# cure-lab/MotionCraft

Hardware: AMD Instinct MI355X
Metric: sampled SMPL-X frames/sec (196-frame seq, 1000-step DDPM) (higher is better)
Workload: dtype f32

## Files before the change

### include/motioncraft_amd.h

```cpp
#ifndef MOTIONCRAFT_AMD_H
#define MOTIONCRAFT_AMD_H
#include <stdint.h>

#ifdef __cplusplus
extern "C" {
#endif

#define MC_OK 0
#define MC_ERR_ARG 1
#define MC_ERR_HIP 2
#define MC_ERR_STATE 3
#define MC_ERR_NOCONV 4

typedef struct mc_model mc_model;
typedef struct mc_ctx mc_ctx;

typedef struct mc_model_config {
    int32_t input_feats;
    int32_t max_seq_len;
    int32_t latent_dim;
    int32_t num_parts;
    int32_t num_layers;
    int32_t ffn_dim;
    int32_t time_embed_dim;
    int32_t text_latent_dim;
    int32_t max_text_len;
    int32_t num_experts;
    int32_t topk;
    int32_t dyn_heads;
    float capacity_factor;
    float cfg_scale;
    int32_t num_ctrl_layers;
    int32_t ctrl_cond_feats;
    int32_t ctrl_condition_cfg;
} mc_model_config;

#define MC_SAMPLER_DDPM 0
#define MC_SAMPLER_DDIM 1
#define MC_SAMPLER_MULTISTEP 2
typedef struct mc_step_coefs {
    int32_t mode;
    float text_coef;
    float none_coef;
    float c1, c2;
    float log_var;
    float sqrt_recip, sqrt_recipm1, ab, ab_prev, eta;
    float nonzero;
} mc_step_coefs;

typedef struct mc_inpaint {
    const float* gt_dev;
    const uint8_t* keep_dev;
    const float* gt_noise_dev;
    const float* blend_w_dev;
    int32_t blend_len;
} mc_inpaint;

#define MC_MAX_TRANSL 8
typedef struct mc_seed {
    const float* pre_seq_dev;
    const float* pre_noise_dev;
    int32_t pre_len;
    float sqrt_ab, sqrt_1mab;
    int32_t num_transl;
    int32_t transl_channel[MC_MAX_TRANSL];
    float transl_value[MC_MAX_TRANSL][2];
} mc_seed;

const char* mc_last_error(void);
int mc_device_count(int* n);
int mc_set_device(int dev);

int mc_model_create(const mc_model_config* cfg, mc_model** out);
void mc_model_destroy(mc_model* m);
int mc_model_set_param(mc_model* m, const char* name, const float* host, int64_t numel);
int mc_model_finalize(mc_model* m);

int mc_ctx_create(mc_model* m, int32_t batch, int32_t frames, int32_t max_steps, mc_ctx** out);
void mc_ctx_destroy(mc_ctx* c);
int64_t mc_ctx_workspace_bytes(const mc_ctx* c);
int mc_ctx_check(mc_ctx* c, void* stream);
int mc_ctx_profile(mc_ctx* c, int32_t on);
int mc_ctx_profile_read(mc_ctx* c, int64_t rows_filter, double* avg_us, int32_t* count, double* gflop_per_launch);
int mc_ctx_effective_precision(const mc_ctx* c);
int mc_ctx_uses_coop_routing(const mc_ctx* c);
int mc_ctx_enable_capture(mc_ctx* c);
#define MC_PREC_F32 0
#define MC_PREC_F16 1
#define MC_PREC_F16X3 2
int mc_ctx_set_precision(mc_ctx* c, int32_t precision);
#define MC_TIE_STABLE 0
#define MC_TIE_REVERSE 1
int mc_ctx_set_tie_policy(mc_ctx* c, int32_t policy);
int mc_ctx_set_option(mc_ctx* c, const char* key, int64_t value);
int mc_ctx_set_timesteps(mc_ctx* c, const int32_t* t_orig_host, int32_t num_steps, void* stream);
int mc_ctx_set_condition(mc_ctx* c, const float* xf_out_dev, const float* mask_dev, void* stream);
int mc_ctx_set_control(mc_ctx* c, const float* c_feat_dev, int32_t Tc, void* stream);

int mc_denoise(mc_ctx* c, const float* x_t_dev, int32_t step_index, float* out2_dev,
               int32_t stop_after_layers, void* stream);
int mc_sample_step(mc_ctx* c, const float* x_t_dev, int32_t step_index, const mc_step_coefs* coefs,
                   const float* noise_dev, float* x_prev_dev, float* x0_dev, void* stream);

int mc_sample_loop(mc_ctx* c, float* x_dev, const int32_t* step_indices_host, const mc_step_coefs* coefs_host, int32_t num_steps,
                   const float* noise_dev, uint64_t seed, uint64_t noise_draw0, float* x0_last_dev, void* stream);
int mc_op_philox_normal(float* out_dev, uint32_t* bits_dev, int64_t n, uint64_t seed, uint64_t draw, void* stream);

int mc_ctx_graph_capture(mc_ctx* c, float* x_dev, const float* noise_dev, const mc_step_coefs* coefs_host, int32_t num_steps,
                         void* stream);
int mc_ctx_graph_step(mc_ctx* c, int32_t step_index, void* stream);
int mc_ctx_graph_release(mc_ctx* c);

int mc_sample_step_seeded(mc_ctx* c, float* x_t_dev, int32_t step_index, const mc_step_coefs* coefs,
                          const float* noise_dev, const mc_seed* seed, float* x_prev_dev, float* x0_dev, void* stream);

int mc_sample_step_inpaint(mc_ctx* c, const float* x_t_dev, int32_t step_index, const mc_step_coefs* coefs,
                           const float* noise_dev, const mc_inpaint* inpaint, float* x_prev_dev, float* x0_dev,
                           void* stream);

int mc_ctx_get_buffer(mc_ctx* c, const char* name, int32_t layer, void** dev_ptr, int64_t* numel);

int mc_debug_flop_ledger(int32_t enable);
int64_t mc_debug_flop_ledger_dump(char* buf, int64_t cap);

enum { MC_ACT_NONE = 0, MC_ACT_GELU = 1, MC_ACT_SILU = 2, MC_ACT_LRELU = 3, MC_ACT_QUICKGELU = 4 };
int mc_op_gemm(const float* a_dev, const float* w_dev, const float* bias_dev, const float* res_dev,
               float* c_dev, int32_t M, int32_t N, int32_t K, int32_t ldw, int32_t act, void* stream);
int mc_op_gemm_f16(const float* a_dev, const float* w_dev, const float* bias_dev, const float* res_dev, float* c_dev,
                   int32_t M, int32_t N, int32_t K, int32_t split, void* stream);
int mc_op_gemm_f16_planes(const void* a_hi_dev, const void* a_lo_dev, const float* w_dev, const float* bias_dev, const float* res_dev,
                          float* c_dev, int32_t M, int32_t N, int32_t K, int32_t split, int32_t pre, int32_t frag_major, void* stream);
int mc_op_gemm_tail(const float* h_dev, const float* a_dev, const float* w_dev, const float* bias_dev, float* c_dev, float* c2_dev,
                    int32_t M, int32_t N, int32_t K, float wc, float wu, int32_t variant, void* stream);
int mc_op_ln_rows(const float* x_dev, int64_t ldx, const float* gamma_dev, const float* beta_dev,
                  const float* add_dev, int32_t add_mod, float* y_dev, int64_t rows, int32_t L, void* stream);
enum { MC_TEMPORAL_STEP = 0,
       MC_TEMPORAL_WHOLE = 1,
       MC_TEMPORAL_LSPLIT = 2,
       MC_TEMPORAL_PAIR = 3,
       MC_TEMPORAL_F16X3 = 4,
       MC_TEMPORAL_F16 = 5 };
int mc_op_body_attention(const float* mf_dev, int64_t ldmf, const float* qkv_dev, const float* wsm_dev, float* ys_dev, int64_t frames,
                         int32_t H, int32_t L, int64_t twin_from, const int32_t* split_flag_dev, int64_t frame0, void* stream);
int mc_op_temporal_attention(const float* mf_dev, const float* tf_dev, const float* mask_dev, float* yt_dev, int32_t b0, int32_t nb,
                             int32_t B, int32_t T, int32_t Nt, int32_t H, int32_t L, int32_t form, int32_t skip_text,
                             const int32_t* twin_flag_dev, void* stream);
enum { MC_ENC_ATTN_LAYER = 0,
       MC_ENC_ATTN_SMALL = 1,
       MC_ENC_ATTN_STREAM = 2 };
int mc_op_enc_ln(const float* x_dev, const float* gamma_dev, const float* beta_dev, float* y_dev, int64_t rows, int32_t L, float eps,
                 int32_t relu, void* stream);
int mc_op_enc_embed_tokens(const int32_t* ids_dev, const float* emb_dev, const float* pos_dev, float* x_dev, int64_t rows, int32_t S,
                           int32_t d, int32_t vocab, void* stream);
int mc_op_enc_attention(const float* qkv_dev, const uint8_t* valid_dev, float* out_dev, int32_t B, int32_t S, int32_t d, int32_t heads,
                        int32_t causal, int32_t form, void* stream);
enum { MC_GM_PLAIN = 0, MC_GM_ENC = 4 };
typedef struct mc_gemm_strided {
    const float* a_dev; int64_t lda, a_gstride;
    const float* w_dev; int64_t ldw, w_gstride;
    const float* bias_dev; int64_t b_gstride;
    float* c_dev; int64_t ldc, c_gstride;
    const float* res_dev; int64_t ldr, r_gstride;
    const float* add_dev; int64_t ld_add, dup_rows;
    int32_t add_mod, act, act_after_res, M, N, K;
} mc_gemm_strided;
int mc_op_gemm_strided(int32_t mode, int32_t groups, const mc_gemm_strided* args, void* stream);
int mc_op_bigru_steps(const float* gi_dev, const float* whh_dev, const float* bhh_dev, float* h_dev, const int32_t* lens_dev,
                      int32_t len_div, int32_t B, int32_t S, int32_t H, int32_t s0, int32_t steps, void* stream);
int mc_op_conv1d_k4s2(const float* x_dev, int64_t ldx, const float* w_tapmajor_dev, const float* bias_dev, float* y_padded_dev, int32_t B,
                      int32_t T, int32_t C, int32_t Cp, int32_t O, float slope, void* stream);
int mc_op_sampler_update(const float* x_t_dev, const float* out_text_dev, const float* out_none_dev,
                         const float* noise_dev, float* x_prev_dev, float* x0_dev, int64_t n,
                         const mc_step_coefs* coefs, void* stream);
int mc_op_sampler_multistep(const float* x_t_dev, const float* out_text_dev, const float* out_none_dev, float* x0_hist_dev,
                            float* x_prev_dev, float* x0_dev, int64_t n, const mc_step_coefs* coefs, void* stream);

#define MC_POST_MAXTAP 129
int mc_postprocess_smplx(const float* pred_dev, const int32_t* lengths_dev, const double* mean_dev,
                         const double* std_dev, const double* taps_dev, const int32_t radius[4], int32_t stats_f32,
                         int32_t B, int32_t T, int32_t C, double* poses_dev, double* expr_dev, double* trans_dev,
                         void* stream);
int mc_postprocess_smplx_stitched(const float* pred_dev, const int32_t* rows_dev, int32_t n_frames,
                                  const double* mean_dev, const double* std_dev, const double* taps_dev,
                                  const int32_t radius[4], int32_t stats_f32, int32_t C, double* poses_dev,
                                  double* expr_dev, double* trans_dev, void* stream);

int mc_postprocess_t2m_joints(const float* pred_dev, const int32_t* lengths_dev, const double* mean_dev,
                              const double* std_dev, const double* taps_dev, int32_t radius, int32_t stats_f32,
                              int32_t B, int32_t T, int32_t C, int32_t joints_num, float* joints_out_dev, void* stream);
int mc_postprocess_t2m_joints_stitched(const float* pred_dev, const int32_t* rows_dev, int32_t n_frames,
                                       const double* mean_dev, const double* std_dev, const double* taps_dev,
                                       int32_t radius, int32_t stats_f32, int32_t C, int32_t joints_num,
                                       double* work_dev, float* joints_out_dev, void* stream);

typedef struct mc_textenc mc_textenc;
typedef struct mc_textenc_config {
    int32_t clip_dim;
    int32_t text_latent_dim;
    int32_t num_layers;
    int32_t ff_size;
    int32_t num_heads;
    int32_t max_len;
    int32_t clip_layers;
    int32_t clip_heads;
    int32_t clip_ff;
    int32_t vocab;
} mc_textenc_config;
int mc_textenc_create(const mc_textenc_config* cfg, mc_textenc** out);
void mc_textenc_destroy(mc_textenc* e);
int mc_textenc_set_param(mc_textenc* e, const char* name, const float* host, int64_t numel);
int mc_textenc_finalize(mc_textenc* e);
int mc_textenc_forward_feat(mc_textenc* e, const float* clip_feat_dev, int32_t B, float* xf_out_dev, void* stream);
int mc_textenc_forward_tokens(mc_textenc* e, const int32_t* tokens_dev, int32_t B, float* clip_feat_out_dev,
                              float* xf_out_dev, void* stream);

typedef struct mc_evalenc mc_evalenc;
typedef struct mc_evalenc_config {
    int32_t nfeats;
    int32_t latent_dim;
    int32_t ff_size;
    int32_t num_layers;
    int32_t num_heads;
    int32_t pe_len;
    int32_t bert_dim;
    int32_t bert_layers;
    int32_t bert_heads;
    int32_t bert_ff;
    int32_t bert_vocab;
    int32_t bert_max_pos;
} mc_evalenc_config;
int mc_evalenc_create(const mc_evalenc_config* cfg, mc_evalenc** out);
void mc_evalenc_destroy(mc_evalenc* e);
int mc_evalenc_set_param(mc_evalenc* e, const char* name, const float* host, int64_t numel);
int mc_evalenc_finalize(mc_evalenc* e);
int mc_evalenc_encode_motion(mc_evalenc* e, const float* motion_dev, const int32_t* lengths_dev, int32_t B, int32_t T,
                             float* mu_out_dev, void* stream);
int mc_evalenc_encode_text(mc_evalenc* e, const int32_t* ids_dev, const uint8_t* mask_dev, int32_t B, int32_t S,
                           float* mu_out_dev, void* stream);

typedef struct mc_t2meval mc_t2meval;
typedef struct mc_t2meval_config {
    int32_t input_size;
    int32_t movement_hidden;
    int32_t movement_latent;
    int32_t motion_hidden;
    int32_t motion_latent;
    int32_t word_size;
    int32_t pos_size;
    int32_t text_hidden;
    int32_t text_out;
} mc_t2meval_config;
int mc_t2meval_create(const mc_t2meval_config* cfg, mc_t2meval** out);
void mc_t2meval_destroy(mc_t2meval* e);
int mc_t2meval_set_param(mc_t2meval* e, const char* name, const float* host, int64_t numel);
int mc_t2meval_finalize(mc_t2meval* e);
int mc_t2meval_encode_motion(mc_t2meval* e, const float* motion_dev, const int32_t* lengths_dev, int32_t B, int32_t T,
                             float* out_dev, void* stream);
int mc_t2meval_encode_text(mc_t2meval* e, const float* word_emb_dev, const float* pos_onehot_dev, const int32_t* sent_len_dev,
                           int32_t B, int32_t S, float* out_dev, void* stream);

typedef struct mc_wavenc mc_wavenc;
int mc_wavenc_create(int32_t audio_in, int32_t out_dim, mc_wavenc** out);
void mc_wavenc_destroy(mc_wavenc* e);
int mc_wavenc_set_param(mc_wavenc* e, const char* name, const float* host, int64_t numel);
int mc_wavenc_finalize(mc_wavenc* e);
int mc_wavenc_out_len(const mc_wavenc* e, int32_t samples, int32_t* frames);
int mc_wavenc_forward(mc_wavenc* e, const float* wav_dev, int32_t B, int32_t samples, float* out_dev, void* stream);

typedef struct mc_smplx mc_smplx;
typedef struct mc_smplx_config {
    int32_t num_vertices;
    int32_t num_joints;
    int32_t num_betas;
    int32_t num_expr;
    int32_t num_pose_feats;
} mc_smplx_config;
int mc_smplx_create(const mc_smplx_config* cfg, mc_smplx** out);
void mc_smplx_destroy(mc_smplx* m);
int mc_smplx_set_param(mc_smplx* m, const char* name, const float* host, int64_t numel);
int mc_smplx_finalize(mc_smplx* m);
int mc_smplx_joints(mc_smplx* m, const double* poses_dev, const double* expr_dev, const double* trans_dev,
                    const double* betas_dev, int32_t betas_per_frame, int32_t n, float* joints_out_dev, void* stream);
int64_t mc_smplx_work_bytes(const mc_smplx* m, int32_t n_frames, int32_t betas_per_frame);
int mc_smplx_vertices(mc_smplx* m, const double* poses_dev, const double* expr_dev, const double* trans_dev,
                      const double* betas_dev, int32_t betas_per_frame, int32_t n, void* work_dev, int64_t work_bytes,
                      float* verts_out_dev, float* joints_out_dev, void* stream);
int64_t mc_smplx_vertex_errors_work_bytes(const mc_smplx* m, int32_t chunk_frames, int32_t n_frames, int32_t betas_per_frame);
int mc_smplx_vertex_errors(mc_smplx* m, const double* poses_a_dev, const double* expr_a_dev, const double* trans_a_dev,
                           const double* poses_b_dev, const double* expr_b_dev, const double* trans_b_dev, const double* betas_dev,
                           int32_t betas_per_frame, int32_t n, void* work_dev, int64_t work_bytes, double* sums_out_dev, void* stream);

#define MC_BEAT_MAX_ORDER 64
#define MC_BEAT_MAX_UPPER 64
int mc_beat_mask(const float* joints_dev, int32_t n_frames, int32_t num_joints, const double* mean_vel_dev, int32_t mean_vel_fp32,
                 int32_t t_start, int32_t t_end, double pose_fps, int32_t order, double threshold, uint8_t* mask_out_dev, void* stream);
int64_t mc_beat_align_work_bytes(int32_t n_slice, int32_t n_upper);
int mc_beat_align(const uint8_t* mask_dev, int32_t num_joints, int32_t n_slice, const int32_t* upper_body_host, int32_t n_upper,
                  const double* onsets_dev, int32_t n_onsets, double pose_fps, double sigma, void* work_dev, int64_t work_bytes,
                  double* score_out_dev, void* stream);

#define MC_ONSET_N_FFT 2048
#define MC_ONSET_MAX_HOP 512
#define MC_ONSET_MAX_MELS 128
int64_t mc_onset_work_bytes(int64_t n_samples, int32_t n_fft, int32_t hop, int32_t n_mels);
int mc_onset_strength(const float* wave_dev, int64_t n_samples, const float* dft_dev, const float* mel_dev, int32_t n_fft, int32_t hop,
                      int32_t n_mels, void* work_dev, int64_t work_bytes, float* env_out_dev, void* stream);
int mc_onset_pick(const float* env_dev, int32_t n_frames, int32_t pre_max, int32_t post_max, int32_t pre_avg, int32_t post_avg, double delta,
                  int32_t wait, int32_t normalize, uint8_t* mask_out_dev, int32_t* count_out_dev, void* stream);

#define MC_AUDIO_COND_MAX_WINDOW 1024
#define MC_AUDIO_COND_TILE 4096
int mc_audio_condition(const float* wave_dev, int64_t n_samples, int32_t window, const uint8_t* onset_mask_dev, int32_t n_frames,
                       float* out_dev, void* stream);

#define MC_RESAMPLE_TILE 512
int mc_pcm_decode(const uint8_t* pcm_dev, int64_t n_frames, int32_t channels, int32_t sample_bytes, int32_t mono, float* out_dev, void* stream);
int64_t mc_resample_out_len(int64_t n_in, int32_t up, int32_t down);
int mc_resample_poly(const float* x_dev, int64_t n_in, int32_t up, int32_t down, const double* taps_dev, int32_t n_taps, float* y_dev,
                     int64_t n_out, void* stream);
// ... 76 lines not shown
```

### motioncraft_amd/csrc/mc_ctx.h

```cpp
#pragma once
#include <map>
#include <mutex>
#include <string>
#include <vector>

#include "../../include/motioncraft_amd.h"
#include "mc_common.h"
#include "mc_gemm.h"
#include "mc_kernels.h"
#include "mc_chain.h"
#include "mc_half.h"
#include "mc_options.h"
#include "mc_params.h"

struct mc_model {
    mc_model_config cfg;
    ParamStore params{""};
    std::map<std::string, HalfW> half;
    std::mutex half_mu;
    size_t half_bytes = 0;
    bool finalized = false;
    int Cp = 0;
};

struct MoeW {
    const float *emb, *gate_w, *gate_b, *sim_n, *sim_nT, *scale, *fc1_w, *fc1_b, *fc2_wt, *fc2_b, *proj_w, *proj_b;
    int din, dout;
};

struct LayerW {
    const float *norm_g, *norm_b, *tnorm_g, *tnorm_b, *wsm;
    MoeW mm, tm;
    const float *dyn_g, *dyn_b, *qkv_w, *qkv_b;
    const float *ca_film_w, *ca_film_b, *ca_ln_g, *ca_ln_b, *ca_out_w, *ca_out_b;
    const float *ffn_w1, *ffn_b1, *ffn_w2, *ffn_b2;
    const float *ffn_film_w, *ffn_film_b, *ffn_ln_g, *ffn_ln_b, *ffn_out_w, *ffn_out_b;
    const float *before_w = nullptr, *before_b = nullptr, *after_w = nullptr, *after_b = nullptr;
    HalfW h_ca_out, h_ffn_out, h_fc1, h_fc2, h_w1, h_w2, h_after, h_proj, h_qkv;
};

struct ProfRec { hipEvent_t e0 = nullptr, e1 = nullptr; long rows = 0; };

struct mc_ctx {
    mc_model* m = nullptr;
    McOptions opt{};
    int B = 0, T = 0, S = 0, maxS = 0;
    long N = 0, rows = 0, Ntxt = 0;
    std::vector<LayerW> lw;
    const float *enc_w, *enc_b, *seq_emb, *time_w0, *time_b0, *time_w2, *time_b2, *dec_w, *dec_b;
    const float *dec_wf = nullptr, *dec_bf = nullptr;
    float *dec_cat_w = nullptr, *dec_cat_b = nullptr;
    const float *ctrl_in_w = nullptr, *ctrl_in_b = nullptr;
    int NLA = 0;
    float *hc = nullptr, *cb = nullptr, *cenc = nullptr;
    bool have_ctrl = false;
    std::vector<void*> allocs;
    int64_t bytes = 0;
    float *h, *z, *proj, *hbuf, *y2, *mf, *qkv, *ys, *yt, *a, *z2, *fh, *out2, *xpad;
    float* a_tail = nullptr;
    size_t hbuf_cap = 0;
    size_t hbuf_floats = 0;
    bool cnt_clean = false;
    long led_nsrc = 0, led_gsplit = 0;
    float *xfn, *tf;
    const float* mask = nullptr;
    float* mask_own = nullptr;
    int* t_orig;
    float *te, *e1, *emb, *semb, *ss;
    RouteBufs rb;
    int device = 0;
    int coop_reserved = 0;
    bool prof_on = false;
    std::vector<ProfRec> prof;
    bool have_cond = false;
    hipStream_t side = nullptr;
    bool xpad_ready = false;
    hipEvent_t ev_fork = nullptr, ev_join = nullptr;
    hipEvent_t ev_side = nullptr;
    hipEvent_t ev_stag = nullptr;
    hipEvent_t ev_gate1 = nullptr, ev_sel = nullptr, ev_front = nullptr;
    bool early_clean = false;
    bool no_alias = false;
    bool defer_last_gemm = false;
    static constexpr int SIDE_CAND = 4;
    hipStream_t side_cand[SIDE_CAND] = {nullptr, nullptr, nullptr, nullptr};
    hipStream_t side_for = nullptr;
    bool side_picked = false;
    float side_probe_ms[SIDE_CAND] = {0.f, 0.f, 0.f, 0.f};
    static constexpr int SIDE_MEMO = 4;
    hipStream_t side_memo_for[SIDE_MEMO] = {nullptr, nullptr, nullptr, nullptr};
    int side_memo_pick[SIDE_MEMO] = {-1, -1, -1, -1};
    int side_memo_n = 0;
    int* gstep = nullptr;
    SamplerCoefs* gcoefs = nullptr;
    bool graph_mode = false;
    hipGraph_t graph = nullptr;
    hipGraphExec_t graph_exec = nullptr;
    int graph_steps = 0;
    float* x0_hist = nullptr;
    bool hist_valid = false;
    bool graph_multistep = false;
    std::vector<float> graph_k1;
    int prec = MC_PREC_F32;
    int* cap_idx = nullptr;
    float* cap_w = nullptr;
};

#pragma GCC visibility push(hidden)
inline bool chain_on(const mc_ctx* c, ChainBit which) { return (c->opt.chain >> which) & 1; }
bool use_half(const mc_ctx* c);
int dense(const mc_ctx* c, const float* A, long lda, const float* W, long ldw, const float* bias, const float* R, long ldr,
          float* C, long ldc, long M, int N, int K, int act, hipStream_t s);
int run_moe(mc_ctx* c, const MoeW& w, const float* z, long Ntok, float* out, long ldout, bool gated, bool twin, long gsplit,
            hipStream_t s, const HalfW* hw, const HalfW* hw2);
inline float* deferred_a(const mc_ctx* c) { return c->a_tail ? c->a_tail : c->a; }
bool a_holds_planes(const mc_ctx* c);
int denoise_impl(mc_ctx* c, const float* x_t, int32_t step, float* out2_dev, int32_t stop_after, void* stream, const SeedArgs* seed);
SamplerCoefs to_coefs(const mc_step_coefs* k);

struct X0Parts {
    const float *a = nullptr, *b = nullptr;
    const float* second() const { return b ? b : a; }
    SamplerCoefs coefs(const mc_step_coefs* k) const {
        SamplerCoefs sc = to_coefs(k);
        sc.text_coef = 1.f; sc.none_coef = b ? 1.f : 0.f;
        return sc;
    }
};
int denoise_combined(mc_ctx* c, const float* x_t, int32_t step, const mc_step_coefs* k, void* stream, X0Parts* x0, const SeedArgs* seed = nullptr);
int sampler_update(mc_ctx* c, const float* x_t, const X0Parts& x0p, const mc_step_coefs* k, const float* noise, float* x_prev, float* x0,
                   hipStream_t s, const RngArgs* rng = nullptr, const PadOut* pad = nullptr);
#pragma GCC visibility pop
```

### motioncraft_amd/csrc/mc_gemm.h

```cpp
#pragma once
#include <hip/hip_runtime.h>
#include "mc_options.h"
#include "../../include/motioncraft_amd.h"

enum { GM_PLAIN = MC_GM_PLAIN, GM_EXP1 = 1, GM_EXP2 = 2, GM_COMB = 3, GM_ENC = MC_GM_ENC };

enum : int {
    kTuneStaging = 1 << 0,
    kTuneDma = 1 << 4,
    kTuneWp = 1 << 5,
    kTuneNoXcd = 1 << 6,
    kTuneSmallXcd = 1 << 8,
    kTuneEncWp = 1 << 9,
    kTuneTail2 = 1 << 10,
    kTuneBits = kTuneStaging | kTuneDma | kTuneWp | kTuneNoXcd | kTuneSmallXcd | kTuneEncWp | kTuneTail2,
    kTuneDefault = kTuneBits & ~kTuneNoXcd,
};
static_assert(kTuneDefault == 1841, "the default tune bits are public ABI");

struct GemmArgs {
    const float* A = nullptr;
    long lda = 0;
    int a_col = 0;
    long a_gstride = 0;
    const float* W = nullptr;
    long ldw = 0;
    long w_gstride = 0;
    const float* bias = nullptr;
    long b_gstride = 0;
    float* C = nullptr;
    long ldc = 0;
    int c_col = 0;
    long c_gstride = 0;
    const float* R = nullptr;
    long ldr = 0;
    long r_gstride = -1;
    int act = 0;
    int act_after_res = 0;
    const float* add = nullptr;
    int add_mod = 1;
    long ld_add = 0;
    long dup_rows = 0;
    int M = 0, N = 0, K = 0;
    const int* tile_group = nullptr;
    const int* tile_row0 = nullptr;
    const int* tile_nrows = nullptr;
    const int* num_tiles = nullptr;
    const int* src_row = nullptr;
    const int* dst_row = nullptr;
    const float* comb_w = nullptr;
    int small_tile_n = 0;
    int wp_grid = 0;
    int tune = -1;
};

inline void mc_gemm_opts(const McOptions& o, GemmArgs& g) {
    g.tune = (int)o.gemm_tune;
    g.small_tile_n = o.small_tile_n ? (int)o.small_tile_n : -1;
    g.wp_grid = o.gemm_wp_grid > 0 ? (int)o.gemm_wp_grid : -1;
}

inline double mc_cu_load(long workgroups) {
    const long n = (workgroups + 255) / 256;
    return (1.45 * (double)(n / 2) + (double)(n % 2));
}

int mc_device_cus();
int mc_launch_gemm(int mode, const GemmArgs& g, int groups, int max_tiles, hipStream_t stream);
int mc_launch_gemm_small(const GemmArgs& g, hipStream_t stream, int groups = 1);

struct TailArgs {
    const float* H = nullptr;
    const float* Af = nullptr;
    long half = 0, lda = 0;
    const float* W = nullptr;
    long ldw = 0, w_gstride = 0;
    const float* bias = nullptr;
    long b_gstride = 0;
    float* C = nullptr;
    float* C2 = nullptr;
    long ldc = 0;
    int M = 0, N = 0, K = 0;
    float wc = 1.f, wu = 0.f;
    const float* coef_table = nullptr;
    const int* step_ptr = nullptr;
    long coef_stride = 0;
    int tune = -1;
};
int mc_launch_gemm_tail(const TailArgs& g, hipStream_t stream);
bool mc_gemm_tail_two_outputs(const TailArgs& g);
```

### motioncraft_amd/csrc/mc_gemm.hip

```cpp
#include "mc_common.h"
#include "mc_gemm.h"

namespace {

constexpr int BM = 128, BN = 128, BK = 32, LD = BK + 4;

struct Stage {
    long aoff[4], woff[4];
    bool aok[4], wok[4];
    float cw0[4], cw1[4];
};

template <int MODE, bool GUARD>
__device__ __forceinline__ void load_tile(const GemmArgs& g, const float* __restrict__ Ab, const float* __restrict__ Wb,
                                          const Stage& st, int k, f32x4 (&ra)[4], f32x4 (&rb)[4]) {
    const bool kin = !GUARD || k < g.K;
#pragma unroll
    for (int i = 0; i < 4; ++i) {
        f32x4 v = {0.f, 0.f, 0.f, 0.f};
        if ((!GUARD || st.aok[i]) && kin) {
            if constexpr (MODE == GM_COMB) {
                f32x4 y0 = {0.f, 0.f, 0.f, 0.f}, y1 = {0.f, 0.f, 0.f, 0.f};
                if (st.cw0[i] != 0.f) y0 = *reinterpret_cast<const f32x4*>(Ab + st.aoff[i] + k);
                if (st.cw1[i] != 0.f) y1 = *reinterpret_cast<const f32x4*>(Ab + st.aoff[i] + g.lda + k);
#pragma unroll
                for (int j = 0; j < 4; ++j) v[j] = gelu_exact(st.cw0[i] * y0[j] + st.cw1[i] * y1[j]);
            } else if constexpr (MODE == GM_ENC && GUARD) {
#pragma unroll
                for (int j = 0; j < 4; ++j)
                    if (k + j < g.K) v[j] = Ab[st.aoff[i] + k + j];
            } else {
                v = *reinterpret_cast<const f32x4*>(Ab + st.aoff[i] + k);
            }
        }
        ra[i] = v;
        f32x4 w = {0.f, 0.f, 0.f, 0.f};
        if ((!GUARD || st.wok[i]) && kin) w = *reinterpret_cast<const f32x4*>(Wb + st.woff[i] + k);
        rb[i] = w;
    }
}

template <int MODE, bool GUARD, bool EARLY>
__device__ __forceinline__ void mainloop(const GemmArgs& g, const float* __restrict__ Ab, const float* __restrict__ Wb,
                                         const Stage& st, float* As, float* Bs, int sr, int sk, int wm, int wn, int lane,
                                         f32x16 (&acc)[2][2]) {
    f32x4 ra[4], rb[4];
    auto store_tile = [&](int buf) {
#pragma unroll
        for (int i = 0; i < 4; ++i) {
            *reinterpret_cast<f32x4*>(As + buf * BM * LD + (sr + 32 * i) * LD + sk) = ra[i];
            *reinterpret_cast<f32x4*>(Bs + buf * BN * LD + (sr + 32 * i) * LD + sk) = rb[i];
        }
    };
    const int nk = (g.K + BK - 1) / BK;
    const int frow = lane & 31;
    const int fk = (lane >> 5) * 4;
    struct Frag { f32x4 a0, a1, b0, b1; };
    auto ld_frag = [&](const float* Ap, const float* Bp, int j) {
        Frag f;
        f.a0 = *reinterpret_cast<const f32x4*>(Ap + j * 8);
        f.a1 = *reinterpret_cast<const f32x4*>(Ap + 32 * LD + j * 8);
        f.b0 = *reinterpret_cast<const f32x4*>(Bp + j * 8);
        f.b1 = *reinterpret_cast<const f32x4*>(Bp + 32 * LD + j * 8);
        return f;
    };
    auto mma = [&](const Frag& f) {
#pragma unroll
        for (int i = 0; i < 4; ++i) {
            acc[0][0] = __builtin_amdgcn_mfma_f32_32x32x2f32(f.b0[i], f.a0[i], acc[0][0], 0, 0, 0);
            acc[0][1] = __builtin_amdgcn_mfma_f32_32x32x2f32(f.b1[i], f.a0[i], acc[0][1], 0, 0, 0);
            acc[1][0] = __builtin_amdgcn_mfma_f32_32x32x2f32(f.b0[i], f.a1[i], acc[1][0], 0, 0, 0);
            acc[1][1] = __builtin_amdgcn_mfma_f32_32x32x2f32(f.b1[i], f.a1[i], acc[1][1], 0, 0, 0);
        }
    };
    if constexpr (!EARLY) {
        load_tile<MODE, GUARD>(g, Ab, Wb, st, sk, ra, rb);
        store_tile(0);
        __syncthreads();
        for (int kt = 0; kt < nk; ++kt) {
            const int buf = kt & 1;
            if (kt + 1 < nk) load_tile<MODE, GUARD>(g, Ab, Wb, st, (kt + 1) * BK + sk, ra, rb);
            const float* Ap = As + buf * BM * LD + (wm * 64 + frow) * LD + fk;
            const float* Bp = Bs + buf * BN * LD + (wn * 64 + frow) * LD + fk;
            Frag f0 = ld_frag(Ap, Bp, 0);
            Frag f1 = ld_frag(Ap, Bp, 1);
            mma(f0);
            f0 = ld_frag(Ap, Bp, 2);
            mma(f1);
            f1 = ld_frag(Ap, Bp, 3);
            mma(f0);
            mma(f1);
            if (kt + 1 < nk) store_tile(buf ^ 1);
            __syncthreads();
        }
    } else {
        load_tile<MODE, GUARD>(g, Ab, Wb, st, sk, ra, rb);
        store_tile(0);
        if (nk > 1) load_tile<MODE, GUARD>(g, Ab, Wb, st, BK + sk, ra, rb);
        __syncthreads();
        for (int kt = 0; kt < nk; ++kt) {
            const int buf = kt & 1;
            const float* Ap = As + buf * BM * LD + (wm * 64 + frow) * LD + fk;
            const float* Bp = Bs + buf * BN * LD + (wn * 64 + frow) * LD + fk;
            Frag f0 = ld_frag(Ap, Bp, 0);
            Frag f1 = ld_frag(Ap, Bp, 1);
            mma(f0);
            f0 = ld_frag(Ap, Bp, 2);
            if (kt + 1 < nk) store_tile(buf ^ 1);
            if (kt + 2 < nk) load_tile<MODE, GUARD>(g, Ab, Wb, st, (kt + 2) * BK + sk, ra, rb);
            mma(f1);
            f1 = ld_frag(Ap, Bp, 3);
            mma(f0);
            mma(f1);
            __syncthreads();
        }
    }
}

template <int MODE, bool GUARD, int ACT>
__device__ __forceinline__ void epilogue_vec(const GemmArgs& g, int grp, int row0, int nrows, int tn, int wm, int wn,
                                             int lane, f32x16 (&acc)[2][2]) {
    const float* __restrict__ bias = g.bias ? g.bias + (long)grp * g.b_gstride : nullptr;
    float* __restrict__ Cb = g.C + (long)grp * g.c_gstride + g.c_col;
    const float* __restrict__ Rb = g.R ? g.R + (long)grp * (g.r_gstride >= 0 ? g.r_gstride : g.c_gstride) + g.c_col : nullptr;
#pragma unroll
    for (int mi = 0; mi < 2; ++mi) {
        const int m = wm * 64 + mi * 32 + (lane & 31);
        if (GUARD && m >= nrows) continue;
        long drow = row0 + m;
        if constexpr (MODE == GM_EXP2) drow = g.dst_row[row0 + m];
        float* crow = Cb + drow * g.ldc;
        const float* rrow = Rb ? Rb + drow * g.ldr : nullptr;
        const float* arow = nullptr;
        if constexpr (MODE == GM_ENC) arow = g.add ? g.add + (long)((row0 + m) % g.add_mod) * g.ld_add : nullptr;
#pragma unroll
        for (int ni = 0; ni < 2; ++ni) {
#pragma unroll
            for (int q = 0; q < 4; ++q) {
                const int n = tn * BN + wn * 64 + ni * 32 + 8 * q + 4 * (lane >> 5);
                if (GUARD && n >= g.N) continue;
                f32x4 v = {acc[mi][ni][4 * q], acc[mi][ni][4 * q + 1], acc[mi][ni][4 * q + 2], acc[mi][ni][4 * q + 3]};
                if (bias) v += *reinterpret_cast<const f32x4*>(bias + n);
                if (g.act_after_res && rrow) v += *reinterpret_cast<const f32x4*>(rrow + n);
#pragma unroll
                for (int j = 0; j < 4; ++j) v[j] = apply_act(v[j], ACT);
                if constexpr (MODE == GM_ENC) {
                    if (arow) v += *reinterpret_cast<const f32x4*>(arow + n);
                }
                if (!g.act_after_res && rrow) v += *reinterpret_cast<const f32x4*>(rrow + n);
                *reinterpret_cast<f32x4*>(crow + n) = v;
                if constexpr (MODE == GM_ENC) {
                    if (g.dup_rows) *reinterpret_cast<f32x4*>(crow + g.dup_rows * g.ldc + n) = v;
                }
            }
// ... 52 lines not shown
    }
    const int tm = bid / ntn, tn = bid % ntn;
    int row0, nrows;
    if constexpr (MODE == GM_EXP1 || MODE == GM_EXP2) {
        grp = g.tile_group[tm];
        row0 = g.tile_row0[tm];
        nrows = g.tile_nrows[tm];
    } else {
        row0 = tm * BM;
        nrows = min(BM, g.M - row0);
        if (nrows <= 0) return;
    }
    const float* __restrict__ Ab = g.A + (long)grp * g.a_gstride + g.a_col;
    const float* __restrict__ Wb = g.W + (long)grp * g.w_gstride;

    const int sr = tid >> 3;
    const int sk = (tid & 7) * 4;
    Stage st;
#pragma unroll
    for (int i = 0; i < 4; ++i) {
        const int r = sr + 32 * i;
        st.aok[i] = r < nrows;
        long srow = row0 + r;
        if constexpr (MODE == GM_EXP1) srow = st.aok[i] ? g.src_row[row0 + r] : 0;
        if constexpr (MODE == GM_COMB) {
            st.aoff[i] = 2 * srow * g.lda;
            st.cw0[i] = st.aok[i] ? g.comb_w[2 * srow] : 0.f;
            st.cw1[i] = st.aok[i] ? g.comb_w[2 * srow + 1] : 0.f;
        } else {
            st.aoff[i] = srow * g.lda;
        }
        const int n = tn * BN + r;
        st.wok[i] = n < g.N;
        st.woff[i] = (long)n * g.ldw;
    }

    f32x16 acc[2][2];
#pragma unroll
    for (int mi = 0; mi < 2; ++mi)
#pragma unroll
        for (int ni = 0; ni < 2; ++ni)
#pragma unroll
            for (int r = 0; r < 16; ++r) acc[mi][ni][r] = 0.f;

    const bool full = nrows == BM && (tn + 1) * BN <= g.N && (g.K % BK) == 0 &&
                      (MODE != GM_ENC || (g.lda % 4 == 0 && g.a_gstride % 4 == 0));
    if (full) {
        if (g.tune & kTuneStaging) mainloop<MODE, false, true>(g, Ab, Wb, st, As, Bs, sr, sk, wm, wn, lane, acc);
        else mainloop<MODE, false, false>(g, Ab, Wb, st, As, Bs, sr, sk, wm, wn, lane, acc);
    } else {
        mainloop<MODE, true, false>(g, Ab, Wb, st, As, Bs, sr, sk, wm, wn, lane, acc);
    }

    const bool vec = (g.N % 4 == 0) && (g.ldc % 4 == 0) && (g.c_col % 4 == 0) && (g.c_gstride % 4 == 0) &&
                     (!g.R || (g.ldr % 4 == 0 && (g.r_gstride < 0 || g.r_gstride % 4 == 0)));
    if (!vec) {
        epilogue_scalar<MODE>(g, grp, row0, nrows, tn, wm, wn, lane, acc);
    } else if (full) {
        if (g.act == ACT_GELU) epilogue_vec<MODE, false, ACT_GELU>(g, grp, row0, nrows, tn, wm, wn, lane, acc);
        else if (g.act == ACT_SILU) epilogue_vec<MODE, false, ACT_SILU>(g, grp, row0, nrows, tn, wm, wn, lane, acc);
        else if (g.act == ACT_LRELU) epilogue_vec<MODE, false, ACT_LRELU>(g, grp, row0, nrows, tn, wm, wn, lane, acc);
        else if (g.act == ACT_QUICKGELU) epilogue_vec<MODE, false, ACT_QUICKGELU>(g, grp, row0, nrows, tn, wm, wn, lane, acc);
        else epilogue_vec<MODE, false, ACT_NONE>(g, grp, row0, nrows, tn, wm, wn, lane, acc);
    } else {
        if (g.act == ACT_GELU) epilogue_vec<MODE, true, ACT_GELU>(g, grp, row0, nrows, tn, wm, wn, lane, acc);
        else if (g.act == ACT_SILU) epilogue_vec<MODE, true, ACT_SILU>(g, grp, row0, nrows, tn, wm, wn, lane, acc);
        else if (g.act == ACT_LRELU) epilogue_vec<MODE, true, ACT_LRELU>(g, grp, row0, nrows, tn, wm, wn, lane, acc);
        else if (g.act == ACT_QUICKGELU) epilogue_vec<MODE, true, ACT_QUICKGELU>(g, grp, row0, nrows, tn, wm, wn, lane, acc);
        else epilogue_vec<MODE, true, ACT_NONE>(g, grp, row0, nrows, tn, wm, wn, lane, acc);
    }
}

__global__ __launch_bounds__(256, 2) void gemm_dma_k(GemmArgs g) {
    __shared__ __attribute__((aligned(16))) float smem[2 * (BM + BN) * BK];
    float* As = smem;
    float* Bs = smem + 2 * BM * BK;
    const int tid = threadIdx.x, lane = tid & 63, wave = tid >> 6;
    const int wm = wave >> 1, wn = wave & 1;
    const int ntn = g.N / BN;
    const int bid = (g.tune & kTuneNoXcd) ? (int)blockIdx.x : xcd_remap(blockIdx.x, gridDim.x);
    const int tm = bid / ntn, tn = bid % ntn;
    const int row0 = tm * BM;
    const float* __restrict__ Ab = g.A + g.a_col;
    const float* __restrict__ Wb = g.W;
    const int dr = lane >> 3, dc = ((lane & 7) ^ dr) * 4;
    const float* ga = Ab + (long)(row0 + 32 * wave + dr) * g.lda + dc;
    const float* gw = Wb + (long)(tn * BN + 32 * wave + dr) * g.ldw + dc;
    const int wave_u = __builtin_amdgcn_readfirstlane(wave);
    auto issue = [&](int kt, int buf) {
        float* la = As + buf * BM * BK + 32 * wave_u * BK;
        float* lw = Bs + buf * BN * BK + 32 * wave_u * BK;
#pragma unroll
        for (int q = 0; q < 4; ++q) {
            __builtin_amdgcn_global_load_lds(ga + (long)8 * q * g.lda + kt * BK, la + 8 * q * BK, 16, 0, 0);
            __builtin_amdgcn_global_load_lds(gw + (long)8 * q * g.ldw + kt * BK, lw + 8 * q * BK, 16, 0, 0);
        }
    };
    f32x16 acc[2][2];
#pragma unroll
    for (int mi = 0; mi < 2; ++mi)
#pragma unroll
        for (int ni = 0; ni < 2; ++ni)
#pragma unroll
            for (int r = 0; r < 16; ++r) acc[mi][ni][r] = 0.f;
    const int frow = lane & 31, hf = lane >> 5, sw = frow & 7;
    struct Frag { f32x4 a0, a1, b0, b1; };
    auto ld_frag = [&](const float* At, const float* Bt, int j) {
        const int pos = ((2 * j + hf) ^ sw) * 4;
        Frag f;
        f.a0 = *reinterpret_cast<const f32x4*>(At + pos);
        f.a1 = *reinterpret_cast<const f32x4*>(At + 32 * BK + pos);
        f.b0 = *reinterpret_cast<const f32x4*>(Bt + pos);
        f.b1 = *reinterpret_cast<const f32x4*>(Bt + 32 * BK + pos);
        return f;
    };
    auto mma = [&](const Frag& f) {
#pragma unroll
        for (int i = 0; i < 4; ++i) {
            acc[0][0] = __builtin_amdgcn_mfma_f32_32x32x2f32(f.b0[i], f.a0[i], acc[0][0], 0, 0, 0);
            acc[0][1] = __builtin_amdgcn_mfma_f32_32x32x2f32(f.b1[i], f.a0[i], acc[0][1], 0, 0, 0);
            acc[1][0] = __builtin_amdgcn_mfma_f32_32x32x2f32(f.b0[i], f.a1[i], acc[1][0], 0, 0, 0);
            acc[1][1] = __builtin_amdgcn_mfma_f32_32x32x2f32(f.b1[i], f.a1[i], acc[1][1], 0, 0, 0);
        }
    };
    const int nk = g.K / BK;
    issue(0, 0);
    __syncthreads();
    for (int kt = 0; kt < nk; ++kt) {
        const int buf = kt & 1;
        if (kt + 1 < nk) issue(kt + 1, buf ^ 1);
        const float* At = As + buf * BM * BK + (wm * 64 + frow) * BK;
        const float* Bt = Bs + buf * BN * BK + (wn * 64 + frow) * BK;
        Frag f0 = ld_frag(At, Bt, 0);
        Frag f1 = ld_frag(At, Bt, 1);
        __builtin_amdgcn_sched_barrier(0);
        mma(f0);
        f0 = ld_frag(At, Bt, 2);
        __builtin_amdgcn_sched_barrier(0);
        mma(f1);
        f1 = ld_frag(At, Bt, 3);
        __builtin_amdgcn_sched_barrier(0);
        mma(f0);
        mma(f1);
        __syncthreads();
    }
    if (g.act == ACT_GELU) epilogue_vec<GM_PLAIN, false, ACT_GELU>(g, 0, row0, BM, tn, wm, wn, lane, acc);
    else if (g.act == ACT_SILU) epilogue_vec<GM_PLAIN, false, ACT_SILU>(g, 0, row0, BM, tn, wm, wn, lane, acc);
    else if (g.act == ACT_NONE) epilogue_vec<GM_PLAIN, false, ACT_NONE>(g, 0, row0, BM, tn, wm, wn, lane, acc);
    else epilogue_vec<GM_PLAIN, false, ACT_LRELU>(g, 0, row0, BM, tn, wm, wn, lane, acc);
}

constexpr int WBK = 16, WSTAGE = 128 * WBK;

__global__ __launch_bounds__(256, 2) void gemm_wp_k(GemmArgs g) {
    __shared__ __attribute__((aligned(16))) float smem[4 * 2 * WSTAGE];
    const int tid = threadIdx.x, lane = tid & 63, wave = tid >> 6;
    const int wm = wave >> 1, wn = wave & 1;
    const int ntn = g.N / BN, ntiles = (g.M / BM) * ntn;
    const int wave_u = __builtin_amdgcn_readfirstlane(wave);
    float* wbase = smem + wave_u * 2 * WSTAGE;
    const unsigned lds0 = (unsigned)(size_t)wbase;
    const int dr = lane >> 2, dc = ((lane & 3) ^ ((dr >> 2) & 3)) * 4;
    const int frow = lane & 31, hf = lane >> 5, sw = (frow >> 2) & 3;
    const float* Ab = g.A + g.a_col;
    const float* Wb = g.W;
    const float* __restrict__ Rb = g.R ? g.R + g.c_col : nullptr;
    float* __restrict__ Cb = g.C + g.c_col;
    const int nk = g.K / WBK;
    struct Frag { f32x4 a0, a1, b0, b1; };
    auto ld_frag = [&](int st, int j) {
        const float* S = wbase + st * WSTAGE + frow * WBK + ((2 * j + hf) ^ sw) * 4;
        Frag f;
        f.a0 = *reinterpret_cast<const f32x4*>(S);
        f.a1 = *reinterpret_cast<const f32x4*>(S + 32 * WBK);
        f.b0 = *reinterpret_cast<const f32x4*>(S + 64 * WBK);
        f.b1 = *reinterpret_cast<const f32x4*>(S + 96 * WBK);
        return f;
    };
    for (int t = blockIdx.x; t < ntiles; t += gridDim.x) {
        const int bid = (g.tune & kTuneNoXcd) ? t : xcd_remap(t, ntiles);
        const int tm = bid / ntn, tn = bid % ntn;
        const int row0 = tm * BM;
        unsigned voa[4], vow[4];
#pragma unroll
        for (int q = 0; q < 4; ++q) {
            voa[q] = (unsigned)(((long)(row0 + wm * 64 + 16 * q + dr) * g.lda + dc) * 4);
            vow[q] = (unsigned)(((long)(tn * BN + wn * 64 + 16 * q + dr) * g.ldw + dc) * 4);
        }
        auto issue_q = [&](int kt, int st, int q) {
            const unsigned l = lds0 + st * WSTAGE * 4;
            dma16(voa[q], Ab + kt * WBK, l + q * 1024);
            dma16(vow[q], Wb + kt * WBK, l + 4096 + q * 1024);
        };
        f32x16 acc[2][2];
#pragma unroll
        for (int mi = 0; mi < 2; ++mi)
#pragma unroll
            for (int ni = 0; ni < 2; ++ni)
#pragma unroll
                for (int r = 0; r < 16; ++r) acc[mi][ni][r] = 0.f;
        auto mma2 = [&](const Frag& f, int i0) {
#pragma unroll
            for (int i = i0; i < i0 + 2; ++i) {
                acc[0][0] = __builtin_amdgcn_mfma_f32_32x32x2f32(f.b0[i], f.a0[i], acc[0][0], 0, 0, 0);
                acc[0][1] = __builtin_amdgcn_mfma_f32_32x32x2f32(f.b1[i], f.a0[i], acc[0][1], 0, 0, 0);
                acc[1][0] = __builtin_amdgcn_mfma_f32_32x32x2f32(f.b0[i], f.a1[i], acc[1][0], 0, 0, 0);
                acc[1][1] = __builtin_amdgcn_mfma_f32_32x32x2f32(f.b1[i], f.a1[i], acc[1][1], 0, 0, 0);
            }
        };
#pragma unroll
        for (int q = 0; q < 4; ++q) issue_q(0, 0, q);
        asm volatile("s_waitcnt vmcnt(0)" ::: "memory");
        Frag f0 = ld_frag(0, 0);
        auto ktile = [&](int kt) {
            const int st = kt & 1;
            const bool more = kt + 1 < nk;
            Frag f1 = ld_frag(st, 1);
            __builtin_amdgcn_sched_barrier(0);
            mma2(f0, 0);
            if (more) { issue_q(kt + 1, st ^ 1, 0); issue_q(kt + 1, st ^ 1, 1); }
            __builtin_amdgcn_sched_barrier(0);
            mma2(f0, 2);
            if (more) { issue_q(kt + 1, st ^ 1, 2); issue_q(kt + 1, st ^ 1, 3); }
            __builtin_amdgcn_sched_barrier(0);
            mma2(f1, 0);
            if (more) {
                asm volatile("s_waitcnt vmcnt(0)" ::: "memory");
                f0 = ld_frag(st ^ 1, 0);
            }
            __builtin_amdgcn_sched_barrier(0);
            mma2(f1, 2);
        };
        const int npre = nk > 2 ? nk - 2 : 0;
        for (int kt = 0; kt < npre; ++kt) ktile(kt);
        f32x4 rv[2][2][4], bv[2][4];
#pragma unroll
        for (int ni = 0; ni < 2; ++ni)
#pragma unroll
            for (int q = 0; q < 4; ++q) {
                const int n = tn * BN + wn * 64 + ni * 32 + 8 * q + 4 * hf;
                bv[ni][q] = g.bias ? *reinterpret_cast<const f32x4*>(g.bias + n) : f32x4{0.f, 0.f, 0.f, 0.f};
#pragma unroll
                for (int mi = 0; mi < 2; ++mi) {
                    const long m = row0 + wm * 64 + mi * 32 + frow;
                    rv[mi][ni][q] = Rb ? *reinterpret_cast<const f32x4*>(Rb + m * g.ldr + n) : f32x4{0.f, 0.f, 0.f, 0.f};
                    if (g.add) rv[mi][ni][q] = *reinterpret_cast<const f32x4*>(g.add + (m % g.add_mod) * g.ld_add + n);
                }
            }
        for (int kt = npre; kt < nk; ++kt) ktile(kt);
#pragma unroll
        for (int mi = 0; mi < 2; ++mi) {
            float* crow = Cb + (long)(row0 + wm * 64 + mi * 32 + frow) * g.ldc;
#pragma unroll
            for (int ni = 0; ni < 2; ++ni)
#pragma unroll
                for (int q = 0; q < 4; ++q) {
                    const int n = tn * BN + wn * 64 + ni * 32 + 8 * q + 4 * hf;
                    f32x4 v = {acc[mi][ni][4 * q], acc[mi][ni][4 * q + 1], acc[mi][ni][4 * q + 2], acc[mi][ni][4 * q + 3]};
                    v += bv[ni][q];
                    if (g.act != ACT_NONE) {
#pragma unroll
                        for (int jj = 0; jj < 4; ++jj) v[jj] = apply_act(v[jj], g.act);
                    }
                    v += rv[mi][ni][q];
                    *reinterpret_cast<f32x4*>(crow + n) = v;
                    if (g.dup_rows) *reinterpret_cast<f32x4*>(crow + g.dup_rows * g.ldc + n) = v;
                }
        }
    }
}

constexpr int SM = 64, SN = 64, SRING = 4;
template <bool VEC>
__global__ __launch_bounds__(256) void gemm_small_k(GemmArgs g) {
    __shared__ __attribute__((aligned(16))) float smem[SRING * 2 * SM * BK];
    const int tid = threadIdx.x, lane = tid & 63, wave = tid >> 6;
    const int wm = wave >> 1, wn = wave & 1;
    const int ntn = (g.N + SN - 1) / SN;
    const int bid = (g.tune & kTuneSmallXcd) ? xcd_remap((int)blockIdx.x, (int)gridDim.x) : (int)blockIdx.x;
    const int tm = bid / ntn, tn = bid % ntn, grp = blockIdx.y;
    const int row0 = tm * SM;
    const int wave_u = __builtin_amdgcn_readfirstlane(wave);
    const int dr = lane >> 3, dc = ((lane & 7) ^ dr) * 4;
    const float* Ab = g.A + (long)grp * g.a_gstride + g.a_col;
    const float* Wb = g.W + (long)grp * g.w_gstride;
    unsigned voa[2], vow[2];
#pragma unroll
    for (int q = 0; q < 2; ++q) {
        const int ar = min(row0 + 16 * wave + 8 * q + dr, g.M - 1), wr = min(tn * SN + 16 * wave + 8 * q + dr, g.N - 1);
        voa[q] = (unsigned)(((long)ar * g.lda + dc) * 4);
        vow[q] = (unsigned)(((long)wr * g.ldw + dc) * 4);
    }
    const unsigned lds0 = (unsigned)(size_t)smem + (unsigned)(16 * wave_u) * BK * 4;
    auto issue = [&](int kt) {
        const unsigned l = lds0 + (unsigned)(kt & (SRING - 1)) * (2 * SM * BK * 4);
#pragma unroll
        for (int q = 0; q < 2; ++q) {
            dma16(voa[q], Ab + kt * BK, l + q * 8 * BK * 4);
            dma16(vow[q], Wb + kt * BK, l + SM * BK * 4 + q * 8 * BK * 4);
        }
    };
    f32x16 acc;
#pragma unroll
    for (int r = 0; r < 16; ++r) acc[r] = 0.f;
    const int nk = g.K / BK;
    const int frow = lane & 31, hf = lane >> 5, sw = frow & 7;
    const int me = min(row0 + wm * 32 + frow, g.M - 1);
    const long rgs = g.r_gstride >= 0 ? g.r_gstride : g.c_gstride;
    f32x4 pb[4], pa[4], pr[4];
    if constexpr (VEC) {
#pragma unroll
        for (int q = 0; q < 4; ++q) {
            const int n = tn * SN + wn * 32 + 8 * q + 4 * hf;
            const f32x4 z = {0.f, 0.f, 0.f, 0.f};
            pb[q] = g.bias ? *reinterpret_cast<const f32x4*>(g.bias + (long)grp * g.b_gstride + n) : z;
            pa[q] = g.add ? *reinterpret_cast<const f32x4*>(g.add + (long)(me % g.add_mod) * g.ld_add + n) : z;
            pr[q] = g.R ? *reinterpret_cast<const f32x4*>(g.R + (long)grp * rgs + (long)me * g.ldr + g.c_col + n) : z;
        }
    }
    for (int kt = 0; kt < SRING - 1 && kt < nk; ++kt) issue(kt);
    for (int kt = 0; kt < nk; ++kt) {
        const int ahead = min(nk - 1 - kt, SRING - 2);
        if (ahead == 2) asm volatile("s_waitcnt vmcnt(8)" ::: "memory");
        else if (ahead == 1) asm volatile("s_waitcnt vmcnt(4)" ::: "memory");
        else asm volatile("s_waitcnt vmcnt(0)" ::: "memory");
        __syncthreads();
        if (kt + SRING - 1 < nk) issue(kt + SRING - 1);
        const float* St = smem + (kt & (SRING - 1)) * (2 * SM * BK);
        const float* At = St + (wm * 32 + frow) * BK;
        const float* Bt = St + SM * BK + (wn * 32 + frow) * BK;
        f32x4 fa[4], fb[4];
#pragma unroll
        for (int j = 0; j < 4; ++j) {
            const int pos = ((2 * j + hf) ^ sw) * 4;
            fa[j] = *reinterpret_cast<const f32x4*>(At + pos);
            fb[j] = *reinterpret_cast<const f32x4*>(Bt + pos);
        }
        __builtin_amdgcn_sched_barrier(0);
#pragma unroll
        for (int j = 0; j < 4; ++j)
#pragma unroll
            for (int i = 0; i < 4; ++i) acc = __builtin_amdgcn_mfma_f32_32x32x2f32(fb[j][i], fa[j][i], acc, 0, 0, 0);
    }
    const int m = row0 + wm * 32 + frow;
    if (m >= g.M) return;
    float* crow = g.C + (long)grp * g.c_gstride + (long)m * g.ldc + g.c_col;
    const float* rrow = g.R ? g.R + (long)grp * rgs + (long)m * g.ldr + g.c_col : nullptr;
    const float* arow = g.add ? g.add + (long)(m % g.add_mod) * g.ld_add : nullptr;
    const float* bias = g.bias ? g.bias + (long)grp * g.b_gstride : nullptr;
#pragma unroll
    for (int q = 0; q < 4; ++q) {
        const int n = tn * SN + wn * 32 + 8 * q + 4 * hf;
        f32x4 v = {acc[4 * q], acc[4 * q + 1], acc[4 * q + 2], acc[4 * q + 3]};
        if constexpr (VEC) {
            v += pb[q];
            v += pa[q];
            v += pr[q];
            *reinterpret_cast<f32x4*>(crow + n) = v;
            if (g.dup_rows) *reinterpret_cast<f32x4*>(crow + g.dup_rows * g.ldc + n) = v;
        } else {
#pragma unroll
            for (int i = 0; i < 4; ++i) {
                if (n + i >= g.N) continue;
                float x = v[i];
                if (bias) x += bias[n + i];
                if (arow) x += arow[n + i];
                if (rrow) x += rrow[n + i];
                crow[n + i] = x;
                if (g.dup_rows) crow[g.dup_rows * g.ldc + n + i] = x;
            }
        }
    }
}

template <int NBLK, bool VEC>
__global__ __launch_bounds__(256) void gemm_small16_k(GemmArgs g) {
    constexpr int NB = 16 * NBLK, NWP = NB / 8;
    constexpr int STAGE = (SM + NB) * BK;
    __shared__ __attribute__((aligned(16))) float smem[SRING * STAGE];
    const int tid = threadIdx.x, lane = tid & 63, wave = tid >> 6;
    const int ntn = (g.N + NB - 1) / NB;
    const int bid = (g.tune & kTuneSmallXcd) ? xcd_remap((int)blockIdx.x, (int)gridDim.x) : (int)blockIdx.x;
    const int tm = bid / ntn, tn = bid % ntn, grp = blockIdx.y;
    const int row0 = tm * SM;
    const int wave_u = __builtin_amdgcn_readfirstlane(wave);
    const int dr = lane >> 3, dc = ((lane & 7) ^ dr) * 4;
    const float* Ab = g.A + (long)grp * g.a_gstride + g.a_col;
    const float* Wb = g.W + (long)grp * g.w_gstride;
    constexpr int MAXW = (NWP + 3) / 4;
    unsigned voa[2], vow[MAXW];
#pragma unroll
    for (int q = 0; q < 2; ++q) voa[q] = (unsigned)(((long)min(row0 + 16 * wave + 8 * q + dr, g.M - 1) * g.lda + dc) * 4);
#pragma unroll
    for (int q = 0; q < MAXW; ++q) vow[q] = (unsigned)(((long)min(tn * NB + 8 * (wave + 4 * q) + dr, g.N - 1) * g.ldw + dc) * 4);
    const int nw = (NWP - wave_u + 3) / 4;
    const unsigned lds_base = (unsigned)(size_t)smem;
    auto issue = [&](int kt) {
        const unsigned l = lds_base + (unsigned)(kt & (SRING - 1)) * (STAGE * 4);
#pragma unroll
        for (int q = 0; q < 2; ++q) dma16(voa[q], Ab + kt * BK, l + (unsigned)(16 * wave_u + 8 * q) * BK * 4);
#pragma unroll
        for (int q = 0; q < MAXW; ++q)
            if (q < nw) dma16(vow[q], Wb + kt * BK, l + SM * BK * 4 + (unsigned)(8 * (wave_u + 4 * q)) * BK * 4);
    };
    f32x4 acc[NBLK];
#pragma unroll
    for (int b = 0; b < NBLK; ++b) acc[b] = f32x4{0.f, 0.f, 0.f, 0.f};
    const int nk = g.K / BK;
    const int frow = lane & 15, kg = lane >> 4;
    const int per = 2 + nw;
    const int sw = frow & 7;
    const int me = min(row0 + 16 * wave + frow, g.M - 1);
    const long rgs = g.r_gstride >= 0 ? g.r_gstride : g.c_gstride;
    f32x4 pb[NBLK], pa[NBLK], pr[NBLK];
    if constexpr (VEC) {
#pragma unroll
        for (int b = 0; b < NBLK; ++b) {
            const int n = tn * NB + 16 * b + 4 * kg;
            const f32x4 z = {0.f, 0.f, 0.f, 0.f};
            pb[b] = g.bias ? *reinterpret_cast<const f32x4*>(g.bias + (long)grp * g.b_gstride + n) : z;
            pa[b] = g.add ? *reinterpret_cast<const f32x4*>(g.add + (long)(me % g.add_mod) * g.ld_add + n) : z;
// ... 56 lines not shown
                if (bias) x += bias[n + i];
                if (arow) x += arow[n + i];
                if (rrow) x += rrow[n + i];
                crow[n + i] = x;
                if (g.dup_rows) crow[g.dup_rows * g.ldc + n + i] = x;
            }
        }
    }
}

__device__ __forceinline__ void gload16(f32x4& v, const float* p) {
    asm volatile("global_load_dwordx4 %0, %1, off" : "=v"(v) : "v"(p) : "memory");
}

__device__ __forceinline__ void vm_wait(int n) {
    switch (n) {
        case 0: asm volatile("s_waitcnt vmcnt(0)" ::: "memory"); break;
        case 1: asm volatile("s_waitcnt vmcnt(1)" ::: "memory"); break;
        case 2: asm volatile("s_waitcnt vmcnt(2)" ::: "memory"); break;
        case 3: asm volatile("s_waitcnt vmcnt(3)" ::: "memory"); break;
        case 4: asm volatile("s_waitcnt vmcnt(4)" ::: "memory"); break;
        case 5: asm volatile("s_waitcnt vmcnt(5)" ::: "memory"); break;
        case 6: asm volatile("s_waitcnt vmcnt(6)" ::: "memory"); break;
        case 7: asm volatile("s_waitcnt vmcnt(7)" ::: "memory"); break;
        case 8: asm volatile("s_waitcnt vmcnt(8)" ::: "memory"); break;
        case 9: asm volatile("s_waitcnt vmcnt(9)" ::: "memory"); break;
        case 10: asm volatile("s_waitcnt vmcnt(10)" ::: "memory"); break;
        case 11: asm volatile("s_waitcnt vmcnt(11)" ::: "memory"); break;
        case 12: asm volatile("s_waitcnt vmcnt(12)" ::: "memory"); break;
        case 13: asm volatile("s_waitcnt vmcnt(13)" ::: "memory"); break;
        default: asm volatile("s_waitcnt vmcnt(14)" ::: "memory"); break;
    }
}

template <int NBLK>
__global__ __launch_bounds__(256) void gemm_tail_k(TailArgs g) {
    constexpr int NB = 16 * NBLK, NWP = NB / 8;
    constexpr int STAGE = (SM + NB) * BK;
    __shared__ __attribute__((aligned(16))) float smem[SRING * STAGE];
    const int tid = threadIdx.x, lane = tid & 63, wave = tid >> 6;
    const int ntn = (g.N + NB - 1) / NB;
    const int bid = (g.tune & kTuneSmallXcd) ? xcd_remap((int)blockIdx.x, (int)gridDim.x) : (int)blockIdx.x;
    const int tm = bid / ntn, tn = bid % ntn;
    const int row0 = tm * SM;
    const int wave_u = __builtin_amdgcn_readfirstlane(wave);
    float wc = g.wc, wu = g.wu;
    if (g.coef_table) { wc = g.coef_table[(long)*g.step_ptr * g.coef_stride]; wu = g.coef_table[(long)*g.step_ptr * g.coef_stride + 1]; }
    long aoff[2];
    int alds[2];
#pragma unroll
    for (int j = 0; j < 2; ++j) {
        const int i = tid + 256 * j, row = i >> 3, pos = i & 7;
        aoff[j] = (long)min(row0 + row, g.M - 1) * g.lda + ((pos ^ (row & 7)) << 2);
        alds[j] = row * BK + (pos << 2);
    }
    const int dr = lane >> 3, dc = ((lane & 7) ^ dr) * 4;
    constexpr int MAXW = (NWP + 3) / 4;
    unsigned vow[MAXW];
#pragma unroll
    for (int q = 0; q < MAXW; ++q) vow[q] = (unsigned)(((long)min(tn * NB + 8 * (wave + 4 * q) + dr, g.N - 1) * g.ldw + dc) * 4);
    const int nw = (NWP - wave_u + 3) / 4;
    const unsigned lds_base = (unsigned)(size_t)smem;
    const int nk = g.K / BK, NK = 2 * nk;
    auto a_load = [&](int kt, f32x4 (&c)[2], f32x4 (&u)[2]) {
        const float* A = (kt < nk ? g.H : g.Af) + (long)(kt < nk ? kt : kt - nk) * BK;
#pragma unroll
        for (int j = 0; j < 2; ++j) {
            gload16(c[j], A + aoff[j]);
            gload16(u[j], A + g.half + aoff[j]);
        }
    };
    auto a_store = [&](int kt, const f32x4 (&c)[2], const f32x4 (&u)[2]) {
        float* St = smem + (kt & (SRING - 1)) * STAGE;
#pragma unroll
        for (int j = 0; j < 2; ++j) {
            f32x4 v;
#pragma unroll
            for (int i = 0; i < 4; ++i) v[i] = wc * c[j][i] + wu * u[j][i];
            *reinterpret_cast<f32x4*>(St + alds[j]) = v;
        }
    };
    auto w_issue = [&](int kt) {
        const float* Wb = g.W + (kt < nk ? 0 : g.w_gstride) + (long)(kt < nk ? kt : kt - nk) * BK;
        const unsigned l = lds_base + (unsigned)(kt & (SRING - 1)) * (STAGE * 4) + SM * BK * 4;
#pragma unroll
        for (int q = 0; q < MAXW; ++q)
            if (q < nw) dma16(vow[q], Wb, l + (unsigned)(8 * (wave_u + 4 * q)) * BK * 4);
    };
    f32x4 acc[NBLK];
#pragma unroll
    for (int b = 0; b < NBLK; ++b) acc[b] = f32x4{0.f, 0.f, 0.f, 0.f};
    const int frow = lane & 15, kg = lane >> 4;
    const int sw = frow & 7;
    f32x4 c0[2], u0[2], c1[2], u1[2], c2[2], u2[2];
    a_load(0, c0, u0);
    w_issue(0);
    if (NK > 1) { a_load(1, c1, u1); w_issue(1); }
    if (NK > 2) { a_load(2, c2, u2); w_issue(2); }
    constexpr int A_OPS = 4;
    static_assert(NWP <= 8, "a wave issues at most two W pieces per stage: the counted waits below assume nw <= 2");
    vm_wait(NK > 2 ? 3 * nw + 2 * A_OPS : 0);
    asm volatile("" : "+v"(c0[0]), "+v"(c0[1]), "+v"(u0[0]), "+v"(u0[1]));
    a_store(0, c0, u0);
    auto step = [&](int kt, f32x4 (&cs)[2], f32x4 (&us)[2], f32x4 (&cl)[2], f32x4 (&ul)[2]) {
        vm_wait(kt + 2 < NK ? 2 * nw + A_OPS : 0);
        asm volatile("" : "+v"(cs[0]), "+v"(cs[1]), "+v"(us[0]), "+v"(us[1]));
        __syncthreads();
        if (kt + 1 < NK) a_store(kt + 1, cs, us);
        if (kt + 3 < NK) { a_load(kt + 3, cl, ul); w_issue(kt + 3); }
        const float* St = smem + (kt & (SRING - 1)) * STAGE;
        const float* At = St + (16 * wave + frow) * BK;
        const float* Bt = St + SM * BK + frow * BK;
        f32x4 fa[2], fb[NBLK][2];
#pragma unroll
        for (int j = 0; j < 2; ++j) {
            const int pos = ((4 * j + kg) ^ sw) * 4;
            fa[j] = *reinterpret_cast<const f32x4*>(At + pos);
#pragma unroll
            for (int b = 0; b < NBLK; ++b) fb[b][j] = *reinterpret_cast<const f32x4*>(Bt + b * 16 * BK + pos);
        }
        __builtin_amdgcn_sched_barrier(0);
#pragma unroll
        for (int j = 0; j < 2; ++j)
#pragma unroll
            for (int i = 0; i < 4; ++i)
#pragma unroll
                for (int b = 0; b < NBLK; ++b) acc[b] = __builtin_amdgcn_mfma_f32_16x16x4f32(fb[b][j][i], fa[j][i], acc[b], 0, 0, 0);
    };
    for (int kt = 0; kt < NK; kt += 3) {
        step(kt, c1, u1, c0, u0);
        if (kt + 1 < NK) step(kt + 1, c2, u2, c1, u1);
        if (kt + 2 < NK) step(kt + 2, c0, u0, c2, u2);
    }
    const int m = row0 + 16 * wave + frow;
    if (m >= g.M) return;
    float* crow = g.C + (long)m * g.ldc;
#pragma unroll
    for (int b = 0; b < NBLK; ++b) {
        const int n = tn * NB + 16 * b + 4 * kg;
#pragma unroll
        for (int i = 0; i < 4; ++i) {
            if (n + i >= g.N) continue;
            crow[n + i] = acc[b][i] + (g.bias[n + i] + g.bias[g.b_gstride + n + i]);
        }
    }
}

constexpr int T2_BK = 16, T2_MAXCB = 21, T2_MAXRT = 5, T2_RING = 3;
constexpr int T2_STAGE = 16 * (T2_MAXRT + T2_MAXCB) * T2_BK;
constexpr int T2_WROW0 = 16 * T2_MAXRT;

__device__ __forceinline__ int t2_swz(int row) { return (0x78 >> (2 * ((row >> 2) & 3))) & 3; }

template <int NBW>
__global__ __launch_bounds__(256, 2) void gemm_tail2_k(TailArgs g, int ncb, long nblocks) {
    static_assert(NBW % 4 == 0 && NBW >= 4 && NBW <= 16, "NBW");
    constexpr int PH = 4;
    __shared__ __attribute__((aligned(16))) float smem[T2_RING * T2_STAGE];
    const int tid = threadIdx.x, lane = tid & 63;
    const int qw = __builtin_amdgcn_readfirstlane(tid >> 6);
    float wc = g.wc, wu = g.wu;
    if (g.coef_table) { wc = g.coef_table[(long)*g.step_ptr * g.coef_stride]; wu = g.coef_table[(long)*g.step_ptr * g.coef_stride + 1]; }
    const int G = gridDim.x >> 1, rid = xcd_remap((int)blockIdx.x, (int)gridDim.x);
    const int wg = rid >> 1, grp = rid & 1;
    const long gb0 = nblocks * wg / G, gb1 = nblocks * (wg + 1) / G;
    const int n = (int)(gb1 - gb0);
    if (n <= 0) return;
    const int rt_first = (int)(gb0 / ncb), nrt = (int)((gb1 - 1) / ncb) - rt_first + 1;
    const int wb0 = qw * n / 4, wb1 = (qw + 1) * n / 4, nb = wb1 - wb0;
    const int frow = lane & 15, kg = lane >> 4;
    const int lfrag = frow * T2_BK + ((kg ^ t2_swz(frow)) << 2);
    const int g0 = (int)(gb0 - (long)rt_first * ncb) + wb0;
    int aoff[NBW + 1], boff[NBW + 1];
    {
        int rt = g0 / ncb, cb = g0 - rt * ncb;
#pragma unroll
        for (int b = 0; b <= NBW; ++b) {
            aoff[b] = rt * 16 * T2_BK;
            boff[b] = (T2_WROW0 + 16 * cb) * T2_BK;
            if (b + 1 < nb) { if (++cb == ncb) { cb = 0; ++rt; } }
        }
    }
    const float* Asrc = grp ? g.Af : g.H;
    long a_go[2];
    int a_lds[2];
#pragma unroll
    for (int j = 0; j < 2; ++j) {
        const int s = tid + 256 * j, row = s >> 2, pos = s & 3;
        long grow = (long)rt_first * 16 + row;
        if (grow > g.M - 1) grow = g.M - 1;
        a_go[j] = grow * g.lda + ((pos ^ t2_swz(row)) << 2);
        a_lds[j] = row * T2_BK + (pos << 2);
    }
    const int nslot = (qw < nrt ? 1 : 0) + ((4 + qw) < nrt ? 1 : 0);
    const int na = 2 * nslot;
    constexpr int MAXP = (T2_MAXCB + 3) / 4;
    unsigned vow[MAXP];
    {
        const int dr = lane >> 2, pos = lane & 3;
#pragma unroll
        for (int q = 0; q < MAXP; ++q) {
            int wr = 16 * (qw + 4 * q) + dr;
            if (wr > g.N - 1) wr = g.N - 1;
            vow[q] = (unsigned)(((long)wr * g.ldw + ((pos ^ t2_swz(dr)) << 2)) * 4);
        }
    }
    const int nwp = qw < ncb ? (ncb - qw + 3) / 4 : 0;
    const float* Wsrc = g.W + (grp ? g.w_gstride : 0);
    const unsigned lds_q = (unsigned)(size_t)smem;
    const int nk = g.K / T2_BK;
    auto a_load = [&](int kt, f32x4 (&c)[2], f32x4 (&u)[2]) {
        const float* A = Asrc + (long)kt * T2_BK;
#pragma unroll
        for (int j = 0; j < 2; ++j)
            if (j < nslot) { gload16(c[j], A + a_go[j]); gload16(u[j], A + g.half + a_go[j]); }
    };
    auto a_store = [&](int kt, const f32x4 (&c)[2], const f32x4 (&u)[2]) {
        float* St = smem + (kt % T2_RING) * T2_STAGE;
#pragma unroll
        for (int j = 0; j < 2; ++j)
            if (j < nslot) {
                f32x4 v;
#pragma unroll
                for (int i = 0; i < 4; ++i) v[i] = wc * c[j][i] + wu * u[j][i];
                *reinterpret_cast<f32x4*>(St + a_lds[j]) = v;
            }
    };
    auto w_issue = [&](int kt) {
        const float* Wb = Wsrc + (long)kt * T2_BK;
        const unsigned l = lds_q + (unsigned)((kt % T2_RING) * T2_STAGE + T2_WROW0 * T2_BK) * 4;
#pragma unroll
        for (int q = 0; q < MAXP; ++q)
            if (q < nwp) dma16(vow[q], Wb, l + (unsigned)(16 * (qw + 4 * q)) * T2_BK * 4);
    };
    f32x4 acc[NBW + 1];
#pragma unroll
    for (int b = 0; b <= NBW; ++b) acc[b] = f32x4{0.f, 0.f, 0.f, 0.f};
    f32x4 c0[2], u0[2], c1[2], u1[2];
    a_load(0, c0, u0);
    vm_wait(0);
    asm volatile("" : "+v"(c0[0]), "+v"(c0[1]), "+v"(u0[0]), "+v"(u0[1]));
    a_store(0, c0, u0);
    a_load(1, c1, u1);
    w_issue(0);
    if (nk > 2) a_load(2, c0, u0);
    if (nk > 1) w_issue(1);
    auto step = [&](int kt, f32x4 (&cs)[2], f32x4 (&us)[2]) {
        vm_wait((kt + 2 < nk ? na : 0) + (kt + 1 < nk ? nwp : 0));
        asm volatile("" : "+v"(cs[0]), "+v"(cs[1]), "+v"(us[0]), "+v"(us[1]));
        if (kt + 1 < nk) a_store(kt + 1, cs, us);
        __syncthreads();
        if (kt + 3 < nk) a_load(kt + 3, cs, us);
        if (kt + 2 < nk) w_issue(kt + 2);
        const float* St = smem + (kt % T2_RING) * T2_STAGE + lfrag;
#pragma unroll
        for (int p0 = 0; p0 < NBW; p0 += PH) {
            f32x4 fa[PH], fb[PH];
#pragma unroll
            for (int b = 0; b < PH; ++b) {
                fa[b] = *reinterpret_cast<const f32x4*>(St + aoff[p0 + b]);
                fb[b] = *reinterpret_cast<const f32x4*>(St + boff[p0 + b]);
            }
#pragma unroll
            for (int i = 0; i < 4; ++i)
#pragma unroll
                for (int b = 0; b < PH; ++b)
                    acc[p0 + b] = __builtin_amdgcn_mfma_f32_16x16x4f32(fb[b][i], fa[b][i], acc[p0 + b], 0, 0, 0);
        }
        if (nb > NBW) {
            const f32x4 fa = *reinterpret_cast<const f32x4*>(St + aoff[NBW]);
            const f32x4 fb = *reinterpret_cast<const f32x4*>(St + boff[NBW]);
#pragma unroll
            for (int i = 0; i < 4; ++i) acc[NBW] = __builtin_amdgcn_mfma_f32_16x16x4f32(fb[i], fa[i], acc[NBW], 0, 0, 0);
        }
    };
    for (int kt = 0; kt < nk; kt += 2) {
        step(kt, c1, u1);
        if (kt + 1 < nk) step(kt + 1, c0, u0);
    }
    float* Cout = grp ? g.C2 : g.C;
    {
        int rt = g0 / ncb, cb = g0 - rt * ncb;
#pragma unroll
        for (int b = 0; b <= NBW; ++b) {
            if (b < nb) {
                const long m = ((long)rt_first + rt) * 16 + frow;
                const int n0 = cb * 16 + 4 * kg;
                if (m < g.M) {
                    float* crow = Cout + m * g.ldc;
#pragma unroll
                    for (int i = 0; i < 4; ++i)
                        if (n0 + i < g.N) crow[n0 + i] = grp ? acc[b][i] : acc[b][i] + (g.bias[n0 + i] + g.bias[g.b_gstride + n0 + i]);
                }
                if (++cb == ncb) { cb = 0; ++rt; }
            }
        }
    }
}

}

static int resolve_opts(GemmArgs& g) {
    if (g.tune >= 0 && g.small_tile_n && g.wp_grid) return MC_OK;
    const McOptions* o = mc_process_options();
    if (!o) return MC_ERR_ARG;
    GemmArgs p;
    mc_gemm_opts(*o, p);
    g.tune = g.tune < 0 ? p.tune : g.tune;
    g.small_tile_n = g.small_tile_n ? g.small_tile_n : p.small_tile_n;
    g.wp_grid = g.wp_grid ? g.wp_grid : p.wp_grid;
    return MC_OK;
}
int mc_launch_gemm_small(const GemmArgs& g, hipStream_t stream, int groups) {
    MC_REQUIRE(g.K % BK == 0 && g.lda % 4 == 0 && g.ldw % 4 == 0 && g.a_col % 4 == 0 && g.a_gstride % 4 == 0 && g.w_gstride % 4 == 0 &&
                   g.act == ACT_NONE,
               "gemm_small: unsupported shape / options (M=%d N=%d K=%d)", g.M, g.N, g.K);
    if (g.M <= 0 || g.N <= 0) return MC_OK;
    MC_REQUIRE((long)g.M * g.lda * 4 < (1L << 32) && (long)g.N * g.ldw * 4 < (1L << 32),
               "gemm_small: operands beyond 4 GB (the DMA takes 32-bit byte offsets into A and W; this kernel is for a few thousand rows)");
    const bool vec = g.N % SN == 0 && g.ldc % 4 == 0 && g.c_col % 4 == 0 && g.c_gstride % 4 == 0 && (!g.R || (g.ldr % 4 == 0 && (g.r_gstride < 0 || g.r_gstride % 4 == 0))) &&
                     (!g.add || g.ld_add % 4 == 0) && g.b_gstride % 4 == 0;
    const int ng = groups > 0 ? groups : 1;
    GemmArgs gg = g;
    if (int r = resolve_opts(gg)) return r;
    auto cost = [&](int nb, double unit) { return mc_cu_load((long)cdiv(g.M, SM) * cdiv(g.N, nb) * ng) * unit; };
    int nb = SN;
    double best = cost(SN, 30.0);
    const bool any_width = g.M > 6400;
    if ((g.N % 48 == 0 || any_width) && cost(48, 23.0) < 0.97 * best) { nb = 48; best = cost(48, 23.0); }
    if ((g.N % 96 == 0 || any_width) && cost(96, 41.0) < 0.97 * best) { nb = 96; best = cost(96, 41.0); }
    if (gg.small_tile_n == 64 || gg.small_tile_n == 48 || gg.small_tile_n == 96) nb = gg.small_tile_n;
    dim3 grid(cdiv(g.M, SM) * cdiv(g.N, nb), ng);
    const bool vec16 = vec && g.N % nb == 0;
    MC_LEDGER(nb == 48 ? "gemm_small16_k<3" : nb == 96 ? "gemm_small16_k<6" : "gemm_small_k", grid, 2.0 * g.M * g.N * g.K * ng);
    if (nb == 48) {
        if (vec16) hipLaunchKernelGGL((gemm_small16_k<3, true>), grid, dim3(256), 0, stream, gg);
        else hipLaunchKernelGGL((gemm_small16_k<3, false>), grid, dim3(256), 0, stream, gg);
    } else if (nb == 96) {
        if (vec16) hipLaunchKernelGGL((gemm_small16_k<6, true>), grid, dim3(256), 0, stream, gg);
        else hipLaunchKernelGGL((gemm_small16_k<6, false>), grid, dim3(256), 0, stream, gg);
    } else {
        if (vec) hipLaunchKernelGGL(gemm_small_k<true>, grid, dim3(256), 0, stream, gg);
        else hipLaunchKernelGGL(gemm_small_k<false>, grid, dim3(256), 0, stream, gg);
    }
    MC_LAUNCH_CHECK();
    return MC_OK;
}

int mc_launch_gemm(int mode, const GemmArgs& g0, int groups, int max_tiles, hipStream_t stream) {
    GemmArgs g = g0;
    if (int r = resolve_opts(g)) return r;
    const int ntn = cdiv(g.N, BN);
    int ntm = (mode == GM_EXP1 || mode == GM_EXP2) ? max_tiles : cdiv(g.M, BM);
    if (ntm <= 0 || ntn <= 0) return MC_OK;
    if (mode != GM_ENC) MC_REQUIRE(g.K % 4 == 0 && g.lda % 4 == 0 && g.ldw % 4 == 0, "gemm: K/lda/ldw must be multiples of 4");
    if (mode == GM_ENC && (g.add || g.dup_rows))
        MC_REQUIRE(g.N % 4 == 0 && g.ldc % 4 == 0 && g.c_col % 4 == 0 && g.c_gstride % 4 == 0 && (!g.add || g.ld_add % 4 == 0) &&
                       (!g.R || (g.ldr % 4 == 0 && (g.r_gstride < 0 || g.r_gstride % 4 == 0))),
                   "gemm: an add table or duplicate rows need 16-byte aligned output rows (N=%d ldc=%ld)", g.N, g.ldc);
    dim3 grid(ntm * ntn, groups > 0 ? groups : 1, 1);
    const bool vec_out = (g.ldc % 4 == 0) && (g.c_col % 4 == 0) && (!g.R || g.ldr % 4 == 0);
    const bool wp_ok = (g.tune & kTuneWp) && g.K % WBK == 0 && (long)g.M * g.lda * 4 < (1L << 32) && (long)g.N * g.ldw * 4 < (1L << 32);
    const bool enc_fast = mode == GM_ENC && (g.tune & kTuneEncWp) && wp_ok && !g.R && g.add && g.ld_add % 4 == 0 && g.act == ACT_NONE;
    if ((g.tune & kTuneDma) && (mode == GM_PLAIN || enc_fast) && groups <= 1 && g.M % BM == 0 && g.N % BN == 0 && (g.K % BK == 0 || enc_fast) &&
        g.lda % 4 == 0 && g.ldw % 4 == 0 && g.a_col % 4 == 0 && vec_out && g.act != ACT_QUICKGELU && !g.act_after_res &&
        (enc_fast || (!g.add && !g.dup_rows))) {
        if (wp_ok) {
            const int persistent = g.wp_grid > 0 ? g.wp_grid : (int)grid.x;
            MC_LEDGER("gemm_wp_k", dim3(grid.x < persistent ? grid.x : persistent), 2.0 * g.M * g.N * g.K);
            hipLaunchKernelGGL(gemm_wp_k, dim3(grid.x < persistent ? grid.x : persistent), dim3(256), 0, stream, g);
        } else {
            MC_LEDGER("gemm_dma_k", grid, 2.0 * g.M * g.N * g.K);
            hipLaunchKernelGGL(gemm_dma_k, grid, dim3(256), 0, stream, g);
        }
        MC_LAUNCH_CHECK();
        return MC_OK;
    }
    if (mc_ledger_on) {
        char name[24];
        snprintf(name, sizeof(name), "gemm_k<%d>", mode);
        const double rows = (mode == GM_EXP1 || mode == GM_EXP2) ? (double)ntm * BM : (double)g.M;
        MC_LEDGER(name, grid, 2.0 * rows * g.N * g.K * (groups > 0 ? groups : 1));
    }
    switch (mode) {
        case GM_PLAIN: hipLaunchKernelGGL(gemm_k<GM_PLAIN>, grid, dim3(256), 0, stream, g); break;
        case GM_EXP1: hipLaunchKernelGGL(gemm_k<GM_EXP1>, grid, dim3(256), 0, stream, g); break;
        case GM_EXP2: hipLaunchKernelGGL(gemm_k<GM_EXP2>, grid, dim3(256), 0, stream, g); break;
        case GM_COMB: hipLaunchKernelGGL(gemm_k<GM_COMB>, grid, dim3(256), 0, stream, g); break;
        case GM_ENC: hipLaunchKernelGGL(gemm_k<GM_ENC>, grid, dim3(256), 0, stream, g); break;
        default: mc_set_error("bad gemm mode %d", mode); return MC_ERR_ARG;
    }
    MC_LAUNCH_CHECK();
    return MC_OK;
}

int mc_device_cus() {
    static int v = 0;
    if (v <= 0) {
        int dev = 0;
        hipDeviceProp_t prop;
        if (hipGetDevice(&dev) == hipSuccess && hipGetDeviceProperties(&prop, dev) == hipSuccess) v = prop.multiProcessorCount;
        if (v <= 0) v = 256;
    }
    return v;
}

static int tail2_grid(const TailArgs& g, int tune, int* per_wave_out) {
    const int ncb = cdiv(g.N, 16);
    const long nblocks = (long)cdiv(g.M, 16) * ncb;
    if (!(tune & kTuneTail2) || !g.C2 || ncb > T2_MAXCB || g.K < 3 * T2_BK || g.K % T2_BK) return 0;
    int G = mc_device_cus();
    if (nblocks < (long)G * 16) G = (int)(nblocks / 16) > 0 ? (int)(nblocks / 16) : 1;
    else G *= (int)cdiv(nblocks, (long)G * 66);
    const int nmax = (int)cdiv(nblocks, (long)G);
    const int per_wave = cdiv(nmax, 4);
    const int max_rt = (ncb - 1 + nmax - 1) / ncb + 1;
    if (per_wave > 17 || max_rt > T2_MAXRT) return 0;
    if (per_wave_out) *per_wave_out = per_wave;
    return G;
}

bool mc_gemm_tail_two_outputs(const TailArgs& g) { return tail2_grid(g, g.tune, nullptr) > 0; }

static int tail_kernels_scratch_free() {
    static const int verdict = [] {
        const void* fns[] = {(const void*)gemm_tail_k<3>, (const void*)gemm_tail2_k<4>, (const void*)gemm_tail2_k<8>, (const void*)gemm_tail2_k<12>,
                             (const void*)gemm_tail2_k<16>};
        for (const void* f : fns) {
            hipFuncAttributes at;
            if (hipFuncGetAttributes(&at, f) != hipSuccess) return -1;
            if (at.localSizeBytes != 0) return (int)at.localSizeBytes;
        }
        return 0;
    }();
    return verdict;
}

int mc_launch_gemm_tail(const TailArgs& g, hipStream_t stream) {
    MC_REQUIRE(g.H && g.Af && g.W && g.bias && g.C && g.tune >= 0, "gemm_tail: null operand or unset tune bits");
    MC_REQUIRE(tail_kernels_scratch_free() == 0,
               "gemm_tail: a tail kernel of this build uses scratch memory (%d bytes per lane; -1 = attributes unreadable): its hand-counted vmcnt "
               "waits are invalid -- rebuild with the toolchain the kernels were counted for", tail_kernels_scratch_free());
    MC_REQUIRE(g.K % BK == 0 && g.K >= BK && g.lda % 4 == 0 && g.ldw % 4 == 0 && g.half % 4 == 0 && g.w_gstride % 4 == 0,
               "gemm_tail: unsupported shape (M=%d N=%d K=%d)", g.M, g.N, g.K);
    if (g.M <= 0 || g.N <= 0) return MC_OK;
    MC_REQUIRE((long)g.N * g.ldw * 4 < (1L << 32), "gemm_tail: weight beyond 4 GB");
    TailArgs gg = g;
    int per_wave = 0;
    if (const int G = tail2_grid(gg, gg.tune, &per_wave)) {
        const int ncb = cdiv(g.N, 16);
        const long nblocks = (long)cdiv(g.M, 16) * ncb;
        dim3 grid(2 * G);
        MC_LEDGER("gemm_tail2_k", grid, 2.0 * g.M * g.N * g.K * 2);
        if (per_wave <= 5) hipLaunchKernelGGL((gemm_tail2_k<4>), grid, dim3(256), 0, stream, gg, ncb, nblocks);
        else if (per_wave <= 9) hipLaunchKernelGGL((gemm_tail2_k<8>), grid, dim3(256), 0, stream, gg, ncb, nblocks);
        else if (per_wave <= 13) hipLaunchKernelGGL((gemm_tail2_k<12>), grid, dim3(256), 0, stream, gg, ncb, nblocks);
        else hipLaunchKernelGGL((gemm_tail2_k<16>), grid, dim3(256), 0, stream, gg, ncb, nblocks);
        MC_LAUNCH_CHECK();
        return MC_OK;
    }
    dim3 grid(cdiv(g.M, SM) * cdiv(g.N, 48));
    MC_LEDGER("gemm_tail_k", grid, 2.0 * g.M * g.N * g.K * 2);
    hipLaunchKernelGGL((gemm_tail_k<3>), grid, dim3(256), 0, stream, gg);
    MC_LAUNCH_CHECK();
    return MC_OK;
}
```

### motioncraft_amd/csrc/mc_model.hip

```cpp
#include "mc_ctx.h"

namespace {

template <class T>
int ws_alloc(mc_ctx* c, T** p, size_t n) {
    void* d = nullptr;
    size_t bytes = (n * sizeof(T) + 255) & ~(size_t)255;
    if (bytes == 0) bytes = 256;
    MC_HIP(hipMalloc(&d, bytes));
    c->allocs.push_back(d);
    c->bytes += (int64_t)bytes;
    *p = (T*)d;
    return MC_OK;
}

int bind_moe(const mc_model* m, const std::string& pre, int din, int dout, int seq_rows, MoeW* w) {
    const int64_t E = m->cfg.num_experts;
    w->din = din;
    w->dout = dout;
    return m->params.bind({{&w->emb, pre + "emb", (int64_t)seq_rows * din},       {&w->gate_w, pre + "gate_w", 256 * din},
                           {&w->gate_b, pre + "gate_b", 256},                      {&w->sim_n, pre + "sim_n", 256 * E},
                           {&w->sim_nT, pre + "sim_nT", 32 * 256},                 {&w->scale, pre + "scale", 1},
                           {&w->fc1_w, pre + "fc1_w", E * 4 * din * din},          {&w->fc1_b, pre + "fc1_b", E * 4 * din},
                           {&w->fc2_wt, pre + "fc2_wt", E * din * 4 * din},        {&w->fc2_b, pre + "fc2_b", E * din},
                           {&w->proj_w, pre + "proj_w", (int64_t)dout * din},      {&w->proj_b, pre + "proj_b", dout}});
}

int bind_weights(mc_ctx* c) {
    const mc_model* m = c->m;
    const ParamStore& ps = m->params;
    const mc_model_config& g = m->cfg;
    const int L = g.latent_dim, H = g.num_parts, D = L * H, F = g.ffn_dim, Te = g.time_embed_dim, C = g.input_feats;
    const int64_t DD = (int64_t)D * D;
    int r;
    if ((r = ps.bind({{&c->enc_w, "enc.w", (int64_t)D * m->Cp},                 {&c->enc_b, "enc.b", D},
                      {&c->seq_emb, "seq_emb", (int64_t)g.max_seq_len * D},
                      {&c->time_w0, "time.w0", (int64_t)Te * D},                {&c->time_b0, "time.b0", Te},
                      {&c->time_w2, "time.w2", (int64_t)Te * Te},               {&c->time_b2, "time.b2", Te},
                      {&c->dec_w, "dec.w", (int64_t)C * D},                     {&c->dec_b, "dec.b", C}})))
        return r;
    if (ps.has("dec.wf") && ps.has("dec.bf")) {
        if ((r = ps.bind({{&c->dec_wf, "dec.wf", (int64_t)C * D}, {&c->dec_bf, "dec.bf", C}}))) return r;
    }
    c->NLA = g.num_layers + g.num_ctrl_layers;
    c->lw.resize(c->NLA);
    if (g.num_ctrl_layers > 0) {
        const int64_t n = (int64_t)D * ((g.ctrl_cond_feats + 3) / 4 * 4);
        if ((r = ps.bind({{&c->ctrl_in_w, "ctrl_in.w", n}, {&c->ctrl_in_b, "ctrl_in.b", D}}))) return r;
    }
    for (int i = 0; i < c->NLA; ++i) {
        LayerW& w = c->lw[i];
        const bool is_ctrl = i >= g.num_layers;
        const std::string p = (is_ctrl ? "c" + std::to_string(i - g.num_layers) : "l" + std::to_string(i)) + ".";
        if (is_ctrl) {
            if (i == g.num_layers && (r = ps.bind({{&w.before_w, p + "before_w", DD}, {&w.before_b, p + "before_b", D}}))) return r;
            if ((r = ps.bind({{&w.after_w, p + "after_w", DD}, {&w.after_b, p + "after_b", D}}))) return r;
        }
        if ((r = ps.bind({{&w.norm_g, p + "norm.g", L},                         {&w.norm_b, p + "norm.b", L},
                          {&w.tnorm_g, p + "text_norm.g", g.text_latent_dim},   {&w.tnorm_b, p + "text_norm.b", g.text_latent_dim},
                          {&w.wsm, p + "body_wsm", H * H}})))
            return r;
        if ((r = bind_moe(m, p + "mm.", L, 4 * L, g.max_seq_len * H, &w.mm))) return r;
        if ((r = bind_moe(m, p + "tm.", g.text_latent_dim, 2 * L, g.max_text_len, &w.tm))) return r;
        if ((r = ps.bind({{&w.dyn_g, p + "dyn.norm.g", L},                      {&w.dyn_b, p + "dyn.norm.b", L},
                          {&w.qkv_w, p + "dyn.qkv_w", 3 * L * L},               {&w.qkv_b, p + "dyn.qkv_b", 3 * L},
                          {&w.ca_film_w, p + "ca.film_w", (int64_t)2 * D * Te}, {&w.ca_film_b, p + "ca.film_b", 2 * D},
                          {&w.ca_ln_g, p + "ca.ln_g", D},                       {&w.ca_ln_b, p + "ca.ln_b", D},
                          {&w.ca_out_w, p + "ca.out_w", DD},                    {&w.ca_out_b, p + "ca.out_b", D},
                          {&w.ffn_w1, p + "ffn.w1", (int64_t)H * F * L},        {&w.ffn_b1, p + "ffn.b1", H * F},
                          {&w.ffn_w2, p + "ffn.w2", (int64_t)H * L * F},        {&w.ffn_b2, p + "ffn.b2", H * L},
                          {&w.ffn_film_w, p + "ffn.film_w", (int64_t)2 * D * Te}, {&w.ffn_film_b, p + "ffn.film_b", 2 * D},
                          {&w.ffn_ln_g, p + "ffn.ln_g", D},                     {&w.ffn_ln_b, p + "ffn.ln_b", D},
                          {&w.ffn_out_w, p + "ffn.out_w", DD},                  {&w.ffn_out_b, p + "ffn.out_b", D}})))
            return r;
    }
    return MC_OK;
}

int build_ctx_weights(mc_ctx* c) {
    if (!c->dec_wf) return MC_OK;
    const mc_model_config& g = c->m->cfg;
    const int D = g.latent_dim * g.num_parts;
    const size_t wn = (size_t)g.input_feats * D, bn = (size_t)g.input_feats;
    int rr;
    if ((rr = ws_alloc(c, &c->dec_cat_w, 2 * wn)) != MC_OK || (rr = ws_alloc(c, &c->dec_cat_b, 2 * bn)) != MC_OK) return rr;
    MC_HIP(hipMemcpy(c->dec_cat_w, c->dec_w, wn * sizeof(float), hipMemcpyDeviceToDevice));
    MC_HIP(hipMemcpy(c->dec_cat_w + wn, c->dec_wf, wn * sizeof(float), hipMemcpyDeviceToDevice));
    MC_HIP(hipMemcpy(c->dec_cat_b, c->dec_bf, bn * sizeof(float), hipMemcpyDeviceToDevice));
    MC_HIP(hipMemset(c->dec_cat_b + bn, 0, bn * sizeof(float)));
    return MC_OK;
}

int half_weight(mc_model* m, const std::string& name, long rows, int K, bool chain, HalfW* out) {
    std::lock_guard<std::mutex> lock(m->half_mu);
    auto it = m->half.find(name);
    if (it != m->half.end()) { *out = it->second; return MC_OK; }
    const float* src = nullptr;
    int r = m->params.get(name, (int64_t)rows * K, &src);
    if (r != MC_OK) return r;
    mc_half* hi = nullptr;
    MC_HIP(hipMalloc((void**)&hi, sizeof(mc_half) * 2 * (size_t)rows * K));
    mc_half* lo = hi + (size_t)rows * K;
    r = chain ? mc_launch_split_f16_chainperm(src, hi, lo, rows, K, nullptr) : mc_launch_split_f16(src, hi, lo, rows * K, nullptr);
    if (r != MC_OK) { (void)hipFree(hi); return r; }
    MC_HIP(hipStreamSynchronize(nullptr));
    const HalfW h{hi, lo};
    m->half[name] = h;
    m->half_bytes += sizeof(mc_half) * 2 * (size_t)rows * K;
    *out = h;
    return MC_OK;
}

int bind_half_weights(mc_ctx* c) {
    mc_model* m = c->m;
    const mc_model_config& g = m->cfg;
    const int L = g.latent_dim, H = g.num_parts, D = L * H, F = g.ffn_dim, E = g.num_experts;
    int r;
    for (int i = 0; i < c->NLA; ++i) {
        LayerW& w = c->lw[i];
        const bool is_ctrl = i >= g.num_layers;
        const std::string p = (is_ctrl ? "c" + std::to_string(i - g.num_layers) : "l" + std::to_string(i)) + ".";
        if (D % 128 == 0) {
            if ((r = half_weight(m, p + "ca.out_w", D, D, false, &w.h_ca_out))) return r;
            if ((r = half_weight(m, p + "ffn.out_w", D, D, false, &w.h_ffn_out))) return r;
            if (is_ctrl && (r = half_weight(m, p + "after_w", D, D, false, &w.h_after))) return r;
        }
        if (mc_mlp_h_supported(L, 4 * L)) {
            if ((r = half_weight(m, p + "mm.proj_w", 4 * L, L, false, &w.h_proj))) return r;
            if ((r = half_weight(m, p + "dyn.qkv_w", 3 * L, L, true, &w.h_qkv))) return r;
            if ((r = half_weight(m, p + "mm.fc1_w", (long)E * 4 * L, L, false, &w.h_fc1))) return r;
            if ((r = half_weight(m, p + "mm.fc2_wt", (long)E * L, 4 * L, true, &w.h_fc2))) return r;
        }
        if (mc_mlp_h_supported(L, F)) {
            if ((r = half_weight(m, p + "ffn.w1", (long)H * F, L, false, &w.h_w1))) return r;
            if ((r = half_weight(m, p + "ffn.w2", (long)H * L, F, true, &w.h_w2))) return r;
        }
    }
    return MC_OK;
}

int coop_grid_needed(const mc_ctx* c) {
    int nwg = 0;
    for (long n : {c->N, c->Ntxt})
        if (!mc_route_is_small(c->opt, n) && mc_route_coop_wgs(n) > nwg) nwg = mc_route_coop_wgs(n);
    return nwg;
}

struct OptionDef {
    const char *key, *env, *env_alt;
    long McOptions::*field;
    long dflt;
    std::string (*check)(long v);
    int (*hook)(mc_ctx* c, long& v);
};

std::string check_chain(long v) {
    const long bad = v & ~kChainDefault;
    const int b = bad ? __builtin_ctzl((unsigned long)bad) : 0;
    return !bad ? "" : "chain bit " + std::to_string(b) + (b < kChainBits ? " is retired (DESIGN.md section 5)" : " is not defined");
}
std::string check_tune(long v) {
    const long bad = v & ~(long)kTuneBits;
    return !bad ? "" : v < 0 ? "gemm_tune: a bit mask (>= 0)" : "gemm_tune bit " + std::to_string(__builtin_ctzl(bad)) + " is not defined";
}
int chain_hook(mc_ctx* c, long& v) {
    const int L = c->m->cfg.latent_dim;
    c->hbuf_floats = ((v >> kChainMlp) & 1) && mc_mlp_supported(L, 4 * L) ? c->hbuf_cap : 0;
    return MC_OK;
}
int route_coop_hook(mc_ctx* c, long& v) {
    if (!v) {
        if (c->coop_reserved) { mc_route_coop_release(c->device, c->coop_reserved); c->coop_reserved = 0; }
    } else if (!c->opt.route_coop) {
        const int nwg = coop_grid_needed(c);
        MC_REQUIRE(nwg == 0 || mc_route_coop_reserve(c->device, nwg), "route_coop: the cooperative routing grid cannot be reserved on this device");
        c->coop_reserved = nwg;
        v = nwg > 0;
    }
    return MC_OK;
}

const OptionDef kOptions[] = {
    {"chain", "MC_CHAIN", nullptr, &McOptions::chain, kChainDefault, check_chain, chain_hook},
    {"small_gemm_rows", "MC_SMALL_GEMM_ROWS", nullptr, &McOptions::small_gemm_rows, 5600},
    {"split_rows_expert", "MC_SPLIT_ROWS_EXPERT", nullptr, &McOptions::split_rows_expert, 2048},
    {"split_rows_sffn", "MC_SPLIT_ROWS_SFFN", nullptr, &McOptions::split_rows_sffn, 8192},
    {"temporal_split", "MC_TEMPORAL_SPLIT", nullptr, &McOptions::temporal_split, 96},
    {"big_tokens", "MC_BIG_TOKENS", nullptr, &McOptions::big_tokens, 65536},
    {"rowchain_split", "MC_ROWCHAIN_SPLIT", nullptr, &McOptions::rowchain_split, 20480},
    {"gemm_tune", "MC_GEMM_TUNE", nullptr, &McOptions::gemm_tune, kTuneDefault, check_tune},
    {"small_tile_n", "MC_SMALL_TILE_N", nullptr, &McOptions::small_tile_n, 0,
     [](long v) -> std::string { return v == 0 || v == 48 || v == 64 || v == 96 ? "" : "small_tile_n: 0 (per-launch choice), 48, 64 or 96"; }},
    {"gemm_wp_grid", "MC_GEMM_WP_GRID", nullptr, &McOptions::gemm_wp_grid, 512},
    {"half_min_rows", "MC_HALF_MIN_ROWS", nullptr, &McOptions::half_min_rows, 512},
    {"gate_small", "MC_GATE_SMALL", nullptr, &McOptions::gate_small, 12000},
    {"split_expert", "MC_SPLIT_EXPERT", nullptr, &McOptions::split_expert, 0},
    {"split_sffn", "MC_SPLIT_SFFN", nullptr, &McOptions::split_sffn, 0},
    {"route_reg", "MC_ROUTE_REG", nullptr, &McOptions::route_reg, 1},
    {"route_coop", "MC_ROUTE_COOP", nullptr, &McOptions::route_coop, 1, nullptr, route_coop_hook},
    {"route_small", "MC_ROUTE_SMALL_CTX", "MC_ROUTE_SMALL", &McOptions::route_small, 20480,
     [](long v) -> std::string { return v >= 0 && v <= 131072 ? "" : "route_small: 0 .. 131072 pairs (the one-workgroup kernels hold at most 131072)"; }},
    {"route_early", "MC_ROUTE_EARLY", nullptr, &McOptions::route_early, 1,
     [](long v) -> std::string { return v == 0 || v == 1 ? "" : "route_early: 0 or 1"; }},
    {"route_per", nullptr, nullptr, &McOptions::route_per, 0,
     [](long v) -> std::string { return v == 0 || v == 10 || v == 16 ? "" : "route_per: 0 (default), 10 or 16"; }},
    {"dbg_delay_us", nullptr, nullptr, &McOptions::dbg_delay_us, 0,
     [](long v) -> std::string { return v >= -100000 && v <= 100000 ? "" : "dbg_delay_us: -100000 .. 100000"; }},
};

int seed_options(McOptions& o) {
    for (const OptionDef& d : kOptions) {
        const char *var = nullptr, *e = nullptr;
        for (const char* v : {d.env, d.env_alt})
            if (v && !e && (e = getenv(v))) var = v;
        const std::string why = e && d.check ? d.check(atol(e)) : "";
        MC_REQUIRE(why.empty(), "%s=%s: %s", var, e, why.c_str());
        o.*d.field = e ? atol(e) : d.dflt;
    }
    return MC_OK;
}

}

const McOptions* mc_process_options() {
    static McOptions o;
    static const std::string err = seed_options(o) == MC_OK ? "" : mc_last_error();
    if (!err.empty()) mc_set_error("%s", err.c_str());
    return err.empty() ? &o : nullptr;
}

extern "C" {

int mc_device_count(int* n) {
    MC_HIP(hipGetDeviceCount(n));
    return MC_OK;
}
int mc_set_device(int dev) {
    MC_HIP(hipSetDevice(dev));
    return MC_OK;
}

int mc_model_create(const mc_model_config* cfg, mc_model** out) {
    MC_REQUIRE(cfg && out, "null argument");
    MC_REQUIRE(cfg->latent_dim == 32 || cfg->latent_dim == 64 || cfg->latent_dim == 128,
               "latent_dim=%d unsupported (32, 64, 128)", cfg->latent_dim);
    MC_REQUIRE(cfg->topk == 2, "topk=%d unsupported (reference configs use 2)", cfg->topk);
    MC_REQUIRE(cfg->num_experts >= 2 && cfg->num_experts <= 16, "num_experts=%d unsupported", cfg->num_experts);
    MC_REQUIRE(cfg->latent_dim % cfg->dyn_heads == 0, "latent_dim %% dyn_heads != 0");
    MC_REQUIRE(cfg->num_ctrl_layers >= 0 && cfg->num_ctrl_layers < cfg->num_layers, "copy_blocks_num=%d must be in [0, num_layers)", cfg->num_ctrl_layers);
    MC_REQUIRE(cfg->num_ctrl_layers == 0 || cfg->ctrl_cond_feats >= 1, "ctrl_cond_feats must be >= 1");
    MC_REQUIRE(cfg->ffn_dim % 4 == 0 && cfg->time_embed_dim % 4 == 0 && cfg->text_latent_dim % 4 == 0, "dims must be multiples of 4");
    {
        const int q = cfg->text_latent_dim / 4;
        MC_REQUIRE(q >= 1 && q <= 64 && (q & (q - 1)) == 0, "text_latent_dim=%d unsupported", cfg->text_latent_dim);
    }
    mc_model* m = new mc_model();
    m->cfg = *cfg;
    m->Cp = (cfg->input_feats + 31) / 32 * 32;
    *out = m;
    return MC_OK;
}

void mc_model_destroy(mc_model* m) {
    if (!m) return;
    for (auto& kv : m->half) (void)hipFree(const_cast<mc_half*>(kv.second.hi));
    delete m;
}

int mc_model_set_param(mc_model* m, const char* name, const float* host, int64_t numel) {
    MC_REQUIRE(m && name && host && numel > 0, "bad argument");
    MC_REQUIRE(!m->finalized || !m->params.has(name), "mc_model_set_param(%s): the model is finalized; weights are immutable from then on", name);
    return m->params.set(name, host, numel);
}

int mc_model_finalize(mc_model* m) {
    MC_REQUIRE(m, "null model");
    mc_ctx probe;
    probe.m = m;
    int r = bind_weights(&probe);
    if (r != MC_OK) return r;
    m->finalized = true;
    return MC_OK;
}

int mc_ctx_create(mc_model* m, int32_t batch, int32_t frames, int32_t max_steps, mc_ctx** out) {
    MC_REQUIRE(m && out, "null argument");
    MC_REQUIRE(m->finalized, "model not finalized");
    MC_REQUIRE(batch >= 1 && frames >= 1 && frames <= m->cfg.max_seq_len, "bad batch/frames (%d, %d)", batch, frames);
    MC_REQUIRE(max_steps >= 1, "max_steps < 1");
    const mc_model_config& g = m->cfg;
    mc_ctx* c = new mc_ctx();
    if (int r = seed_options(c->opt)) { mc_ctx_destroy(c); return r; }
    if (m->cfg.latent_dim == 64 && !getenv("MC_ROUTE_EARLY")) c->opt.route_early = 0;
    c->m = m;
    c->B = batch;
    c->T = frames;
    c->maxS = max_steps;
    const int L = g.latent_dim, H = g.num_parts, D = L * H, F = g.ffn_dim, Te = g.time_embed_dim, Dt = g.text_latent_dim;
    const long B2 = 2L * batch;
    c->rows = B2 * frames;
    c->N = c->rows * H;
    c->Ntxt = B2 * g.max_text_len;
    int r = bind_weights(c);
    if (r == MC_OK) r = build_ctx_weights(c);
    if (r != MC_OK) { mc_ctx_destroy(c); return r; }
    bool cand_ok = true;
    for (int k = 0; k < mc_ctx::SIDE_CAND; ++k) cand_ok = cand_ok && hipStreamCreateWithFlags(&c->side_cand[k], hipStreamNonBlocking) == hipSuccess;
    c->side = c->side_cand[0];
    for (hipEvent_t* e : {&c->ev_fork, &c->ev_join, &c->ev_side, &c->ev_stag, &c->ev_gate1, &c->ev_sel, &c->ev_front}) cand_ok = cand_ok && hipEventCreateWithFlags(e, hipEventDisableTiming) == hipSuccess;
    if (!cand_ok) {
        mc_set_error("could not create the side stream / events");
        mc_ctx_destroy(c);
        return MC_ERR_HIP;
    }
    const long Nmax = c->N > c->Ntxt ? c->N : c->Ntxt;
    const size_t zsz = (size_t)(c->N * L > c->Ntxt * Dt ? c->N * L : c->Ntxt * Dt);
    const size_t hsz = (size_t)(2 * c->N * 4 * L > 2 * c->Ntxt * 4 * Dt ? 2 * c->N * 4 * L : 2 * c->Ntxt * 4 * Dt);
#define WS(p, n) do { if ((r = ws_alloc(c, &(p), (size_t)(n))) != MC_OK) { mc_ctx_destroy(c); return r; } } while (0)
    WS(c->h, c->rows * D);
    WS(c->z, zsz);
    WS(c->proj, Nmax * 256);
    WS(c->hbuf, hsz);
    c->hbuf_cap = hsz;
    if (chain_on(c, kChainMlp) && mc_mlp_supported(L, 4 * L)) c->hbuf_floats = hsz;
    WS(c->y2, 2 * zsz);
    WS(c->mf, (c->N + 128) * 4 * L);
    WS(c->qkv, (c->N + 128) * 3 * L);
    WS(c->ys, c->rows * D);
    WS(c->yt, c->rows * D);
    WS(c->a, c->rows * D);
    WS(c->z2, c->rows * D);
    WS(c->fh, c->rows * H * F);
    WS(c->out2, c->rows * g.input_feats);
    WS(c->xpad, (long)batch * frames * m->Cp);
    WS(c->xfn, c->Ntxt * Dt);
    WS(c->mask_own, (long)batch * frames);
    WS(c->tf, (long)c->NLA * c->Ntxt * 2 * L);
    WS(c->t_orig, max_steps);
    WS(c->te, (long)max_steps * D);
    WS(c->e1, (long)max_steps * Te);
    WS(c->emb, (long)max_steps * Te);
    WS(c->semb, (long)max_steps * Te);
    WS(c->ss, (long)c->NLA * 2 * max_steps * 2 * D);
    if (g.num_ctrl_layers > 0) {
        WS(c->hc, c->rows * D);
        WS(c->cb, c->rows * D);
        WS(c->cenc, (long)batch * frames * D);
    }
    WS(c->rb.idx, 2 * Nmax);
    WS(c->rb.gate, 2 * Nmax);
    WS(c->rb.key, Nmax);
    WS(c->rb.comb_w, 2 * Nmax);
    WS(c->rb.src_row, 2 * Nmax);
    WS(c->rb.dst_row, 2 * Nmax);
    c->rb.max_tiles = cdiv(2 * Nmax, 128) + g.num_experts;
    WS(c->rb.tile_group, 2 * c->rb.max_tiles);
    WS(c->rb.tile_row0, 2 * c->rb.max_tiles);
    WS(c->rb.tile_nrows, 2 * c->rb.max_tiles);
    WS(c->rb.state, mc_route_state_ints(g.num_experts));
    MC_HIP(hipMemset(c->rb.state + mc_route_barrier_offset(), 0, mc_route_barrier_ints() * sizeof(int)));
    MC_HIP(hipGetDevice(&c->device));
    if (c->opt.route_coop) {
        const int nwg = coop_grid_needed(c);
        if (nwg > 0 && mc_route_coop_reserve(c->device, nwg)) c->coop_reserved = nwg;
        else c->opt.route_coop = 0;
    }
#undef WS
    *out = c;
    return MC_OK;
}

static void graph_release(mc_ctx* c) {
    if (c->graph_exec) { (void)hipGraphExecDestroy(c->graph_exec); c->graph_exec = nullptr; }
    if (c->graph) { (void)hipGraphDestroy(c->graph); c->graph = nullptr; }
    c->graph_steps = 0;
    c->graph_multistep = false;
    c->graph_k1.clear();
}
static void prof_clear(mc_ctx* c) {
    for (auto& p : c->prof) { if (p.e0) (void)hipEventDestroy(p.e0); if (p.e1) (void)hipEventDestroy(p.e1); }
    c->prof.clear();
}

void mc_ctx_destroy(mc_ctx* c) {
    if (!c) return;
    graph_release(c);
    if (c->coop_reserved) { mc_route_coop_release(c->device, c->coop_reserved); c->coop_reserved = 0; }
    prof_clear(c);
    for (int k = 0; k < mc_ctx::SIDE_CAND; ++k)
        if (c->side_cand[k]) { (void)hipStreamSynchronize(c->side_cand[k]); (void)hipStreamDestroy(c->side_cand[k]); }
    for (hipEvent_t e : {c->ev_fork, c->ev_join, c->ev_side, c->ev_stag, c->ev_gate1, c->ev_sel, c->ev_front})
        if (e) (void)hipEventDestroy(e);
    for (void* p : c->allocs) (void)hipFree(p);
    delete c;
}

int64_t mc_ctx_workspace_bytes(const mc_ctx* c) { return c ? (int64_t)(c->bytes + (c->prec != MC_PREC_F32 ? c->m->half_bytes : 0)) : 0; }

int mc_ctx_check(mc_ctx* c, void* stream) {
    MC_REQUIRE(c, "null context");
    int flag = 0;
    MC_HIP(hipMemcpyAsync(&flag, c->rb.state + mc_route_error_offset(), sizeof(int), hipMemcpyDeviceToHost, (hipStream_t)stream));
    MC_HIP(hipStreamSynchronize((hipStream_t)stream));
    if (flag != 0) {
        mc_set_error("the cooperative routing kernel's grid barrier timed out (its workgroups were not all resident: another process "
                     "is holding the GPU with barrier kernels of its own); the results of this context are invalid -- destroy it and "
                     "create the context with MC_ROUTE_COOP=0");
        return MC_ERR_STATE;
    }
    return MC_OK;
}

int mc_ctx_effective_precision(const mc_ctx* c) { return c ? (use_half(c) ? c->prec : MC_PREC_F32) : MC_PREC_F32; }

int mc_ctx_uses_coop_routing(const mc_ctx* c) { return c && c->opt.route_coop && c->coop_reserved > 0 ? 1 : 0; }

int mc_ctx_profile(mc_ctx* c, int32_t on) {
    MC_REQUIRE(c, "null context");
    MC_REQUIRE(!c->graph_mode, "profiling inside a graph capture");
    prof_clear(c);
    c->prof_on = on != 0;
    return MC_OK;
}

int mc_ctx_profile_read(mc_ctx* c, int64_t rows_filter, double* avg_us, int32_t* count, double* gflop_per_launch) {
    MC_REQUIRE(c && avg_us && count && gflop_per_launch, "null argument");
    const int D = c->m->cfg.latent_dim * c->m->cfg.num_parts;
    double sum = 0.0, rows = 0.0;
    int n = 0;
    for (auto& p : c->prof) {
        MC_HIP(hipEventSynchronize(p.e1));
        if (rows_filter > 0 && p.rows != rows_filter) continue;
        float ms = 0.f;
// ... 264 lines not shown
    MC_REQUIRE(c && c->graph_exec, "no captured graph (mc_ctx_graph_capture)");
    MC_REQUIRE(step >= 0 && step < c->graph_steps, "step_index %d outside the %d captured steps", step, c->graph_steps);
    hipStream_t s = (hipStream_t)stream;
    int r;
    if (c->graph_multistep && (r = hist_require(c, c->graph_k1[step], step))) return r;
    if ((r = mc_launch_set_int(c->gstep, step, s))) return r;
    MC_HIP(hipGraphLaunch(c->graph_exec, s));
    if (c->graph_multistep) c->hist_valid = true;
    return MC_OK;
}

int mc_ctx_graph_release(mc_ctx* c) {
    MC_REQUIRE(c, "null context");
    graph_release(c);
    return MC_OK;
}

int mc_sample_step_seeded(mc_ctx* c, float* x_t, int32_t step, const mc_step_coefs* k, const float* noise,
                          const mc_seed* sd, float* x_prev, float* x0, void* stream) {
    MC_REQUIRE(c && x_t && k && noise && x_prev && sd, "null argument");
    MC_REQUIRE(!is_multistep(k), "mc_sample_step_seeded: the multistep sampler (mode 2) has no pre_seq / transl_req seeding");
    MC_REQUIRE(sd->pre_len >= 0 && sd->pre_len <= c->T, "pre_seq has %d frames, the window %d", sd->pre_len, c->T);
    MC_REQUIRE(sd->num_transl >= 0 && sd->num_transl <= MC_MAX_TRANSL, "num_transl=%d outside [0, %d]", sd->num_transl, MC_MAX_TRANSL);
    MC_REQUIRE(sd->num_transl == 0 || c->T >= 2, "transl_req seeds frames 0 and 1: the window has %d", c->T);
    SeedArgs a;
    a.pre = sd->pre_seq_dev; a.pre_noise = sd->pre_noise_dev; a.pre_len = sd->pre_len; a.T = c->T;
    a.sqrt_ab = sd->sqrt_ab; a.sqrt_1mab = sd->sqrt_1mab; a.num_transl = sd->num_transl;
    for (int i = 0; i < sd->num_transl; ++i) {
        MC_REQUIRE(sd->transl_channel[i] >= 0 && sd->transl_channel[i] < c->m->cfg.input_feats, "transl_req channel %d", sd->transl_channel[i]);
        a.transl_channel[i] = sd->transl_channel[i];
        a.transl_value[i][0] = sd->transl_value[i][0];
        a.transl_value[i][1] = sd->transl_value[i][1];
    }
    X0Parts p;
    if (int r = denoise_combined(c, x_t, step, k, stream, &p, &a)) return r;
    const long n = (long)c->B * c->T * c->m->cfg.input_feats;
    return mc_launch_sampler_update(x_t, p.a, p.second(), noise, x_prev, x0, n, p.coefs(k), (hipStream_t)stream);
}

int mc_sample_step_inpaint(mc_ctx* c, const float* x_t, int32_t step, const mc_step_coefs* k, const float* noise,
                           const mc_inpaint* ip, float* x_prev, float* x0, void* stream) {
    MC_REQUIRE(c && x_t && k && noise && x_prev && ip, "null argument");
    MC_REQUIRE(!is_multistep(k), "mc_sample_step_inpaint: the multistep sampler (mode 2) has no outpainting (RePaint) form");
    X0Parts p;
    if (int r = denoise_combined(c, x_t, step, k, stream, &p)) return r;
    const int C = c->m->cfg.input_feats;
    const long n = (long)c->B * c->T * C;
    InpaintArgs a;
    a.gt = ip->gt_dev; a.keep = ip->keep_dev; a.gt_noise = ip->gt_noise_dev; a.blend_w = ip->blend_w_dev;
    a.blend_len = ip->blend_len; a.T = c->T; a.C = C;
    MC_REQUIRE(a.blend_len >= 0 && a.blend_len <= c->T, "blend_len %d outside the %d-frame window", a.blend_len, c->T);
    return mc_launch_sampler_inpaint(x_t, p.a, p.second(), noise, a, x_prev, x0, n, p.coefs(k), (hipStream_t)stream);
}

int mc_postprocess_smplx(const float* pred, const int32_t* lengths, const double* mean, const double* stdv,
                         const double* taps, const int32_t radius[4], int32_t stats_f32, int32_t B, int32_t T, int32_t C,
                         double* poses, double* expr, double* trans, void* stream) {
    MC_REQUIRE(pred && mean && stdv && taps && radius && poses && expr && trans, "null argument");
    static_assert(MC_POST_MAXTAP == 129, "header / kernel tap table size");
    MC_REQUIRE(mc_smplx_post_maxtap() == MC_POST_MAXTAP, "tap table size mismatch");
    return mc_launch_smplx_post(pred, lengths, nullptr, mean, stdv, taps, radius, stats_f32, B, T, C, poses, expr, trans,
                                (hipStream_t)stream);
}

int mc_postprocess_smplx_stitched(const float* pred, const int32_t* rows, int32_t n_frames, const double* mean,
                                  const double* stdv, const double* taps, const int32_t radius[4], int32_t stats_f32,
                                  int32_t C, double* poses, double* expr, double* trans, void* stream) {
    MC_REQUIRE(pred && rows && mean && stdv && taps && radius && poses && expr && trans && n_frames >= 0, "bad argument");
    MC_REQUIRE(mc_smplx_post_maxtap() == MC_POST_MAXTAP, "tap table size mismatch");
    return mc_launch_smplx_post(pred, nullptr, rows, mean, stdv, taps, radius, stats_f32, 1, n_frames, C, poses, expr,
                                trans, (hipStream_t)stream);
}

int mc_postprocess_t2m_joints(const float* pred, const int32_t* lengths, const double* mean, const double* stdv,
                              const double* taps, int32_t radius, int32_t stats_f32, int32_t B, int32_t T, int32_t C,
                              int32_t joints_num, float* joints, void* stream) {
    MC_REQUIRE(pred && mean && stdv && joints && (taps || radius < 0), "null argument");
    MC_REQUIRE(mc_smplx_post_maxtap() == MC_POST_MAXTAP, "tap table size mismatch");
    return mc_launch_t2m_joints(pred, lengths, nullptr, mean, stdv, taps, radius, stats_f32, B, T, C, joints_num, nullptr,
                                joints, (hipStream_t)stream);
}

int mc_postprocess_t2m_joints_stitched(const float* pred, const int32_t* rows, int32_t n_frames, const double* mean,
                                       const double* stdv, const double* taps, int32_t radius, int32_t stats_f32,
                                       int32_t C, int32_t joints_num, double* work, float* joints, void* stream) {
    MC_REQUIRE(pred && rows && mean && stdv && work && joints && (taps || radius < 0) && n_frames >= 0, "bad argument");
    MC_REQUIRE(mc_smplx_post_maxtap() == MC_POST_MAXTAP, "tap table size mismatch");
    return mc_launch_t2m_joints(pred, nullptr, rows, mean, stdv, taps, radius, stats_f32, 1, n_frames, C, joints_num, work,
                                joints, (hipStream_t)stream);
}

int mc_op_renoise(const float* x, const float* noise, float a, float b, float* out, int64_t n, void* stream) {
    MC_REQUIRE(x && noise && out && n >= 0, "bad argument");
    return mc_launch_axpby(x, noise, a, b, out, (long)n, (hipStream_t)stream);
}

int mc_ctx_get_buffer(mc_ctx* c, const char* name, int32_t layer, void** dev_ptr, int64_t* numel) {
    MC_REQUIRE(c && name && dev_ptr && numel, "null argument");
    const mc_model_config& g = c->m->cfg;
    const int L = g.latent_dim, H = g.num_parts, D = L * H;
    const std::string n(name);
    void* p = nullptr;
    int64_t cnt = 0;
    if (n == "h") { p = c->h; cnt = c->rows * D; }
    else if (n == "z") { p = c->z; cnt = c->N * L; }
    else if (n == "proj") { p = c->proj; cnt = c->N * 256; }
    else if (n == "mf") { p = c->mf; cnt = c->N * 4 * L; }
    else if (n == "qkv") { p = c->qkv; cnt = c->N * 3 * L; }
    else if (n == "y2") { p = c->y2; cnt = c->N * 2 * L; }
    else if (n == "ys") { p = c->ys; cnt = c->rows * D; }
    else if (n == "yt") { p = c->yt; cnt = c->rows * D; }
    else if (n == "a") {
        MC_REQUIRE(!a_holds_planes(c), "buffer 'a' holds fp16 planes in a reduced-precision context (clear chain bit 17 to read fp32 rows)");
        p = c->a; cnt = c->rows * D;
    }
    else if (n == "a_tail") { p = deferred_a(c); cnt = c->rows * D; }
    else if (n == "z2") { p = c->z2; cnt = c->rows * D; }
    else if (n == "out2") { p = c->out2; cnt = c->rows * g.input_feats; }
    else if (n == "emb") { p = c->emb; cnt = (int64_t)c->S * g.time_embed_dim; }
    else if (n == "ss") { p = c->ss + (long)layer * c->maxS * 2 * D; cnt = (int64_t)c->S * 2 * D; }
    else if (n == "tf") { p = c->tf + (long)layer * c->Ntxt * 2 * L; cnt = c->Ntxt * 2 * L; }
    else if (n == "idx") { p = c->rb.idx; cnt = 2 * c->N; }
    else if (n == "gate") { p = c->rb.gate; cnt = 2 * c->N; }
    else if (n == "comb_w") { p = c->rb.comb_w; cnt = 2 * c->N; }
    else if (n == "key") { p = c->rb.key; cnt = c->N; }
    else if (n == "hc" && c->hc) { p = c->hc; cnt = c->rows * D; }
    else if (n == "cb" && c->cb) { p = c->cb; cnt = c->rows * D; }
    else if (n == "cap_idx" && c->cap_idx) { p = c->cap_idx + (long)layer * 2 * c->N; cnt = 2 * c->N; }
    else if (n == "cap_w" && c->cap_w) { p = c->cap_w + (long)layer * 2 * c->N; cnt = 2 * c->N; }
    else if (n == "x0_hist") {
        if (!c->x0_hist) { mc_set_error("buffer 'x0_hist' does not exist before the context's first multistep (mode 2) call"); return MC_ERR_STATE; }
        p = c->x0_hist; cnt = (int64_t)c->B * c->T * g.input_feats;
    }
    else if (n == "src_row") { p = c->rb.src_row; cnt = 2 * c->N; }
    else if (n == "dst_row") { p = c->rb.dst_row; cnt = 2 * c->N; }
    else if (n == "tile_group") { p = c->rb.tile_group; cnt = 2L * c->rb.max_tiles; }
    else if (n == "tile_row0") { p = c->rb.tile_row0; cnt = 2L * c->rb.max_tiles; }
    else if (n == "tile_nrows") { p = c->rb.tile_nrows; cnt = 2L * c->rb.max_tiles; }
    else if (n == "num_tiles") { p = const_cast<int*>(mc_route_num_tiles_ptr(c->rb, 0)); cnt = 2; }
    else if (n == "route_split") { p = const_cast<int*>(mc_route_split_flag_ptr(c->rb)); cnt = 1; }
    else { mc_set_error("unknown buffer '%s'", name); return MC_ERR_ARG; }
    *dev_ptr = p;
    *numel = cnt;
    return MC_OK;
}

int mc_op_gemm(const float* a, const float* w, const float* bias, const float* res, float* cdev, int32_t M, int32_t N,
               int32_t K, int32_t ldw, int32_t act, void* stream) {
    MC_REQUIRE(a && w && cdev && M > 0 && N > 0 && K > 0 && K % 4 == 0 && ldw % 4 == 0 && ldw >= K, "bad gemm args");
    return dense(nullptr, a, K, w, ldw, bias, res, N, cdev, N, M, N, K, act, (hipStream_t)stream);
}

int mc_op_gemm_strided(int32_t mode, int32_t groups, const mc_gemm_strided* a, void* stream) {
    MC_REQUIRE(a && (mode == GM_PLAIN || mode == GM_ENC) && groups >= 1, "gemm_strided: mode %d (0 plain, 4 encoder), groups %d", mode, groups);
    MC_REQUIRE(a->a_dev && a->w_dev && a->c_dev && a->M > 0 && a->N > 0 && a->K > 0 && a->lda > 0 && a->ldc >= a->N && a->ldw >= a->K &&
                   a->ldw % 4 == 0 && a->add_mod >= 1 && a->dup_rows >= 0 && (!a->res_dev || a->ldr >= a->N) && (!a->add_dev || a->ld_add >= a->N),
               "bad gemm_strided args");
    GemmArgs g;
    g.A = a->a_dev; g.lda = a->lda; g.a_gstride = a->a_gstride;
    g.W = a->w_dev; g.ldw = a->ldw; g.w_gstride = a->w_gstride;
    g.bias = a->bias_dev; g.b_gstride = a->b_gstride;
    g.C = a->c_dev; g.ldc = a->ldc; g.c_gstride = a->c_gstride;
    g.R = a->res_dev; g.ldr = a->ldr; g.r_gstride = a->r_gstride;
    g.act = a->act; g.act_after_res = a->act_after_res;
    g.add = a->add_dev; g.add_mod = a->add_mod; g.ld_add = a->ld_add; g.dup_rows = a->dup_rows;
    g.M = a->M; g.N = a->N; g.K = a->K;
    return mc_launch_gemm(mode, g, groups, 0, (hipStream_t)stream);
}

static int gemm_f16_op(GemmHArgs g, const float* w, const float* bias, const float* res, float* cdev, int M, int N, int K, bool split, hipStream_t s) {
    mc_half* planes = nullptr;
    MC_HIP(hipMalloc((void**)&planes, sizeof(mc_half) * 2 * (size_t)N * K));
    int r = mc_launch_split_f16(w, planes, planes + (size_t)N * K, (long)N * K, s);
    if (r == MC_OK) {
        g.Wh = planes; g.Wl = planes + (size_t)N * K; g.bias = bias; g.R = res; g.ldr = N; g.C = cdev; g.ldc = N;
        g.M = M; g.N = N; g.K = K;
        r = mc_launch_gemm_h(g, split, s);
    }
    (void)hipStreamSynchronize(s);
    (void)hipFree(planes);
    return r;
}

int mc_op_gemm_f16(const float* a, const float* w, const float* bias, const float* res, float* cdev, int32_t M, int32_t N,
                   int32_t K, int32_t split, void* stream) {
    MC_REQUIRE(a && w && cdev && M > 0 && N > 0 && K > 0, "bad gemm args");
    GemmHArgs g;
    g.A = a; g.lda = K;
    return gemm_f16_op(g, w, bias, res, cdev, M, N, K, split != 0, (hipStream_t)stream);
}

int mc_op_gemm_f16_planes(const void* a_hi, const void* a_lo, const float* w, const float* bias, const float* res, float* cdev, int32_t M,
                          int32_t N, int32_t K, int32_t split, int32_t pre, int32_t frag_major, void* stream) {
    MC_REQUIRE(a_hi && (!split || a_lo) && w && cdev && M > 0 && N > 0 && K > 0, "bad gemm args");
    GemmHArgs g;
    g.Ah = (const mc_half*)a_hi; g.Al = (const mc_half*)a_lo; g.a_fm = frag_major != 0; g.pre = pre != 0;
    return gemm_f16_op(g, w, bias, res, cdev, M, N, K, split != 0, (hipStream_t)stream);
}

int mc_op_gemm_tail(const float* h, const float* a, const float* w, const float* bias, float* cdev, float* c2dev, int32_t M, int32_t N,
                    int32_t K, float wc, float wu, int32_t variant, void* stream) {
    MC_REQUIRE(h && a && w && bias && cdev && M > 0 && N > 0 && K > 0 && K % 32 == 0, "bad gemm_tail args");
    MC_REQUIRE(variant >= 0 && variant <= 2, "gemm_tail variant %d (0 default, 1 column tiles, 2 block ranges)", variant);
    TailArgs t;
    t.H = h; t.Af = a; t.half = (long)M * K; t.lda = K; t.W = w; t.ldw = K; t.w_gstride = (long)N * K; t.bias = bias; t.b_gstride = N;
    t.C = cdev; t.ldc = N; t.M = M; t.N = N; t.K = K; t.wc = wc; t.wu = wu;
    const McOptions* o = mc_process_options();
    if (!o) return MC_ERR_ARG;
    t.tune = (int)o->gemm_tune;
    if (variant) t.tune = variant == 1 ? (t.tune & ~kTuneTail2) : (t.tune | kTuneTail2);
    t.C2 = c2dev;
    MC_REQUIRE(variant != 2 || c2dev, "gemm_tail variant 2 needs the scratch output c2_dev [M][N]");
    MC_REQUIRE(variant != 2 || mc_gemm_tail_two_outputs(t),
               "gemm_tail variant 2: the block-range form is not eligible for M=%d N=%d K=%d (N <= 336, K %% 16 == 0, K >= 48, <= 17 blocks per wave)", M, N, K);
    int r = mc_launch_gemm_tail(t, (hipStream_t)stream);
    if (r == MC_OK && mc_gemm_tail_two_outputs(t))
        r = mc_launch_axpby(cdev, c2dev, 1.f, 1.f, cdev, (long)M * N, (hipStream_t)stream);
    return r;
}

int mc_op_ln_rows(const float* x, int64_t ldx, const float* gamma, const float* beta, const float* add, int32_t add_mod,
                  float* y, int64_t rows, int32_t L, void* stream) {
    return mc_launch_ln_rows(x, ldx, 0, gamma, beta, add, add_mod, y, L, rows, L, (hipStream_t)stream);
}

int mc_op_body_attention(const float* mf, int64_t ldmf, const float* qkv, const float* wsm, float* ys, int64_t frames, int32_t H, int32_t L,
                         int64_t twin_from, const int32_t* split_flag, int64_t frame0, void* stream) {
    MC_REQUIRE(mf && qkv && wsm && ys && frames >= 0 && ldmf >= L && twin_from >= 0 && frame0 >= 0, "bad body_attention args");
    TwinAlias alias;
    alias.split_flag = split_flag;
    alias.from = twin_from;
    return mc_launch_body(mf, ldmf, qkv, wsm, ys, frames, H, L, 8, (hipStream_t)stream, alias, frame0);
}

int mc_op_temporal_attention(const float* mf, const float* tf, const float* mask, float* yt, int32_t b0, int32_t nb, int32_t B, int32_t T,
                             int32_t Nt, int32_t H, int32_t L, int32_t form, int32_t skip_text, const int32_t* twin_flag, void* stream) {
    MC_REQUIRE(mf && tf && mask && yt && B > 0 && T > 0 && Nt > 0 && H > 0 && b0 >= 0 && nb >= 0 && b0 + nb <= 2 * B,
               "bad temporal_attention args");
    MC_REQUIRE(L == 32 || L == 64 || L == 128, "temporal_attention: latent_dim=%d unsupported (32, 64, 128)", L);
    hipStream_t s = (hipStream_t)stream;
    const bool sk = skip_text != 0;
    switch (form) {
    case MC_TEMPORAL_STEP: {
        const McOptions* o = mc_process_options();
        if (!o) return MC_ERR_ARG;
        return mc_launch_temporal(mf, tf, mask, yt, b0, nb, B, T, Nt, H, L, s, twin_flag, o->temporal_split, (o->chain >> kChainTemporalPair) & 1, sk);
    }
    case MC_TEMPORAL_WHOLE:
        return mc_launch_temporal(mf, tf, mask, yt, b0, nb, B, T, Nt, H, L, s, twin_flag, -1, false, sk);
    case MC_TEMPORAL_LSPLIT:
        MC_REQUIRE(L >= 64, "temporal_attention form LSPLIT: no column-sliced kernel at latent_dim=%d (64, 128)", L);
        return mc_launch_temporal(mf, tf, mask, yt, b0, nb, B, T, Nt, H, L, s, twin_flag, (long)nb * H, false, sk);
    case MC_TEMPORAL_PAIR:
        MC_REQUIRE(L == 64 && H % 2 == 0, "temporal_attention form PAIR: no two-part kernel at latent_dim=%d, num_parts=%d (64, even)", L, H);
        return mc_launch_temporal(mf, tf, mask, yt, b0, nb, B, T, Nt, H, L, s, twin_flag, -1, true, sk);
    case MC_TEMPORAL_F16X3:
    case MC_TEMPORAL_F16:
        MC_REQUIRE(L >= 64, "temporal_attention form %s: no fp16 kernel at latent_dim=%d (64, 128)", form == MC_TEMPORAL_F16X3 ? "F16X3" : "F16", L);
        return mc_launch_temporal_h(mf, tf, mask, yt, b0, nb, B, T, Nt, H, L, form == MC_TEMPORAL_F16X3, s, twin_flag, sk);
    }
    mc_set_error("temporal_attention: form %d (0 step, 1 WHOLE, 2 LSPLIT, 3 PAIR, 4 F16X3, 5 F16)", form);
    return MC_ERR_ARG;
}

int mc_op_sampler_update(const float* x_t, const float* ot, const float* on, const float* noise, float* x_prev, float* x0,
                         int64_t n, const mc_step_coefs* k, void* stream) {
    MC_REQUIRE(x_t && ot && on && noise && x_prev && k, "null argument");
    return mc_launch_sampler_update(x_t, ot, on, noise, x_prev, x0, n, to_coefs(k), (hipStream_t)stream);
}

int mc_op_sampler_multistep(const float* x_t, const float* ot, const float* on, float* x0_hist, float* x_prev, float* x0, int64_t n,
                            const mc_step_coefs* k, void* stream) {
    MC_REQUIRE(x_t && ot && on && x0_hist && x_prev && k && n >= 0, "bad argument");
    MC_REQUIRE(is_multistep(k), "mc_op_sampler_multistep: coefficients of mode %d (MC_SAMPLER_MULTISTEP = 2 expected)", k->mode);
    return mc_launch_sampler_multistep(x_t, ot, on, x0_hist, x_prev, x0, n, to_coefs(k), (hipStream_t)stream);
}

}
```

### motioncraft_amd/csrc/mc_options.h

```cpp
#pragma once

enum ChainBit {
    kChainMlp = 0,
    kChainGate = 1,
    kChainRowchain = 2,
    kChainTwin = 4,
    kChainTwoStreams = 5,
    kChainGroupExperts = 6,
    kChainDeferTail = 7,
    kChainTwinAlias = 8,
    kChainCtrlGroups = 9,
    kChainProjQkv = 10,
    kChainTailGrouped = 11,
    kChainSffnPartials = 12,
    kChainDynSlices = 13,
    kChainSideBody = 14,
    kChainPqBody = 15,
    kChainTwinSplit = 16,
    kChainFilmPlanes = 17,
    kChainMlpDma = 18,
    kChainPadX = 19,
    kChainTemporalHalf = 20,
    kChainTailOnePass = 21,
    kChainTemporalPair = 22,
    kChainSkipText = 24,
    kChainStagger = 26,
    kChainResidualPre = 27,
    kChainFragMajor = 29,
    kChainBits = 30,
};
constexpr long kChainRetired = 1L << 3 | 1L << 23 | 1L << 25 | 1L << 28;
constexpr long kChainDefault = ((1L << kChainBits) - 1) & ~kChainRetired;
static_assert(kChainDefault == 763363319, "the default chain mask is public ABI");

struct McOptions {
    long chain, small_gemm_rows, split_rows_expert, split_rows_sffn, temporal_split, big_tokens, rowchain_split;
    long gemm_tune, small_tile_n, gemm_wp_grid, half_min_rows, gate_small, split_expert, split_sffn;
    long route_reg, route_coop, route_small, route_early, route_per, dbg_delay_us;
};

const McOptions* mc_process_options();
```

### motioncraft_amd/csrc/mc_step.hip

```cpp
#include "mc_ctx.h"

bool use_half(const mc_ctx* c) { return c->prec != MC_PREC_F32 && c->rows > c->opt.half_min_rows; }
static const HalfW* half_planes(const mc_ctx* c, const HalfW* hw) { return hw && hw->hi && use_half(c) ? hw : nullptr; }
static bool split3(const mc_ctx* c) { return c->prec == MC_PREC_F16X3; }

static bool twin_aliased(const mc_ctx* c, bool twin) { return twin && chain_on(c, kChainTwinAlias) && !c->no_alias; }
static TwinAlias twin_alias(const mc_ctx* c, bool twin, bool tokens) {
    return twin_aliased(c, twin) ? TwinAlias{mc_route_split_flag_ptr(c->rb), (tokens ? c->N : c->rows) / 2} : TwinAlias();
}

template <class Args>
static void set_tile_map(const mc_ctx* c, int group, Args& a) {
    const long to = (long)group * c->rb.max_tiles;
    a.tile_group = c->rb.tile_group + to; a.tile_row0 = c->rb.tile_row0 + to; a.tile_nrows = c->rb.tile_nrows + to;
    a.num_tiles = mc_route_num_tiles_ptr(c->rb, group);
}

static int dbg_hold(const mc_ctx* c, hipStream_t pos, hipStream_t neg) {
    const long us = c->opt.dbg_delay_us;
    return us == 0 ? MC_OK : mc_launch_spin((us > 0 ? us : -us) * 100, us > 0 ? pos : neg);
}

int dense(const mc_ctx* c, const float* A, long lda, const float* W, long ldw, const float* bias, const float* R, long ldr,
          float* C, long ldc, long M, int N, int K, int act, hipStream_t s) {
// ... 386 lines not shown
    const int L = g.latent_dim, H = g.num_parts;
    const LayerW& w = c->lw[i];
    int r;
    const bool fused_gate = chain_on(c, kChainGate) && mc_mlp_supported(L, 32);
    const bool twin = twin_ok && fused_gate && chain_on(c, kChainRowchain) && chain_on(c, kChainTwin) && (c->N % 2 == 0) &&
                      c->rb.tie_xor == 0xFFFFFFFFu;
    const long half = (long)c->B * c->T;
    const long sub_rows = ((long)c->B / 2) * c->T;
    const bool twin_split = twin && split == 2 && chain_on(c, kChainGroupExperts) && chain_on(c, kChainTwinAlias) && chain_on(c, kChainTwinSplit) && !c->no_alias && sub_rows > 0;
    const bool grouped = split == 2 && chain_on(c, kChainGroupExperts);
    const long gsplit = twin_split ? sub_rows * H : grouped ? half * H : c->N;
    const bool early = fused_gate && grouped && c->opt.route_early != 0 && !mc_route_is_small(c->opt, c->N);
    if (fused_gate) {
        GateArgs ga;
        ga.X = hs; ga.ldx = L; ga.gamma = w.norm_g; ga.beta = w.norm_b; ga.emb = w.mm.emb; ga.emb_mod = c->T * H;
        ga.Z = c->z; ga.Wp = w.mm.gate_w; ga.bp = w.mm.gate_b; ga.sim_nT = w.mm.sim_nT; ga.logit_scale = w.mm.scale;
        ga.E = g.num_experts; ga.L = L; ga.small_tokens = c->opt.gate_small;
        ga.idx = c->rb.idx; ga.gate = c->rb.gate; ga.key = c->rb.key; ga.cnt = c->rb.state;
        if (early) {
            const bool two = !twin || twin_split;
            const long nsrc = twin ? c->N / 2 : c->N;
            const int E = g.num_experts;
            if (!(c->cnt_clean && c->early_clean) && (r = mc_route_early_reset(c->rb, s))) return r;
            c->cnt_clean = c->early_clean = false;
            c->led_nsrc = nsrc;
            c->led_gsplit = gsplit;
            if (two && (r = side_fork(c, s))) return r;
            ga.zero_cnt = 0;
            ga.tok0 = 0; ga.N = gsplit; ga.cnt = mc_route_group_counts(c->rb, 0);
            if ((r = mc_launch_gate(ga, s))) return r;
            if ((r = mc_launch_route_fill_group(0, 0, gsplit, E, c->rb, s))) return r;
            if ((r = moe_experts(c, w.mm, c->z, c->N, 0, s, &w.h_fc1, &w.h_fc2))) return r;
            if (two) {
                ga.tok0 = gsplit; ga.N = nsrc; ga.cnt = mc_route_group_counts(c->rb, 1);
                if ((r = mc_launch_gate(ga, c->side))) return r;
                if ((r = mc_launch_route_fill_group(1, gsplit, nsrc - gsplit, E, c->rb, c->side))) return r;
                MC_HIP(hipEventRecord(c->ev_gate1, c->side));
                if ((r = moe_experts(c, w.mm, c->z, c->N, 1, c->side, &w.h_fc1, &w.h_fc2))) return r;
                MC_HIP(hipStreamWaitEvent(s, c->ev_gate1, 0));
            } else if ((r = mc_launch_route_fill_group(1, gsplit, 0, E, c->rb, s))) return r;
            if ((r = mc_launch_route(c->N, nsrc, gsplit, E, moe_capacity(g, c->N), c->rb, c->opt, s, true))) return r;
            c->cnt_clean = c->early_clean = true;
            MC_HIP(hipEventRecord(c->ev_sel, s));
            if (two) MC_HIP(hipStreamWaitEvent(c->side, c->ev_sel, 0));
        } else if (split == 2 && (!twin || twin_split)) {
            if (!c->cnt_clean) MC_HIP(hipMemsetAsync(ga.cnt, 0, sizeof(int) * 32, s));
            c->cnt_clean = false;
            if ((r = side_fork(c, s))) return r;
            ga.zero_cnt = 0;
            const long cut = twin_split ? sub_rows * H : half * H;
            ga.tok0 = 0; ga.N = cut;
            if ((r = mc_launch_gate(ga, s))) return r;
            ga.tok0 = cut; ga.N = twin_split ? half * H : c->N;
            if ((r = mc_launch_gate(ga, c->side))) return r;
        } else {
            ga.N = twin ? c->N / 2 : c->N;
            ga.zero_cnt = c->cnt_clean ? 0 : 1;
            c->cnt_clean = false;
            if ((r = mc_launch_gate(ga, s))) return r;
        }
        if (split == 2 && !early && (r = side_join(c, s))) return r;
    } else {
        if ((r = mc_launch_ln_rows(hs, L, 0, w.norm_g, w.norm_b, w.mm.emb, c->T * H, c->z, L, c->N, L, s))) return r;
    }
    if (!early && (r = run_moe(c, w.mm, c->z, c->N, nullptr, 0, fused_gate, twin, gsplit, s, &w.h_fc1, &w.h_fc2))) return r;
    if (c->cap_idx) {
        if (twin) {
            MC_HIP(hipMemcpyAsync(c->cap_idx + (long)i * 2 * c->N, c->rb.idx, sizeof(int) * c->N, hipMemcpyDeviceToDevice, s));
            MC_HIP(hipMemcpyAsync(c->cap_idx + (long)i * 2 * c->N + c->N, c->rb.idx, sizeof(int) * c->N, hipMemcpyDeviceToDevice, s));
        } else {
            MC_HIP(hipMemcpyAsync(c->cap_idx + (long)i * 2 * c->N, c->rb.idx, sizeof(int) * 2 * c->N, hipMemcpyDeviceToDevice, s));
        }
        MC_HIP(hipMemcpyAsync(c->cap_w + (long)i * 2 * c->N, c->rb.comb_w, sizeof(float) * 2 * c->N, hipMemcpyDeviceToDevice, s));
    }
    const bool evstag = split == 2 && chain_on(c, kChainStagger) && !use_half(c) && L == 128;
    if (split) {
        if (twin_split) {
            if (!early) {
                if ((r = side_fork(c, s))) return r;
                if ((r = moe_experts(c, w.mm, c->z, c->N, 0, s, &w.h_fc1, &w.h_fc2))) return r;
                if ((r = moe_experts(c, w.mm, c->z, c->N, 1, c->side, &w.h_fc1, &w.h_fc2))) return r;
            }
            auto front = [&](long row0, long nrows, hipStream_t sk) {
                const int e = layer_proj(c, i, twin, row0, nrows, sk);
                return e ? e : layer_body(c, i, twin, row0, nrows, sk);
            };
            if ((r = front(0, sub_rows, s))) return r;
            if ((r = front(sub_rows, half - sub_rows, c->side))) return r;
            MC_HIP(hipEventRecord(c->ev_join, s));
            MC_HIP(hipEventRecord(c->ev_side, c->side));
            MC_HIP(hipStreamWaitEvent(c->side, c->ev_join, 0));
            MC_HIP(hipStreamWaitEvent(s, c->ev_side, 0));
            if ((r = front(half, half, c->side))) return r;
            if (early) MC_HIP(hipEventRecord(c->ev_front, c->side));
            if ((r = layer_temporal(c, i, twin, 0, half, s))) return r;
            if (early) MC_HIP(hipStreamWaitEvent(s, c->ev_front, 0));
            if ((r = layer_temporal(c, i, twin, half, half, c->side))) return r;
        } else {
            if (grouped && twin) {
                if (!early && (r = moe_experts(c, w.mm, c->z, c->N, 0, s, &w.h_fc1, &w.h_fc2))) return r;
                if ((r = side_fork(c, s))) return r;
            } else if (!early) {
                if ((r = side_fork(c, s))) return r;
                if (grouped) {
                    if ((r = moe_experts(c, w.mm, c->z, c->N, 0, s, &w.h_fc1, &w.h_fc2))) return r;
                    if ((r = moe_experts(c, w.mm, c->z, c->N, 1, c->side, &w.h_fc1, &w.h_fc2))) return r;
                }
            }
            if ((r = layer_rows(c, i, twin, 0, half, s, s))) return r;
            if (twin_aliased(c, twin)) {
                MC_HIP(hipEventRecord(c->ev_join, s));
                MC_HIP(hipStreamWaitEvent(c->side, c->ev_join, 0));
            }
            if ((r = layer_rows(c, i, twin, half, half, c->side, c->side))) return r;
            if (early && twin) {
                MC_HIP(hipEventRecord(c->ev_front, c->side));
                MC_HIP(hipStreamWaitEvent(s, c->ev_front, 0));
            }
        }
        if ((r = dbg_hold(c, c->side, s))) return r;
        if ((r = layer_rows_tail(c, i, hs, step, twin, 0, half, s, evstag ? c->ev_stag : nullptr, nullptr))) return r;
        if ((r = layer_rows_tail(c, i, hs, step, twin, half, half, c->side, nullptr, evstag ? c->ev_stag : nullptr))) return r;
        return split == 1 ? side_join(c, s) : MC_OK;
    }
    const bool side_temporal = c->side && c->N <= c->opt.big_tokens;
    if ((r = layer_rows(c, i, twin, 0, 2 * half, s, side_temporal ? c->side : s))) return r;
    return layer_rows_tail(c, i, hs, step, twin, 0, 2 * half, s);
}

int denoise_impl(mc_ctx* c, const float* x_t, int32_t step, float* out2_dev, int32_t stop_after, void* stream, const SeedArgs* seed) {
    MC_REQUIRE(c && x_t, "null argument");
    MC_REQUIRE(c->have_cond, "mc_ctx_set_condition not called");
    MC_REQUIRE(step >= 0 && step < c->S, "step_index %d outside the %d-step schedule", step, c->S);
    if (c->graph_mode) step = 0;
    hipStream_t s = (hipStream_t)stream;
    const mc_model_config& g = c->m->cfg;
    const int L = g.latent_dim, H = g.num_parts, D = L * H, C = g.input_feats;
    const long BT = (long)c->B * c->T;
    int r;
    if ((r = pick_side_stream(c, s))) return r;
    {
        const bool padded = c->xpad_ready && !seed;
        c->xpad_ready = false;
        if (seed) { if ((r = mc_launch_pad_rows_seeded(const_cast<float*>(x_t), c->xpad, BT, C, c->m->Cp, *seed, s))) return r; }
        else if (!padded && (r = mc_launch_pad_rows(x_t, c->xpad, BT, C, c->m->Cp, s))) return r;
        GemmArgs e;
        mc_gemm_opts(c->opt, e);
        e.A = c->xpad; e.lda = c->m->Cp;
        e.W = c->enc_w; e.ldw = c->m->Cp; e.bias = c->enc_b;
        e.add = c->seq_emb; e.add_mod = c->T; e.ld_add = D;
        e.C = c->h; e.ldc = D; e.dup_rows = BT;
        e.M = (int)BT; e.N = D; e.K = c->m->Cp;
        if (BT <= c->opt.small_gemm_rows && D % 64 == 0 && c->m->Cp % 32 == 0) { if ((r = mc_launch_gemm_small(e, s))) return r; }
        else if ((r = mc_launch_gemm(GM_ENC, e, 1, 0, s))) return r;
    }
    const int nl = stop_after >= 0 ? (stop_after < g.num_layers ? stop_after : g.num_layers) : g.num_layers;
    c->no_alias = stop_after >= 0 && stop_after < g.num_layers;
    const int NC = c->have_ctrl ? g.num_ctrl_layers : 0;
    const bool fused = chain_on(c, kChainGate) && chain_on(c, kChainRowchain) && mc_mlp_supported(L, 32);
    const int split = (c->side && chain_on(c, kChainTwoStreams) && c->N > c->opt.big_tokens && fused) ? ((NC > 0 && !chain_on(c, kChainCtrlGroups)) ? 1 : 2) : 0;
    auto by_group = [&](auto&& fn) -> int {
        if (split != 2) return fn(0L, c->rows, s);
        if (int e = fn(0L, BT, s)) return e;
        return fn(BT, BT, c->side);
    };
    for (int i = 0; i < nl; ++i) {
        if (i >= 1 && i <= NC) {
            const int j = i - 1, slot = g.num_layers + j;
            if (j == 0) {
                if ((r = by_group([&](long r0, long n, hipStream_t sk) {
                         return mc_launch_add_rows(c->hc + r0 * D, c->h + r0 * D, c->cb + r0 * D, nullptr, n, D, sk); })))
                    return r;
            }
            if ((r = run_layer(c, slot, c->hc, step, false, split, s))) return r;
            const LayerW& cw = c->lw[slot];
            if ((r = by_group([&](long r0, long n, hipStream_t sk) {
                     if (const HalfW* hp = half_planes(c, &cw.h_after))
                         return dense_h(c, c->hc + r0 * D, *hp, cw.after_b, c->h + r0 * D, c->h + r0 * D, n, D, D, sk);
                     return dense(c, c->hc + r0 * D, D, cw.after_w, D, cw.after_b, c->h + r0 * D, D, c->h + r0 * D, D, n, D, D, ACT_NONE, sk); })))
                return r;
        }
        if ((r = run_layer(c, i, c->h, step, i == 0, split, s))) return r;
    }
    if (split == 2 && (r = side_join(c, s))) return r;
    if (stop_after >= 0) return MC_OK;
    float* o = out2_dev ? out2_dev : c->out2;
    return dense(c, c->h, D, c->dec_w, D, c->dec_b, nullptr, 0, o, C, c->rows, C, D, ACT_NONE, s);
}

SamplerCoefs to_coefs(const mc_step_coefs* k) {
    SamplerCoefs c;
    c.mode = k->mode; c.text_coef = k->text_coef; c.none_coef = k->none_coef; c.c1 = k->c1; c.c2 = k->c2;
    c.log_var = k->log_var; c.sqrt_recip = k->sqrt_recip; c.sqrt_recipm1 = k->sqrt_recipm1; c.ab = k->ab;
    c.ab_prev = k->ab_prev; c.eta = k->eta; c.nonzero = k->nonzero;
    return c;
}

int denoise_combined(mc_ctx* c, const float* x_t, int32_t step, const mc_step_coefs* k, void* stream, X0Parts* x0, const SeedArgs* seed) {
    const mc_model_config& g = c->m->cfg;
    const bool defer = chain_on(c, kChainDeferTail);
    c->defer_last_gemm = defer;
    int r = denoise_impl(c, x_t, step, nullptr, g.num_layers, stream, seed);
    c->defer_last_gemm = false;
    if (r != MC_OK) return r;
    hipStream_t s = (hipStream_t)stream;
    const int D = g.latent_dim * g.num_parts, C = g.input_feats;
    const long BT = (long)c->B * c->T;
    const LayerW& w = c->lw[g.num_layers - 1];
    *x0 = X0Parts{c->out2, nullptr};
    auto combine = [&](const float* x, const float* y, float* out) -> int {
        if (c->graph_mode) return mc_launch_cfg_combine_tab(x, y, c->gcoefs, c->gstep, out, BT * D, s);
        return mc_launch_axpby(x, y, k->text_coef, k->none_coef, out, BT * D, s);
    };
    const bool grouped = defer && c->dec_cat_w && chain_on(c, kChainTailGrouped);
    if (grouped && chain_on(c, kChainTailOnePass) && BT > c->opt.small_gemm_rows && D % 32 == 0) {
        TailArgs t;
        t.H = c->h; t.Af = deferred_a(c); t.half = BT * D; t.lda = D;
        t.W = c->dec_cat_w; t.ldw = D; t.w_gstride = (long)C * D; t.bias = c->dec_cat_b; t.b_gstride = C;
        t.C = c->out2; t.ldc = C; t.M = (int)BT; t.N = C; t.K = D;
        t.wc = k->text_coef; t.wu = k->none_coef;
        if (c->graph_mode) {
            static_assert(sizeof(SamplerCoefs) % sizeof(float) == 0 && offsetof(SamplerCoefs, none_coef) == offsetof(SamplerCoefs, text_coef) + sizeof(float), "SamplerCoefs layout");
            t.coef_table = reinterpret_cast<const float*>(c->gcoefs) + offsetof(SamplerCoefs, text_coef) / sizeof(float);
            t.coef_stride = sizeof(SamplerCoefs) / sizeof(float);
            t.step_ptr = c->gstep;
        }
        t.tune = (int)c->opt.gemm_tune;
        t.C2 = c->out2 + BT * C;
        if ((r = mc_launch_gemm_tail(t, s))) return r;
        if (mc_gemm_tail_two_outputs(t)) x0->b = t.C2;
        return MC_OK;
    }
    if (grouped) {
        if ((r = mc_launch_axpby_pair(c->h, c->h + BT * D, c->z2, deferred_a(c), deferred_a(c) + BT * D, c->z2 + BT * D, k->text_coef, k->none_coef,
                                      c->graph_mode ? c->gcoefs : nullptr, c->graph_mode ? c->gstep : nullptr, BT * D, s))) return r;
        GemmArgs t;
        mc_gemm_opts(c->opt, t);
        t.A = c->z2; t.lda = D; t.a_gstride = BT * D; t.W = c->dec_cat_w; t.ldw = D; t.w_gstride = (long)C * D;
        t.bias = c->dec_cat_b; t.b_gstride = C; t.C = c->out2; t.ldc = C; t.c_gstride = BT * C;
        t.M = (int)BT; t.N = C; t.K = D;
        x0->b = c->out2 + BT * C;
        return D % 32 == 0 ? mc_launch_gemm_small(t, s, 2) : mc_launch_gemm(GM_PLAIN, t, 2, 0, s);
    }
    if ((r = combine(c->h, c->h + BT * D, c->z2))) return r;
    if (defer) {
        float* const ad = deferred_a(c);
        if ((r = combine(ad, ad + BT * D, ad))) return r;
        if (c->dec_wf) {
            if ((r = dense(c, c->z2, D, c->dec_w, D, c->dec_bf, nullptr, 0, c->out2, C, BT, C, D, ACT_NONE, s))) return r;
            return dense(c, ad, D, c->dec_wf, D, nullptr, c->out2, C, c->out2, C, BT, C, D, ACT_NONE, s);
        }
        if ((r = dense(c, ad, D, w.ffn_out_w, D, w.ffn_out_b, c->z2, D, c->z2, D, BT, D, D, ACT_NONE, s))) return r;
    }
    return dense(c, c->z2, D, c->dec_w, D, c->dec_b, nullptr, 0, c->out2, C, BT, C, D, ACT_NONE, s);
}

int sampler_update(mc_ctx* c, const float* x_t, const X0Parts& x0p, const mc_step_coefs* k, const float* noise, float* x_prev, float* x0,
                   hipStream_t s, const RngArgs* rng, const PadOut* pad) {
    const long n = (long)c->B * c->T * c->m->cfg.input_feats;
    const SamplerCoefs* table = c->graph_mode ? c->gcoefs : nullptr;
    const int* step_ptr = c->graph_mode ? c->gstep : nullptr;
    const bool multistep = c->graph_mode ? c->graph_multistep : k->mode == MC_SAMPLER_MULTISTEP;
    if (!multistep) return mc_launch_sampler_update(x_t, x0p.a, x0p.second(), noise, x_prev, x0, n, x0p.coefs(k), s, table, step_ptr, rng, pad);
    MC_REQUIRE(c->x0_hist, "multistep update without a history buffer");
    return mc_launch_sampler_multistep(x_t, x0p.a, x0p.second(), c->x0_hist, x_prev, x0, n, x0p.coefs(k), s, table, step_ptr, pad);
}
```

Before: 666.1.

## Skip all-zero weight K-blocks in encoder GEMM and decoder tail GEMM

```diff
diff --git a/include/motioncraft_amd.h b/include/motioncraft_amd.h
--- a/include/motioncraft_amd.h
+++ b/include/motioncraft_amd.h
@@ -154,7 +154,7 @@
                            int32_t d, int32_t vocab, void* stream);
 int mc_op_enc_attention(const float* qkv_dev, const uint8_t* valid_dev, float* out_dev, int32_t B, int32_t S, int32_t d, int32_t heads,
                         int32_t causal, int32_t form, void* stream);
-enum { MC_GM_PLAIN = 0, MC_GM_ENC = 4 };
+enum { MC_GM_PLAIN = 0, MC_GM_ENC = 4, MC_GM_ENC_DENSE = 5 };
 typedef struct mc_gemm_strided {
     const float* a_dev; int64_t lda, a_gstride;
     const float* w_dev; int64_t ldw, w_gstride;
@@ -165,6 +165,8 @@
     int32_t add_mod, act, act_after_res, M, N, K;
 } mc_gemm_strided;
 int mc_op_gemm_strided(int32_t mode, int32_t groups, const mc_gemm_strided* args, void* stream);
+int mc_op_enc_ktab(const float* w_dev, int32_t N, int32_t K, int64_t ldw, int32_t* ktab_dev, void* stream);
+int mc_op_dec_zmask(const float* w_dev, int32_t N, int32_t K, int64_t ldw, uint32_t* zmask_dev, void* stream);
 int mc_op_bigru_steps(const float* gi_dev, const float* whh_dev, const float* bhh_dev, float* h_dev, const int32_t* lens_dev,
                       int32_t len_div, int32_t B, int32_t S, int32_t H, int32_t s0, int32_t steps, void* stream);
 int mc_op_conv1d_k4s2(const float* x_dev, int64_t ldx, const float* w_tapmajor_dev, const float* bias_dev, float* y_padded_dev, int32_t B,
diff --git a/motioncraft_amd/csrc/mc_ctx.h b/motioncraft_amd/csrc/mc_ctx.h
--- a/motioncraft_amd/csrc/mc_ctx.h
+++ b/motioncraft_amd/csrc/mc_ctx.h
@@ -21,6 +21,7 @@
     size_t half_bytes = 0;
     bool finalized = false;
     int Cp = 0;
+    const int* enc_ktab = nullptr;
 };
 
 struct MoeW {
@@ -50,6 +51,7 @@
     const float *enc_w, *enc_b, *seq_emb, *time_w0, *time_b0, *time_w2, *time_b2, *dec_w, *dec_b;
     const float *dec_wf = nullptr, *dec_bf = nullptr;
     float *dec_cat_w = nullptr, *dec_cat_b = nullptr;
+    unsigned* dec_zmask = nullptr;
     const float *ctrl_in_w = nullptr, *ctrl_in_b = nullptr;
     int NLA = 0;
     float *hc = nullptr, *cb = nullptr, *cenc = nullptr;
diff --git a/motioncraft_amd/csrc/mc_gemm.h b/motioncraft_amd/csrc/mc_gemm.h
--- a/motioncraft_amd/csrc/mc_gemm.h
+++ b/motioncraft_amd/csrc/mc_gemm.h
@@ -66,7 +66,10 @@
 }
 
 int mc_device_cus();
-int mc_launch_gemm(int mode, const GemmArgs& g, int groups, int max_tiles, hipStream_t stream);
+int mc_launch_gemm(int mode, const GemmArgs& g, int groups, int max_tiles, hipStream_t stream, const int* ktab = nullptr);
+
+inline size_t mc_enc_ktab_ints(int N, int K) { return (size_t)(N / 128) * (size_t)(1 + K / 16); }
+int mc_launch_enc_ktab(const float* W, int N, int K, long ldw, int* ktab, hipStream_t stream);
 int mc_launch_gemm_small(const GemmArgs& g, hipStream_t stream, int groups = 1);
 
 struct TailArgs {
@@ -87,5 +90,6 @@
     long coef_stride = 0;
     int tune = -1;
 };
-int mc_launch_gemm_tail(const TailArgs& g, hipStream_t stream);
-bool mc_gemm_tail_two_outputs(const TailArgs& g);
+int mc_launch_gemm_tail(const TailArgs& g, hipStream_t stream, bool two_pass = false, const unsigned* zmask = nullptr);
+bool mc_gemm_tail_two_outputs(const TailArgs& g, bool two_pass = false);
+int mc_launch_dec_zmask(const float* W, int N, int K, long ldw, unsigned* zmask, hipStream_t stream);
diff --git a/motioncraft_amd/csrc/mc_gemm.hip b/motioncraft_amd/csrc/mc_gemm.hip
--- a/motioncraft_amd/csrc/mc_gemm.hip
+++ b/motioncraft_amd/csrc/mc_gemm.hip
@@ -1,5 +1,6 @@
 #include "mc_common.h"
 #include "mc_gemm.h"
+#include <type_traits>
 
 namespace {
 
@@ -358,7 +359,14 @@
 
 constexpr int WBK = 16, WSTAGE = 128 * WBK;
 
-__global__ __launch_bounds__(256, 2) void gemm_wp_k(GemmArgs g) {
+struct GemmListArgs : GemmArgs {
+    const int* ktab;
+    int ktab_ld;
+};
+
+template <class G>
+__global__ __launch_bounds__(256, 2) void gemm_wp_k(G g) {
+    constexpr bool LIST = !std::is_same<G, GemmArgs>::value;
     __shared__ __attribute__((aligned(16))) float smem[4 * 2 * WSTAGE];
     const int tid = threadIdx.x, lane = tid & 63, wave = tid >> 6;
     const int wm = wave >> 1, wn = wave & 1;
@@ -398,6 +406,13 @@
             dma16(voa[q], Ab + kt * WBK, l + q * 1024);
             dma16(vow[q], Wb + kt * WBK, l + 4096 + q * 1024);
         };
+        typedef const int __attribute__((address_space(4))) ktab_t;
+        ktab_t* kl = nullptr;
+        int nkt = nk;
+        if constexpr (LIST) {
+            kl = (ktab_t*)g.ktab + (long)tn * g.ktab_ld + 1;
+            nkt = min(kl[-1], nk);
+        }
         f32x16 acc[2][2];
 #pragma unroll
         for (int mi = 0; mi < 2; ++mi)
@@ -414,20 +429,24 @@
                 acc[1][1] = __builtin_amdgcn_mfma_f32_32x32x2f32(f.b1[i], f.a1[i], acc[1][1], 0, 0, 0);
             }
         };
-#pragma unroll
-        for (int q = 0; q < 4; ++q) issue_q(0, 0, q);
-        asm volatile("s_waitcnt vmcnt(0)" ::: "memory");
+        if (!LIST || nkt > 0) {
+            const int k0 = LIST ? kl[0] : 0;
+#pragma unroll
+            for (int q = 0; q < 4; ++q) issue_q(k0, 0, q);
+            asm volatile("s_waitcnt vmcnt(0)" ::: "memory");
+        }
         Frag f0 = ld_frag(0, 0);
         auto ktile = [&](int kt) {
             const int st = kt & 1;
-            const bool more = kt + 1 < nk;
+            const bool more = kt + 1 < nkt;
+            const int ktn = !LIST ? kt + 1 : more ? kl[kt + 1] : 0;
             Frag f1 = ld_frag(st, 1);
             __builtin_amdgcn_sched_barrier(0);
             mma2(f0, 0);
-            if (more) { issue_q(kt + 1, st ^ 1, 0); issue_q(kt + 1, st ^ 1, 1); }
+            if (more) { issue_q(ktn, st ^ 1, 0); issue_q(ktn, st ^ 1, 1); }
             __builtin_amdgcn_sched_barrier(0);
             mma2(f0, 2);
-            if (more) { issue_q(kt + 1, st ^ 1, 2); issue_q(kt + 1, st ^ 1, 3); }
+            if (more) { issue_q(ktn, st ^ 1, 2); issue_q(ktn, st ^ 1, 3); }
             __builtin_amdgcn_sched_barrier(0);
             mma2(f1, 0);
             if (more) {
@@ -437,7 +456,7 @@
             __builtin_amdgcn_sched_barrier(0);
             mma2(f1, 2);
         };
-        const int npre = nk > 2 ? nk - 2 : 0;
+        const int npre = nkt > 2 ? nkt - 2 : 0;
         for (int kt = 0; kt < npre; ++kt) ktile(kt);
         f32x4 rv[2][2][4], bv[2][4];
 #pragma unroll
@@ -453,7 +472,7 @@
                     if (g.add) rv[mi][ni][q] = *reinterpret_cast<const f32x4*>(g.add + (m % g.add_mod) * g.ld_add + n);
                 }
             }
-        for (int kt = npre; kt < nk; ++kt) ktile(kt);
+        for (int kt = npre; kt < nkt; ++kt) ktile(kt);
 #pragma unroll
         for (int mi = 0; mi < 2; ++mi) {
             float* crow = Cb + (long)(row0 + wm * 64 + mi * 32 + frow) * g.ldc;
@@ -473,6 +492,25 @@
                     if (g.dup_rows) *reinterpret_cast<f32x4*>(crow + g.dup_rows * g.ldc + n) = v;
                 }
         }
+    }
+}
+
+__global__ __launch_bounds__(256) void enc_ktab_k(const float* __restrict__ W, int K, long ldw, int* __restrict__ ktab) {
+    const int nk = K / WBK, tid = threadIdx.x;
+    int* row = ktab + (long)blockIdx.x * (1 + nk);
+    const unsigned* w = reinterpret_cast<const unsigned*>(W) + ((long)blockIdx.x * BN + (tid >> 1)) * ldw + 8 * (tid & 1);
+    for (int kt = 0; kt < nk; ++kt) {
+        unsigned any = 0;
+#pragma unroll
+        for (int i = 0; i < 8; ++i) any |= w[kt * WBK + i] & 0x7fffffffu;
+        const int f = __syncthreads_or(any != 0);
+        if (tid == 0) row[1 + kt] = f;
+    }
+    if (tid == 0) {
+        int n = 0;
+        for (int kt = 0; kt < nk; ++kt)
+            if (row[1 + kt]) row[1 + n++] = kt;
+        row[0] = n;
     }
 }
 
@@ -835,8 +873,13 @@
 
 __device__ __forceinline__ int t2_swz(int row) { return (0x78 >> (2 * ((row >> 2) & 3))) & 3; }
 
-template <int NBW>
-__global__ __launch_bounds__(256, 2) void gemm_tail2_k(TailArgs g, int ncb, long nblocks) {
+struct TailZArgs : TailArgs {
+    const unsigned* zmask;
+};
+
+template <int NBW, class GA>
+__global__ __launch_bounds__(256, 2) void gemm_tail2_k(GA g, int ncb, long nblocks) {
+    constexpr bool ZB = !std::is_same<GA, TailArgs>::value;
     static_assert(NBW % 4 == 0 && NBW >= 4 && NBW <= 16, "NBW");
     constexpr int PH = 4;
     __shared__ __attribute__((aligned(16))) float smem[T2_RING * T2_STAGE];
@@ -844,8 +887,9 @@
     const int qw = __builtin_amdgcn_readfirstlane(tid >> 6);
     float wc = g.wc, wu = g.wu;
     if (g.coef_table) { wc = g.coef_table[(long)*g.step_ptr * g.coef_stride]; wu = g.coef_table[(long)*g.step_ptr * g.coef_stride + 1]; }
-    const int G = gridDim.x >> 1, rid = xcd_remap((int)blockIdx.x, (int)gridDim.x);
-    const int wg = rid >> 1, grp = rid & 1;
+    const int G = ZB ? gridDim.x : gridDim.x >> 1, rid = xcd_remap((int)blockIdx.x, (int)gridDim.x);
+    const int wg = ZB ? rid : rid >> 1;
+    int grp = ZB ? 1 : rid & 1;
     const long gb0 = nblocks * wg / G, gb1 = nblocks * (wg + 1) / G;
     const int n = (int)(gb1 - gb0);
     if (n <= 0) return;
@@ -855,12 +899,14 @@
     const int lfrag = frow * T2_BK + ((kg ^ t2_swz(frow)) << 2);
     const int g0 = (int)(gb0 - (long)rt_first * ncb) + wb0;
     int aoff[NBW + 1], boff[NBW + 1];
+    unsigned cbit[ZB ? NBW + 1 : 1];
     {
         int rt = g0 / ncb, cb = g0 - rt * ncb;
 #pragma unroll
         for (int b = 0; b <= NBW; ++b) {
             aoff[b] = rt * 16 * T2_BK;
             boff[b] = (T2_WROW0 + 16 * cb) * T2_BK;
+            if constexpr (ZB) cbit[b] = 1u << cb;
             if (b + 1 < nb) { if (++cb == ncb) { cb = 0; ++rt; } }
         }
     }
@@ -909,35 +955,66 @@
                 *reinterpret_cast<f32x4*>(St + a_lds[j]) = v;
             }
     };
-    auto w_issue = [&](int kt) {
+    auto w_issue = [&](int kt, unsigned m) {
         const float* Wb = Wsrc + (long)kt * T2_BK;
         const unsigned l = lds_q + (unsigned)((kt % T2_RING) * T2_STAGE + T2_WROW0 * T2_BK) * 4;
 #pragma unroll
         for (int q = 0; q < MAXP; ++q)
-            if (q < nwp) dma16(vow[q], Wb, l + (unsigned)(16 * (qw + 4 * q)) * T2_BK * 4);
-    };
+            if (q < nwp && (!ZB || ((m >> (qw + 4 * q)) & 1))) dma16(vow[q], Wb, l + (unsigned)(16 * (qw + 4 * q)) * T2_BK * 4);
+    };
+    unsigned wbits = 0;
+#pragma unroll
+    for (int q = 0; q < MAXP; ++q)
+        if (ZB && q < nwp) wbits |= 1u << (qw + 4 * q);
+    const unsigned allcb = (1u << ncb) - 1;
+    typedef const unsigned __attribute__((address_space(4))) zmask_t;
+    zmask_t* zm = nullptr;
+    auto mask_of = [&](int kt) -> unsigned { return zm ? zm[kt < nk ? kt : nk - 1] & allcb : allcb; };
+    auto npieces = [&](unsigned m) { return ZB ? __builtin_popcount(m & wbits) : nwp; };
+    unsigned m0 = 0, m1 = 0;
+    f32x4 c0[2], u0[2], c1[2], u1[2];
+    int pass = 0;
+    do {
     f32x4 acc[NBW + 1];
 #pragma unroll
     for (int b = 0; b <= NBW; ++b) acc[b] = f32x4{0.f, 0.f, 0.f, 0.f};
-    f32x4 c0[2], u0[2], c1[2], u1[2];
+    if constexpr (ZB) { m0 = mask_of(0); m1 = mask_of(1); }
     a_load(0, c0, u0);
     vm_wait(0);
     asm volatile("" : "+v"(c0[0]), "+v"(c0[1]), "+v"(u0[0]), "+v"(u0[1]));
     a_store(0, c0, u0);
     a_load(1, c1, u1);
-    w_issue(0);
+    w_issue(0, m0);
     if (nk > 2) a_load(2, c0, u0);
-    if (nk > 1) w_issue(1);
+    if (nk > 1) w_issue(1, m1);
     auto step = [&](int kt, f32x4 (&cs)[2], f32x4 (&us)[2]) {
-        vm_wait((kt + 2 < nk ? na : 0) + (kt + 1 < nk ? nwp : 0));
+        unsigned m2 = 0;
+        if constexpr (ZB) m2 = mask_of(kt + 2);
+        vm_wait((kt + 2 < nk ? na : 0) + (kt + 1 < nk ? npieces(m1) : 0));
         asm volatile("" : "+v"(cs[0]), "+v"(cs[1]), "+v"(us[0]), "+v"(us[1]));
         if (kt + 1 < nk) a_store(kt + 1, cs, us);
         __syncthreads();
         if (kt + 3 < nk) a_load(kt + 3, cs, us);
-        if (kt + 2 < nk) w_issue(kt + 2);
+        if (kt + 2 < nk) w_issue(kt + 2, m2);
         const float* St = smem + (kt % T2_RING) * T2_STAGE + lfrag;
 #pragma unroll
         for (int p0 = 0; p0 < NBW; p0 += PH) {
+            if constexpr (ZB) {
+                bool all = true;
+#pragma unroll
+                for (int b = 0; b < PH; ++b) all = all && (m0 & cbit[p0 + b]);
+                if (!all) {
+#pragma unroll
+                    for (int b = 0; b < PH; ++b)
+                        if (m0 & cbit[p0 + b]) {
+                            const f32x4 fa1 = *reinterpret_cast<const f32x4*>(St + aoff[p0 + b]);
+                            const f32x4 fb1 = *reinterpret_cast<const f32x4*>(St + boff[p0 + b]);
+#pragma unroll
+                            for (int i = 0; i < 4; ++i) acc[p0 + b] = __builtin_amdgcn_mfma_f32_16x16x4f32(fb1[i], fa1[i], acc[p0 + b], 0, 0, 0);
+                        }
+                    continue;
+                }
+            }
             f32x4 fa[PH], fb[PH];
 #pragma unroll
             for (int b = 0; b < PH; ++b) {
@@ -950,12 +1027,13 @@
                 for (int b = 0; b < PH; ++b)
                     acc[p0 + b] = __builtin_amdgcn_mfma_f32_16x16x4f32(fb[b][i], fa[b][i], acc[p0 + b], 0, 0, 0);
         }
-        if (nb > NBW) {
+        if (nb > NBW && (!ZB || (m0 & cbit[ZB ? NBW : 0]))) {
             const f32x4 fa = *reinterpret_cast<const f32x4*>(St + aoff[NBW]);
             const f32x4 fb = *reinterpret_cast<const f32x4*>(St + boff[NBW]);
 #pragma unroll
             for (int i = 0; i < 4; ++i) acc[NBW] = __builtin_amdgcn_mfma_f32_16x16x4f32(fb[i], fa[i], acc[NBW], 0, 0, 0);
         }
+        if constexpr (ZB) { m0 = m1; m1 = m2; }
     };
     for (int kt = 0; kt < nk; kt += 2) {
         step(kt, c1, u1);
@@ -979,6 +1057,11 @@
             }
         }
     }
+    if constexpr (ZB) {
+        grp = 0; Asrc = g.H; Wsrc = g.W; zm = (zmask_t*)g.zmask;
+        __syncthreads();
+    }
+    } while (ZB && ++pass < 2);
 }
 
 }
@@ -1030,7 +1113,14 @@
     return MC_OK;
 }
 
-int mc_launch_gemm(int mode, const GemmArgs& g0, int groups, int max_tiles, hipStream_t stream) {
+int mc_launch_enc_ktab(const float* W, int N, int K, long ldw, int* ktab, hipStream_t stream) {
+    MC_REQUIRE(W && ktab && N > 0 && N % BN == 0 && K > 0 && K % WBK == 0 && ldw >= K, "enc_ktab: N %% 128 == 0 and K %% 16 == 0 (N=%d K=%d ldw=%ld)", N, K, ldw);
+    hipLaunchKernelGGL(enc_ktab_k, dim3(N / BN), dim3(256), 0, stream, W, K, ldw, ktab);
+    MC_LAUNCH_CHECK();
+    return MC_OK;
+}
+
+int mc_launch_gemm(int mode, const GemmArgs& g0, int groups, int max_tiles, hipStream_t stream, const int* ktab) {
     GemmArgs g = g0;
     if (int r = resolve_opts(g)) return r;
     const int ntn = cdiv(g.N, BN);
@@ -1051,7 +1141,14 @@
         if (wp_ok) {
             const int persistent = g.wp_grid > 0 ? g.wp_grid : (int)grid.x;
             MC_LEDGER("gemm_wp_k", dim3(grid.x < persistent ? grid.x : persistent), 2.0 * g.M * g.N * g.K);
-            hipLaunchKernelGGL(gemm_wp_k, dim3(grid.x < persistent ? grid.x : persistent), dim3(256), 0, stream, g);
+            if (ktab && enc_fast) {
+                GemmListArgs gl;
+                static_cast<GemmArgs&>(gl) = g;
+                gl.ktab = ktab; gl.ktab_ld = 1 + g.K / WBK;
+                hipLaunchKernelGGL(gemm_wp_k<GemmListArgs>, dim3(grid.x < persistent ? grid.x : persistent), dim3(256), 0, stream, gl);
+            } else {
+                hipLaunchKernelGGL(gemm_wp_k<GemmArgs>, dim3(grid.x < persistent ? grid.x : persistent), dim3(256), 0, stream, g);
+            }
         } else {
             MC_LEDGER("gemm_dma_k", grid, 2.0 * g.M * g.N * g.K);
             hipLaunchKernelGGL(gemm_dma_k, grid, dim3(256), 0, stream, g);
@@ -1088,27 +1185,28 @@
     return v;
 }
 
-static int tail2_grid(const TailArgs& g, int tune, int* per_wave_out) {
+static int tail2_grid(const TailArgs& g, int tune, int* per_wave_out, bool two_pass) {
     const int ncb = cdiv(g.N, 16);
     const long nblocks = (long)cdiv(g.M, 16) * ncb;
     if (!(tune & kTuneTail2) || !g.C2 || ncb > T2_MAXCB || g.K < 3 * T2_BK || g.K % T2_BK) return 0;
     int G = mc_device_cus();
     if (nblocks < (long)G * 16) G = (int)(nblocks / 16) > 0 ? (int)(nblocks / 16) : 1;
     else G *= (int)cdiv(nblocks, (long)G * 66);
-    const int nmax = (int)cdiv(nblocks, (long)G);
+    const int nmax = (int)cdiv(nblocks, (long)G * (two_pass ? 2 : 1));
     const int per_wave = cdiv(nmax, 4);
     const int max_rt = (ncb - 1 + nmax - 1) / ncb + 1;
-    if (per_wave > 17 || max_rt > T2_MAXRT) return 0;
+    if (per_wave > (two_pass ? 9 : 17) || max_rt > T2_MAXRT) return 0;
     if (per_wave_out) *per_wave_out = per_wave;
     return G;
 }
 
-bool mc_gemm_tail_two_outputs(const TailArgs& g) { return tail2_grid(g, g.tune, nullptr) > 0; }
+bool mc_gemm_tail_two_outputs(const TailArgs& g, bool two_pass) { return tail2_grid(g, g.tune, nullptr, two_pass) > 0; }
 
 static int tail_kernels_scratch_free() {
     static const int verdict = [] {
-        const void* fns[] = {(const void*)gemm_tail_k<3>, (const void*)gemm_tail2_k<4>, (const void*)gemm_tail2_k<8>, (const void*)gemm_tail2_k<12>,
-                             (const void*)gemm_tail2_k<16>};
+        const void* fns[] = {(const void*)gemm_tail_k<3>, (const void*)gemm_tail2_k<4, TailArgs>, (const void*)gemm_tail2_k<8, TailArgs>,
+                             (const void*)gemm_tail2_k<12, TailArgs>, (const void*)gemm_tail2_k<16, TailArgs>,
+                             (const void*)gemm_tail2_k<4, TailZArgs>, (const void*)gemm_tail2_k<8, TailZArgs>};
         for (const void* f : fns) {
             hipFuncAttributes at;
             if (hipFuncGetAttributes(&at, f) != hipSuccess) return -1;
@@ -1119,7 +1217,29 @@
     return verdict;
 }
 
-int mc_launch_gemm_tail(const TailArgs& g, hipStream_t stream) {
+static __global__ __launch_bounds__(256) void dec_zmask_k(const float* __restrict__ W, int N, long ldw, unsigned* __restrict__ zmask) {
+    __shared__ unsigned m;
+    if (threadIdx.x == 0) m = 0;
+    __syncthreads();
+    for (int r = threadIdx.x; r < N; r += 256) {
+        const unsigned* w = reinterpret_cast<const unsigned*>(W) + (long)r * ldw + (long)blockIdx.x * T2_BK;
+        unsigned any = 0;
+#pragma unroll
+        for (int i = 0; i < T2_BK; ++i) any |= w[i] & 0x7fffffffu;
+        if (any) atomicOr(&m, 1u << (r >> 4));
+    }
+    __syncthreads();
+    if (threadIdx.x == 0) zmask[blockIdx.x] = m;
+}
+
+int mc_launch_dec_zmask(const float* W, int N, int K, long ldw, unsigned* zmask, hipStream_t stream) {
+    MC_REQUIRE(W && zmask && N > 0 && N <= 16 * T2_MAXCB && K > 0 && K % T2_BK == 0 && ldw >= K, "dec_zmask: N <= 336 and K %% 16 == 0 (N=%d K=%d ldw=%ld)", N, K, ldw);
+    hipLaunchKernelGGL(dec_zmask_k, dim3(K / T2_BK), dim3(256), 0, stream, W, N, ldw, zmask);
+    MC_LAUNCH_CHECK();
+    return MC_OK;
+}
+
+int mc_launch_gemm_tail(const TailArgs& g, hipStream_t stream, bool two_pass, const unsigned* zmask) {
     MC_REQUIRE(g.H && g.Af && g.W && g.bias && g.C && g.tune >= 0, "gemm_tail: null operand or unset tune bits");
     MC_REQUIRE(tail_kernels_scratch_free() == 0,
                "gemm_tail: a tail kernel of this build uses scratch memory (%d bytes per lane; -1 = attributes unreadable): its hand-counted vmcnt "
@@ -1130,15 +1250,22 @@
     MC_REQUIRE((long)g.N * g.ldw * 4 < (1L << 32), "gemm_tail: weight beyond 4 GB");
     TailArgs gg = g;
     int per_wave = 0;
-    if (const int G = tail2_grid(gg, gg.tune, &per_wave)) {
+    if (const int G = tail2_grid(gg, gg.tune, &per_wave, two_pass)) {
         const int ncb = cdiv(g.N, 16);
         const long nblocks = (long)cdiv(g.M, 16) * ncb;
         dim3 grid(2 * G);
         MC_LEDGER("gemm_tail2_k", grid, 2.0 * g.M * g.N * g.K * 2);
-        if (per_wave <= 5) hipLaunchKernelGGL((gemm_tail2_k<4>), grid, dim3(256), 0, stream, gg, ncb, nblocks);
-        else if (per_wave <= 9) hipLaunchKernelGGL((gemm_tail2_k<8>), grid, dim3(256), 0, stream, gg, ncb, nblocks);
-        else if (per_wave <= 13) hipLaunchKernelGGL((gemm_tail2_k<12>), grid, dim3(256), 0, stream, gg, ncb, nblocks);
-        else hipLaunchKernelGGL((gemm_tail2_k<16>), grid, dim3(256), 0, stream, gg, ncb, nblocks);
+        if (two_pass) {
+            TailZArgs gz;
+            static_cast<TailArgs&>(gz) = gg;
+            gz.zmask = zmask;
+            if (per_wave <= 5) hipLaunchKernelGGL((gemm_tail2_k<4, TailZArgs>), grid, dim3(256), 0, stream, gz, ncb, nblocks);
+            else hipLaunchKernelGGL((gemm_tail2_k<8, TailZArgs>), grid, dim3(256), 0, stream, gz, ncb, nblocks);
+        }
+        else if (per_wave <= 5) hipLaunchKernelGGL((gemm_tail2_k<4, TailArgs>), grid, dim3(256), 0, stream, gg, ncb, nblocks);
+        else if (per_wave <= 9) hipLaunchKernelGGL((gemm_tail2_k<8, TailArgs>), grid, dim3(256), 0, stream, gg, ncb, nblocks);
+        else if (per_wave <= 13) hipLaunchKernelGGL((gemm_tail2_k<12, TailArgs>), grid, dim3(256), 0, stream, gg, ncb, nblocks);
+        else hipLaunchKernelGGL((gemm_tail2_k<16, TailArgs>), grid, dim3(256), 0, stream, gg, ncb, nblocks);
         MC_LAUNCH_CHECK();
         return MC_OK;
     }
diff --git a/motioncraft_amd/csrc/mc_model.hip b/motioncraft_amd/csrc/mc_model.hip
--- a/motioncraft_amd/csrc/mc_model.hip
+++ b/motioncraft_amd/csrc/mc_model.hip
@@ -88,6 +88,11 @@
     MC_HIP(hipMemcpy(c->dec_cat_w + wn, c->dec_wf, wn * sizeof(float), hipMemcpyDeviceToDevice));
     MC_HIP(hipMemcpy(c->dec_cat_b, c->dec_bf, bn * sizeof(float), hipMemcpyDeviceToDevice));
     MC_HIP(hipMemset(c->dec_cat_b + bn, 0, bn * sizeof(float)));
+    if (g.input_feats <= 336 && D % 16 == 0) {
+        if ((rr = ws_alloc(c, &c->dec_zmask, (size_t)D / 16)) != MC_OK) return rr;
+        if ((rr = mc_launch_dec_zmask(c->dec_cat_w, g.input_feats, D, D, c->dec_zmask, nullptr))) return rr;
+        MC_HIP(hipStreamSynchronize(nullptr));
+    }
     return MC_OK;
 }
 
@@ -202,6 +207,8 @@
      [](long v) -> std::string { return v >= 0 && v <= 131072 ? "" : "route_small: 0 .. 131072 pairs (the one-workgroup kernels hold at most 131072)"; }},
     {"route_early", "MC_ROUTE_EARLY", nullptr, &McOptions::route_early, 1,
      [](long v) -> std::string { return v == 0 || v == 1 ? "" : "route_early: 0 or 1"; }},
+    {"zero_blocks", "MC_ZERO_BLOCKS", nullptr, &McOptions::zero_blocks, 1,
+     [](long v) -> std::string { return v >= 0 && v <= 2 ? "" : "zero_blocks: 0, 1 or 2"; }},
     {"route_per", nullptr, nullptr, &McOptions::route_per, 0,
      [](long v) -> std::string { return v == 0 || v == 10 || v == 16 ? "" : "route_per: 0 (default), 10 or 16"; }},
     {"dbg_delay_us", nullptr, nullptr, &McOptions::dbg_delay_us, 0,
@@ -279,6 +286,14 @@
     probe.m = m;
     int r = bind_weights(&probe);
     if (r != MC_OK) return r;
+    const int D = m->cfg.latent_dim * m->cfg.num_parts;
+    if (!m->enc_ktab && D % 128 == 0 && m->Cp % 16 == 0) {
+        float* tab = nullptr;
+        if ((r = m->params.derived(mc_enc_ktab_ints(D, m->Cp), &tab))) return r;
+        if ((r = mc_launch_enc_ktab(probe.enc_w, D, m->Cp, m->Cp, reinterpret_cast<int*>(tab), nullptr))) return r;
+        MC_HIP(hipStreamSynchronize(nullptr));
+        m->enc_ktab = reinterpret_cast<const int*>(tab);
+    }
     m->finalized = true;
     return MC_OK;
 }
@@ -849,7 +864,10 @@
 }
 
 int mc_op_gemm_strided(int32_t mode, int32_t groups, const mc_gemm_strided* a, void* stream) {
-    MC_REQUIRE(a && (mode == GM_PLAIN || mode == GM_ENC) && groups >= 1, "gemm_strided: mode %d (0 plain, 4 encoder), groups %d", mode, groups);
+    MC_REQUIRE(a && (mode == GM_PLAIN || mode == GM_ENC || mode == MC_GM_ENC_DENSE) && groups >= 1,
+               "gemm_strided: mode %d (0 plain, 4 encoder, 5 encoder without the zero-block table), groups %d", mode, groups);
+    const bool dense_walk = mode == MC_GM_ENC_DENSE;
+    if (dense_walk) mode = GM_ENC;
     MC_REQUIRE(a->a_dev && a->w_dev && a->c_dev && a->M > 0 && a->N > 0 && a->K > 0 && a->lda > 0 && a->ldc >= a->N && a->ldw >= a->K &&
                    a->ldw % 4 == 0 && a->add_mod >= 1 && a->dup_rows >= 0 && (!a->res_dev || a->ldr >= a->N) && (!a->add_dev || a->ld_add >= a->N),
                "bad gemm_strided args");
@@ -862,7 +880,25 @@
     g.act = a->act; g.act_after_res = a->act_after_res;
     g.add = a->add_dev; g.add_mod = a->add_mod; g.ld_add = a->ld_add; g.dup_rows = a->dup_rows;
     g.M = a->M; g.N = a->N; g.K = a->K;
-    return mc_launch_gemm(mode, g, groups, 0, (hipStream_t)stream);
+    const McOptions* o = mc_process_options();
+    if (!o) return MC_ERR_ARG;
+    if (mode != GM_ENC || dense_walk || !o->zero_blocks || groups != 1 || a->N % 128 || a->K % 16)
+        return mc_launch_gemm(mode, g, groups, 0, (hipStream_t)stream);
+    int* ktab = nullptr;
+    MC_HIP(hipMalloc((void**)&ktab, mc_enc_ktab_ints(a->N, a->K) * sizeof(int)));
+    int r = mc_launch_enc_ktab(a->w_dev, a->N, a->K, a->ldw, ktab, (hipStream_t)stream);
+    if (r == MC_OK) r = mc_launch_gemm(mode, g, groups, 0, (hipStream_t)stream, ktab);
+    (void)hipStreamSynchronize((hipStream_t)stream);
+    (void)hipFree(ktab);
+    return r;
+}
+
+int mc_op_enc_ktab(const float* w_dev, int32_t N, int32_t K, int64_t ldw, int32_t* ktab_dev, void* stream) {
+    return mc_launch_enc_ktab(w_dev, N, K, (long)ldw, ktab_dev, (hipStream_t)stream);
+}
+
+int mc_op_dec_zmask(const float* w_dev, int32_t N, int32_t K, int64_t ldw, uint32_t* zmask_dev, void* stream) {
+    return mc_launch_dec_zmask(w_dev, N, K, (long)ldw, zmask_dev, (hipStream_t)stream);
 }
 
 static int gemm_f16_op(GemmHArgs g, const float* w, const float* bias, const float* res, float* cdev, int M, int N, int K, bool split, hipStream_t s) {
@@ -898,7 +934,7 @@
 int mc_op_gemm_tail(const float* h, const float* a, const float* w, const float* bias, float* cdev, float* c2dev, int32_t M, int32_t N,
                     int32_t K, float wc, float wu, int32_t variant, void* stream) {
     MC_REQUIRE(h && a && w && bias && cdev && M > 0 && N > 0 && K > 0 && K % 32 == 0, "bad gemm_tail args");
-    MC_REQUIRE(variant >= 0 && variant <= 2, "gemm_tail variant %d (0 default, 1 column tiles, 2 block ranges)", variant);
+    MC_REQUIRE(variant >= 0 && variant <= 4, "gemm_tail variant %d (0 default, 1 column tiles, 2 block ranges, 3 / 4 two-pass block ranges without / with the zero-block masks)", variant);
     TailArgs t;
     t.H = h; t.Af = a; t.half = (long)M * K; t.lda = K; t.W = w; t.ldw = K; t.w_gstride = (long)N * K; t.bias = bias; t.b_gstride = N;
     t.C = cdev; t.ldc = N; t.M = M; t.N = N; t.K = K; t.wc = wc; t.wu = wu;
@@ -907,12 +943,21 @@
     t.tune = (int)o->gemm_tune;
     if (variant) t.tune = variant == 1 ? (t.tune & ~kTuneTail2) : (t.tune | kTuneTail2);
     t.C2 = c2dev;
-    MC_REQUIRE(variant != 2 || c2dev, "gemm_tail variant 2 needs the scratch output c2_dev [M][N]");
-    MC_REQUIRE(variant != 2 || mc_gemm_tail_two_outputs(t),
-               "gemm_tail variant 2: the block-range form is not eligible for M=%d N=%d K=%d (N <= 336, K %% 16 == 0, K >= 48, <= 17 blocks per wave)", M, N, K);
-    int r = mc_launch_gemm_tail(t, (hipStream_t)stream);
-    if (r == MC_OK && mc_gemm_tail_two_outputs(t))
+    const bool two_pass = variant >= 3 || (variant != 1 && o->zero_blocks >= 2 && c2dev && N <= 336 && mc_gemm_tail_two_outputs(t, true));
+    const bool masks = two_pass && variant != 3;
+    MC_REQUIRE(variant < 2 || c2dev, "gemm_tail variant %d needs the scratch output c2_dev [M][N]", variant);
+    MC_REQUIRE(variant < 2 || mc_gemm_tail_two_outputs(t, two_pass),
+               "gemm_tail variant %d: the block-range form is not eligible for M=%d N=%d K=%d (N <= 336, K %% 16 == 0, K >= 48, <= 17 blocks per wave)", variant, M, N, K);
+    unsigned* zmask = nullptr;
+    if (masks) MC_HIP(hipMalloc((void**)&zmask, sizeof(unsigned) * (size_t)(K / 16)));
+    int r = masks ? mc_launch_dec_zmask(w, N, K, K, zmask, (hipStream_t)stream) : MC_OK;
+    if (r == MC_OK) r = mc_launch_gemm_tail(t, (hipStream_t)stream, two_pass, zmask);
+    if (r == MC_OK && mc_gemm_tail_two_outputs(t, two_pass))
         r = mc_launch_axpby(cdev, c2dev, 1.f, 1.f, cdev, (long)M * N, (hipStream_t)stream);
+    if (zmask) {
+        (void)hipStreamSynchronize((hipStream_t)stream);
+        (void)hipFree(zmask);
+    }
     return r;
 }
 
diff --git a/motioncraft_amd/csrc/mc_options.h b/motioncraft_amd/csrc/mc_options.h
--- a/motioncraft_amd/csrc/mc_options.h
+++ b/motioncraft_amd/csrc/mc_options.h
@@ -36,7 +36,7 @@
 struct McOptions {
     long chain, small_gemm_rows, split_rows_expert, split_rows_sffn, temporal_split, big_tokens, rowchain_split;
     long gemm_tune, small_tile_n, gemm_wp_grid, half_min_rows, gate_small, split_expert, split_sffn;
-    long route_reg, route_coop, route_small, route_early, route_per, dbg_delay_us;
+    long route_reg, route_coop, route_small, route_early, route_per, dbg_delay_us, zero_blocks;
 };
 
 const McOptions* mc_process_options();
diff --git a/motioncraft_amd/csrc/mc_step.hip b/motioncraft_amd/csrc/mc_step.hip
--- a/motioncraft_amd/csrc/mc_step.hip
+++ b/motioncraft_amd/csrc/mc_step.hip
@@ -562,7 +562,7 @@
         e.C = c->h; e.ldc = D; e.dup_rows = BT;
         e.M = (int)BT; e.N = D; e.K = c->m->Cp;
         if (BT <= c->opt.small_gemm_rows && D % 64 == 0 && c->m->Cp % 32 == 0) { if ((r = mc_launch_gemm_small(e, s))) return r; }
-        else if ((r = mc_launch_gemm(GM_ENC, e, 1, 0, s))) return r;
+        else if ((r = mc_launch_gemm(GM_ENC, e, 1, 0, s, c->opt.zero_blocks ? c->m->enc_ktab : nullptr))) return r;
     }
     const int nl = stop_after >= 0 ? (stop_after < g.num_layers ? stop_after : g.num_layers) : g.num_layers;
     c->no_alias = stop_after >= 0 && stop_after < g.num_layers;
@@ -637,8 +637,9 @@
         }
         t.tune = (int)c->opt.gemm_tune;
         t.C2 = c->out2 + BT * C;
-        if ((r = mc_launch_gemm_tail(t, s))) return r;
-        if (mc_gemm_tail_two_outputs(t)) x0->b = t.C2;
+        const bool two_pass = c->opt.zero_blocks >= 2 && c->dec_zmask;
+        if ((r = mc_launch_gemm_tail(t, s, two_pass, c->dec_zmask))) return r;
+        if (mc_gemm_tail_two_outputs(t, two_pass)) x0->b = t.C2;
         return MC_OK;
     }
     if (grouped) {
```

After: 664.7. No clear change (-0.2%).
